# NilsJochem/audio-matcher

Measured on AMD Instinct MI355X. Metric: audio samples/s matched (whole node), 10 s needle vs 1 h haystack, 1/2/4/8 GPU, higher is better.
Workload: dtype f32

## Files before the change

audio-matcher_amd/csrc/am_context.hip:

```cpp
#include "am_internal.h"

namespace am {

thread_local std::string t_err;

int fail(int code, const std::string& msg) {
    t_err = msg;
    return code;
}
int hip_fail(hipError_t e, const char* what) {
    char buf[256];
    snprintf(buf, sizeof(buf), "%s: %s", what, hipGetErrorString(e));
    t_err = buf;
    return e == hipErrorOutOfMemory ? AM_ERR_OOM : AM_ERR_HIP;
}

static std::mutex g_hooks_mu;
static Hooks g_hooks;
Hooks snapshot_hooks() {
    std::lock_guard<std::mutex> lk(g_hooks_mu);
    return g_hooks;
}

using OptRule = const char* (*)(long long& v);
static const char* opt_any(long long&) { return nullptr; }
static const char* opt_bool(long long& v) { v = v ? 1 : 0; return nullptr; }
static const char* opt_log_n(long long& v) { return v != 0 && (v < kLogNMin || v > kLogNMax) ? "log_n out of range" : nullptr; }
static const char* opt_half(long long& v) { v = v <= 0 ? 0 : (v >= 2 ? 2 : 1); return nullptr; }
static const char* opt_every(long long& v) { v = v < 1 ? 1 : v; return nullptr; }
static const char* opt_arm_at(long long& v) { v = v < -1 ? -2 : v; return nullptr; }
static const char* opt_needle_group(long long& v) { return v < 1 || v > kMaxNeedleGroup ? "needle_group out of range" : nullptr; }
static const char* opt_pairs(long long& v) { return v < 1 || v > 64 ? "pairs_per_group out of range" : nullptr; }
static const char* opt_score_norm(long long& v) { return v < 0 || v > 1 ? "score_norm out of range (0 = off, 1 = NCC)" : nullptr; }
static const char* opt_floor_db(long long& v) { return v < 0 || v > 200 ? "score_norm_floor_db out of range (0..200)" : nullptr; }
static const char* opt_trace_form(long long& v) { return v < 0 || v > 2 ? "trace_form out of range (0 = by bin length, 1 = wave form, 2 = sliced form)" : nullptr; }
static const char* opt_distance(long long& v) {
    return v < 0 || v > 3 ? "distance_rule out of range (bit 0: inclusive, bit 1: between plateau starts)" : nullptr;
}
struct Option {
    const char* name;
    std::atomic<long long> value;
    OptRule rule;
    long long Opts::*field;
};
static Option g_options[] = {
    {"log_n", {0}, opt_log_n, &Opts::log_n},
    {"pairs_per_group", {64}, opt_pairs, &Opts::pairs_per_group},
    {"profile_mask", {-1}, opt_any, &Opts::profile_mask},
    {"profile_every", {1}, opt_every, &Opts::profile_every},
    {"half_pipeline", {0}, opt_half, &Opts::half},
    {"batch_overlap", {1}, opt_bool, &Opts::batch_overlap},
    {"needle_group", {8}, opt_needle_group, &Opts::needle_group},
    {"pick_stream_priority", {0}, opt_bool, &Opts::pick_priority},
    {"pick_group", {1}, opt_bool, &Opts::pick_group},
    {"k3_group", {1}, opt_bool, &Opts::k3_group},
    {"host_pick_wait", {1}, opt_bool, &Opts::host_pick_wait},
    {"device_redo", {1}, opt_bool, &Opts::device_redo},
    {"tail_block", {1}, opt_bool, &Opts::tail_block},
    {"dense_scores", {0}, opt_bool, &Opts::dense},
    {"score_norm", {0}, opt_score_norm, &Opts::score_norm},
    {"score_norm_floor_db", {60}, opt_floor_db, &Opts::score_norm_floor_db},
    {"debug_no_realloc", {0}, opt_bool, &Opts::debug_no_realloc},
    {"debug_redo_arm_at", {-2}, opt_arm_at, &Opts::debug_redo_arm_at},
    {"trace_form", {0}, opt_trace_form, &Opts::trace_form},
    {"peak_filter_order", {0}, opt_bool, &Opts::peak_filter_order},
    {"distance_rule", {0}, opt_distance, &Opts::distance_rule},
    {"tail_window", {0}, opt_bool, &Opts::tail_window},
    {"surrounding_from", {0}, opt_bool, &Opts::surrounding_from},
};
static Option* find_option(const char* key) {
    for (Option& r : g_options)
        if (!strcmp(key, r.name)) return &r;
    return nullptr;
}

thread_local const Opts* t_opts_pin = nullptr;
Opts snapshot_opts(const am_needle* h) {
    if (t_opts_pin) return *t_opts_pin;
    Opts o;
    for (const Option& r : g_options) o.*r.field = r.value.load(std::memory_order_relaxed);
    if (h && h->opt_log_n >= 0) o.log_n = h->opt_log_n;
    if (h && h->opt_half >= 0) o.half = h->opt_half;
    if (h && h->opt_score_norm >= 0) o.score_norm = h->opt_score_norm;
    return o;
}

thread_local int t_no_realloc = 0;
int realloc_refused(const char* what, size_t bytes, size_t cap) {
    char buf[160];
    snprintf(buf, sizeof(buf), "debug_no_realloc: %s buffer would grow from %zu to %zu bytes while a call is queueing", what, cap, bytes);
    return fail(AM_ERR_HIP, buf);
}

static const char* kKernelNames[] = {"k1_cols_fwd", "k2_rows", "k3_cols_inv", "tile_stats", "peaks", "other", "trace", "discover"};
static std::mutex g_ctx_mu;
static std::map<int, Ctx*> g_ctx;

int get_ctx(int device, Ctx** out) {
    std::lock_guard<std::mutex> lk(g_ctx_mu);
    int n = 0;
    hipError_t e = hipGetDeviceCount(&n);
    if (e != hipSuccess || n <= 0) return fail(AM_ERR_NO_DEVICE, "no HIP device available");
    if (device < 0 || device >= n) return fail(AM_ERR_NO_DEVICE, "device ordinal out of range");
    auto it = g_ctx.find(device);
    if (it != g_ctx.end()) { *out = it->second; AM_HIP(hipSetDevice(device)); return AM_OK; }
    AM_HIP(hipSetDevice(device));
    (void)hipSetDeviceFlags(hipDeviceScheduleSpin);
    (void)hipGetLastError();
    AM_HIP(fft_kernels_init());
    Ctx* c = new Ctx();
    c->device = device;
    c->hdr.flags = hipHostMallocMapped | hipHostMallocCoherent;
    c->failcnt.flags = hipHostMallocMapped | hipHostMallocCoherent;
    c->spill.flags = hipHostMallocMapped | hipHostMallocCoherent;
    hipError_t se = hipStreamCreateWithFlags(&c->stream, hipStreamNonBlocking);
    if (se != hipSuccess) { delete c; return hip_fail(se, "hipStreamCreate"); }
    {
        int least = 0, greatest = 0;
        if (snapshot_opts(nullptr).pick_priority && hipDeviceGetStreamPriorityRange(&least, &greatest) == hipSuccess && least != greatest)
            (void)hipStreamCreateWithPriority(&c->stream2, hipStreamNonBlocking, least);
        else
            (void)hipStreamCreateWithFlags(&c->stream2, hipStreamNonBlocking);
        (void)hipGetLastError();
    }
    (void)hipStreamCreateWithFlags(&c->stream_tail, hipStreamNonBlocking);
    (void)hipEventCreateWithFlags(&c->ev_fork, kSyncEvent);
    (void)hipEventCreateWithFlags(&c->ev_join, kSyncEvent);
    (void)hipGetLastError();
    for (int i = 0; i < 2; ++i) {
        (void)hipEventCreateWithFlags(&c->ev_k3[i], kSyncEvent);
        (void)hipEventCreateWithFlags(&c->ev_pick[i], kSyncEvent);
    }
    g_ctx[device] = c;
    *out = c;
    return AM_OK;
}

static hipEvent_t prof_event(Ctx* c) {
    if (!c->pool.empty()) { hipEvent_t e = c->pool.back(); c->pool.pop_back(); return e; }
    hipEvent_t e = nullptr;
    (void)hipEventCreateWithFlags(&e, AM_EVENT_NO_SYSTEM_FENCE ? hipEventDisableSystemFence : hipEventDefault);
    return e;
}
ProfScope::ProfScope(Ctx* c_, int name_, hipStream_t st_) : c(c_), name(name_), st(st_ ? st_ : c_->stream) {
    on = c->prof;
    if (on) {
        const Opts o = snapshot_opts(nullptr);
        on = ((o.profile_mask >> name) & 1) && (c->prof_seq[name]++ % (uint64_t)std::max<long long>(1, o.profile_every)) == 0;
    }
    if (on) { e0 = prof_event(c); e1 = prof_event(c); (void)hipEventRecord(e0, st); }
}
static void prof_harvest(Ctx* c) {
    if (c->pending.empty()) return;
    (void)hipStreamSynchronize(c->stream);
    if (c->stream2) (void)hipStreamSynchronize(c->stream2);
    if (c->stream_tail) (void)hipStreamSynchronize(c->stream_tail);
    for (auto& r : c->pending) {
        float ms = 0.f;
        if (hipEventElapsedTime(&ms, r.e0, r.e1) == hipSuccess) { c->prof_ms[r.name] += ms; c->prof_n[r.name] += 1; }
        c->pool.push_back(r.e0); c->pool.push_back(r.e1);
    }
    c->pending.clear();
}

hipError_t copy_on_stream(Ctx* c, void* dst, const void* src, size_t bytes, hipMemcpyKind kind) {
    hipError_t e = hipMemcpyAsync(dst, src, bytes, kind, c->stream);
    if (e != hipSuccess) return e;
    return hipStreamSynchronize(c->stream);
}

static void fill_twiddles(std::vector<float2>& v, size_t off, size_t count, double denom, double mult) {
    for (size_t k = 0; k < count; ++k) {
        const double ang = -2.0 * M_PI * (double)k * mult / denom;
        v[off + k] = make_float2((float)std::cos(ang), (float)std::sin(ang));
    }
}

static void build_mfma_tables(std::vector<unsigned>& tab) {
    tab.assign((size_t)k2_mfma_table_dwords(), 0u);
    auto pack = [](double re, double im) {
        const _Float16 a = (_Float16)re, b = (_Float16)im;
        unsigned short ua, ub;
        memcpy(&ua, &a, 2); memcpy(&ub, &b, 2);
        return (unsigned)ua | ((unsigned)ub << 16);
    };
    auto operand = [&](size_t base, int m_off, int p_off, double denom) {
        for (int ri = 0; ri < 2; ++ri)
            for (int lane = 0; lane < 64; ++lane)
                for (int pp = 0; pp < 4; ++pp) {
                    const int m = m_off + (lane & 15), pt = p_off + 4 * (lane >> 4) + pp;
                    const double ang = 2.0 * M_PI * (double)((m * pt) % (int)denom) / denom;
                    tab[base + (size_t)ri * 256 + (size_t)lane * 4 + pp] = ri == 0 ? pack(std::cos(ang), std::sin(ang)) : pack(-std::sin(ang), std::cos(ang));
                }
    };
    operand(0, 0, 0, 16.0);
    for (int mb = 0; mb < 2; ++mb)
        for (int ks = 0; ks < 2; ++ks) operand(512 + (size_t)(mb * 2 + ks) * 512, 16 * mb, 16 * ks, 32.0);
    const size_t t1 = 512 + 2048, t2 = t1 + 256 * 32;
    for (int t = 0; t < 256; ++t) {
        const int w = t >> 6, g = (t >> 4) & 3, n = t & 15;
        for (int gl = 0; gl < 4; ++gl)
            for (int e = 0; e < 2; ++e)
                for (int r = 0; r < 4; ++r) {
                    const long long m = ((long long)(32 * (4 * w + gl) + 2 * n + e) * (4 * g + r)) % 8192;
                    const double ang = -2.0 * M_PI * (double)m / 8192.0;
                    tab[t1 + (size_t)t * 32 + gl * 8 + e * 4 + r] = pack(std::cos(ang), std::sin(ang));
                }
        for (int ch = 0; ch < 2; ++ch)
            for (int r = 0; r < 4; ++r) {
                const int m = ((16 * ch + n) * (4 * g + r)) % 512;
                const double ang = -2.0 * M_PI * (double)m / 512.0;
                tab[t2 + (size_t)t * 8 + ch * 4 + r] = pack(std::cos(ang), std::sin(ang));
            }
    }
}

// ... 370 lines not shown
```

audio-matcher_amd/csrc/am_correlate.hip:

```cpp
#include "am_internal.h"

namespace am {

static int pick_log_n(size_t s, long long out_count, const Opts& o, int* logN_out) {
    int min_log = kLogNMin;
    while (min_log <= kLogNMax && ((size_t)1 << min_log) < s + 1) ++min_log;
    if (min_log > kLogNMax) return fail(AM_ERR_INVALID_ARG, "needle too long for a forced transform size (2^23 at most; leave log_n at 0 for needle partitioning)");
    if (o.log_n > 0) {
        int l = (int)o.log_n;
        if (l < min_log) l = min_log;
        if (l > kLogNMax) l = kLogNMax;
        *logN_out = l;
        return AM_OK;
    }
    const long long span = out_count + (long long)s - 1;
    if (span > (1ll << 19)) {
        if ((long long)s <= kWideFromSamples) { *logN_out = 21; return AM_OK; }
        if ((long long)s <= kWidestFromSamples) {
            long long hop21 = (1ll << 21) - (long long)s + 1;
            if (hop21 >= 8 * kTile) hop21 = (hop21 / kTile) * kTile;
            *logN_out = (hop21 > 0 && out_count <= 2 * hop21) ? 21 : 22;
            return AM_OK;
        }
        if ((long long)s <= kSegmentFrom) {
            long long hop22 = (1ll << 22) - (long long)s + 1;
            if (hop22 >= 8 * kTile) hop22 = (hop22 / kTile) * kTile;
            *logN_out = (hop22 > 0 && out_count <= 2 * hop22) ? 22 : 23;
            return AM_OK;
        }
    }
    int pref = min_log;
    while (pref < kLogNMax) {
        const double n = (double)((size_t)1 << pref);
        if ((n - (double)s + 1.0) / n >= kMinEfficiency) break;
        ++pref;
    }
    int single = kLogNMin;
    while (single < kLogNMax && (long long)((size_t)1 << single) < span) ++single;
    *logN_out = std::min(pref, std::max(single, min_log));
    return AM_OK;
}

int plan_geometry(size_t s, long long out_count, const Opts& o, Geometry* g) {
    int rc = pick_log_n(s, out_count, o, &g->logN);
    if (rc) return rc;
    g->N = 1ll << g->logN;
    g->hop = g->N - (long long)s + 1;
    if (g->hop >= 8 * kTile) g->hop = (g->hop / kTile) * kTile;
    g->nblocks = (out_count + g->hop - 1) / g->hop;
    g->npairs = (g->nblocks + 1) / 2;
    return AM_OK;
}
bool tail_plan(size_t s, long long out_count, const Opts& o, const Geometry& g, TailPlan* t) {
    t->on = false;
    if (!o.tail_block || o.log_n != 0 || g.logN < 22 || !(g.nblocks & 1) || g.nblocks < 3 || (g.hop % kTile) != 0) return false;
    const long long T = (g.nblocks - 1) * g.hop, rest = out_count - T;
    for (int lt = 21; lt < g.logN; ++lt) {
        const long long N = 1ll << lt;
        long long hop = N - (long long)s + 1;
        if (hop < 8 * kTile) continue;
        hop = (hop / kTile) * kTile;
        if (2 * hop < rest) continue;
        t->on = true; t->T = T;
        t->g.logN = lt; t->g.N = N; t->g.hop = hop; t->g.nblocks = (rest + hop - 1) / hop; t->g.npairs = 1;
        return true;
    }
    return false;
}

static size_t sparse_word_bytes(long long nblocks, const PlanDev& pl) {
    return sizeof(unsigned long long) * (size_t)nblocks * ballot_layout(pl.logN1, pl.logN2).words;
}
size_t sparse_bytes(long long nblocks, const PlanDev& pl) {
    return sparse_word_bytes(nblocks, pl) + sizeof(float) * (size_t)nblocks * ballot_layout(pl.logN1, pl.logN2).tiles;
}
void fill_scan_cfg(ScanCfg* cfg, void* stats32, void* side, long long nblocks, const PlanDev& pl, float margin, float hist_min,
                          long long seg_c, long long seg_d) {
    cfg->stats32 = static_cast<float2*>(stats32);
    cfg->wbits = static_cast<unsigned long long*>(side);
    cfg->tile_theta = reinterpret_cast<float*>(static_cast<char*>(side) + sparse_word_bytes(nblocks, pl));
    cfg->margin = margin;
    cfg->hist_min = hist_min;
    cfg->seg_c = seg_c; cfg->seg_d = seg_d;
    cfg->inv_c = seg_c > 0 ? 1.0 / (double)seg_c : 0.0;
}
SparseScores sparse_view(const ScanCfg& cfg, long long hop, const PlanDev& pl) {
    if (cfg.margin < 0.0f) return SparseScores{nullptr, cfg.stats32, nullptr, (int)hop, pl.logN2, pl.logN1, 1.0 / (double)hop};
    return SparseScores{cfg.wbits, cfg.stats32, cfg.tile_theta, (int)hop, pl.logN2, pl.logN1, 1.0 / (double)hop};
}

bool needle_is_segmented(const am_needle* h, const Opts& o) {
    return (long long)h->n > kSegmentFrom && o.log_n == 0;
}
static void needle_segments(am_needle* h) {
    if (!h->segments.empty()) return;
    const long long n = (long long)h->n;
    const long long nseg = (n + kSegmentLen - 1) / kSegmentLen;
    for (long long i = 0; i < nseg; ++i) {
        const long long a = n * i / nseg, b = n * (i + 1) / nseg;
        am_needle* sub = new am_needle();
        sub->ctx = h->ctx; sub->d_needle = h->d_needle + a; sub->n = (size_t)(b - a);
        sub->inv_autocorr = h->inv_autocorr; sub->owns_data = false;
        h->segments.push_back(sub);
        h->seg_off.push_back(a);
    }
}

bool plan_fuses_scan(const PlanDev& pl, const Geometry& g) { return plan_has_scan(pl) && (g.hop % kTile) == 0; }

int pass_plan(am_needle* h, const Opts& o, long long out_count, bool allow_tail, PassPlan* pp) {
    Ctx* c = h->ctx;
    *pp = PassPlan{};
    int rc;
    if (needle_is_segmented(h, o)) {
        pp->kind = PassKind::Partitioned;
        needle_segments(h);
        Opts os = o;
        os.half = 0;
        pp->parts.resize(h->segments.size());
        for (size_t i = 0; i < pp->parts.size(); ++i) {
            if ((rc = pass_plan(h->segments[i], os, out_count, false, &pp->parts[i]))) return rc;
            pp->need.work = std::max(pp->need.work, pp->parts[i].need.work);
        }
        return AM_OK;
    }
    if (h->n <= (size_t)kDirectMaxNeedle && o.log_n == 0) return AM_OK;
    pp->kind = PassKind::Transform;
    Geometry& g = pp->g;
    if ((rc = plan_geometry(h->n, out_count, o, &g))) return rc;
    if ((rc = get_plan(c, g.logN, &pp->pl))) return rc;
    if ((rc = needle_k2_spectrum(h, o, pp->pl, &pp->hc, &pp->hs))) return rc;
    pp->fused = plan_fuses_scan(pp->pl->dev, g);
    if (allow_tail && pp->fused && c->stream_tail && c->ev_fork && c->ev_join && tail_plan(h->n, out_count, o, g, &pp->tail)) {
        if ((rc = get_plan(c, pp->tail.g.logN, &pp->tail_pl))) return rc;
        if ((rc = needle_k2_spectrum(h, o, pp->tail_pl, &pp->tail_hc, &pp->tail_hs))) return rc;
        pp->need.work_tail = (size_t)pp->tail.g.N * sizeof(float2);
    }
    pp->nblocks = pp->tail.on ? g.nblocks - 1 : g.nblocks;
    pp->npairs = pp->tail.on ? g.npairs - 1 : g.npairs;
    pp->main_count = pp->tail.on ? pp->tail.T : out_count;
    pp->ppg = std::min(std::max<long long>(1, o.pairs_per_group), pp->npairs);
    pp->need.work = (size_t)pp->ppg * (size_t)g.N * sizeof(float2);
    pp->need.npairs = g.npairs;
    if (pp->fused) {
        pp->need.stats32 = (size_t)((out_count + 31) / 32) * sizeof(float2);
        pp->need.side = sparse_bytes(g.nblocks, pp->pl->dev);
    }
    return AM_OK;
}

static int run_tail_block(Ctx* c, const PassPlan& pp, const void* d_src, long long src_len,
                          float* d_dst, long long out_count, float factor, const ScanCfg& main_scan, int src_kind) {
    hipStream_t st = c->stream_tail;
    const TailPlan& tail = pp.tail;
    const PlanDev& pl = pp.tail_pl->dev;
    const HalfScale& hs = pp.tail_hs;
    int rc;
    if ((rc = c->work_tail.ensure(pp.need.work_tail))) return rc;
    Job job = tail_job(tail, d_src, src_len, out_count, src_kind);
    job.dst = d_dst + tail.T;
    ScanCfg scan{};
    scan.stats32 = main_scan.stats32 ? main_scan.stats32 + tail.T / 32 : nullptr;
    scan.margin = -1.0f; scan.hist_min = FLT_MAX;
    { ProfScope ps(c, KN_OTHER, st); AM_HIP(launch_k1(st, job, 1, (float2*)c->work_tail.p, pl, hs.level)); }
    { ProfScope ps(c, KN_OTHER, st); AM_HIP(launch_k2(st, 1, (float2*)c->work_tail.p, pp.tail_hc, pl, nullptr, hs.level, hs.hscale, hs.pre, true)); }
    { ProfScope ps(c, KN_OTHER, st); AM_HIP(launch_k3(st, job, 1, (const float2*)c->work_tail.p, pl, hs.k3(factor), scan, hs.level, false)); }
    if (main_scan.stats32 && main_scan.margin >= 0.0f && main_scan.wbits && main_scan.tile_theta) {
        const BallotLayout bl = ballot_layout(pp.pl->dev.logN1, pp.pl->dev.logN2);
        const size_t blk = (size_t)(pp.g.nblocks - 1);
        AM_HIP(hipMemsetAsync(main_scan.wbits + blk * bl.words, 0xFF, bl.words * sizeof(unsigned long long), st));
        AM_HIP(hipMemsetD32Async(reinterpret_cast<hipDeviceptr_t>(main_scan.tile_theta + blk * bl.tiles), (int)0xFF7FFFFFu, bl.tiles, st));
    }
    return AM_OK;
}

static int run_correlation_one(am_needle* h, const PassPlan& pp, const void* d_src, long long src_len, long long lead,
                               float* d_dst, long long out_count, float factor,
                               const ScanRequest* scan_req, ScanResult* res, int src_kind, bool accumulate);

int run_correlation(am_needle* h, const Opts& o, const void* d_src, long long src_len, long long lead,
                           float* d_dst, long long out_count, float factor,
                           const ScanRequest* scan_req, ScanResult* res, int src_kind, const PassPlan* plan) {
    int rc;
    PassPlan own;
    if (!plan) {
        if ((rc = pass_plan(h, o, out_count, scan_req && !scan_req->no_scan && lead == 0, &own))) return rc;
        plan = &own;
    }
    if (res) { res->fused = false; res->redo_ok = false; res->sparse = plain_scores(); }
    if (plan->kind != PassKind::Partitioned) return run_correlation_one(h, *plan, d_src, src_len, lead, d_dst, out_count, factor, scan_req, res, src_kind, false);
    if (scan_req && scan_req->skip_launch) return fail(AM_ERR_INVALID_ARG, "internal: streaming ingest does not run early pairs for partitioned needles");
    for (size_t i = 0; i < plan->parts.size(); ++i) {
        ScanRequest plain{};
        if (scan_req) {
            plain.margin = -1.0f; plain.range_a = scan_req->range_a; plain.range_b = scan_req->range_b;
            plain.before_k3 = i == 0 ? scan_req->before_k3 : nullptr;
            plain.no_scan = true;
        }
        if ((rc = run_correlation_one(h->segments[i], plan->parts[i], d_src, src_len, lead - h->seg_off[i], d_dst, out_count, factor,
                                      scan_req ? &plain : nullptr, nullptr, src_kind, i > 0)))
            return rc;
    }
    return AM_OK;
}

static int run_correlation_one(am_needle* h, const PassPlan& pp, const void* d_src, long long src_len, long long lead,
                               float* d_dst, long long out_count, float factor,
                               const ScanRequest* scan_req, ScanResult* res, int src_kind, bool accumulate) {
    Ctx* c = h->ctx;
    Job job{};
    job.src = d_src; job.src_len = src_len; job.lead = lead; job.src_kind = src_kind;
    job.dst = d_dst; job.out_count = out_count;
    if (pp.kind == PassKind::Direct) {
        ProfScope ps(c, KN_OTHER);
        AM_HIP(launch_direct(c->stream, job, h->d_needle, (int)h->n, factor));
        return AM_OK;
    }
    int rc;
    const PlanDev& pl = pp.pl->dev;
    const HalfScale& hs = pp.hs;
    const TailPlan& tail = pp.tail;
    const long long N = pp.g.N, hop = pp.g.hop, npairs = pp.npairs, ppg = pp.ppg;
    const ScanBuffers out = (scan_req && scan_req->out.work) ? scan_req->out : scan_buffers(c->side[0]);
    DevBuf& wk = *out.work;
    if ((rc = wk.ensure((size_t)ppg * (size_t)N * sizeof(float2)))) return rc;
    ScanCfg scan{};
    bool fused = false;
    if (scan_req && !scan_req->no_scan) {
        if (res) res->sparse = SparseScores{nullptr, nullptr, nullptr, (int)hop, pl.logN2, pl.logN1, 1.0 / (double)hop};
        if (pp.fused) {
            const long long side_blocks = std::max(pp.g.nblocks, scan_req->side_nblocks);
            if ((rc = out.stats32->ensure((size_t)((out_count + 31) / 32) * sizeof(float2)))) return rc;
            if ((rc = out.wflags->ensure(sparse_bytes(side_blocks, pl)))) return rc;
            fill_scan_cfg(&scan, out.stats32->p, out.wflags->p, side_blocks, pl, scan_req->margin, scan_req->hist_min, scan_req->seg_c, scan_req->seg_d);
            fused = true;
            if (res) { res->fused = true; res->sparse = sparse_view(scan, hop, pl); }
        }
    }
    const float k3scale = hs.k3(factor);
    job.out_count = pp.main_count; job.hop = (int)hop; job.nblocks = (int)pp.nblocks;
    if (scan_req && scan_req->skip_launch) return AM_OK;
    long long pair_lo = 0, pair_hi = npairs;
    bool with_tail = tail.on;
    if (scan_req && scan_req->range_b > scan_req->range_a) {
        pair_lo = (scan_req->range_a / hop) / 2;
        pair_hi = std::min(npairs, ((scan_req->range_b - 1) / hop) / 2 + 1);
        with_tail = tail.on && scan_req->range_b > tail.T;
    }
    if (scan_req && scan_req->tail_by_caller) with_tail = false;
    if (with_tail) {
        AM_HIP(hipEventRecord(c->ev_fork, c->stream));
        AM_HIP(hipStreamWaitEvent(c->stream_tail, c->ev_fork, 0));
        if ((rc = run_tail_block(c, pp, d_src, src_len, d_dst, out_count, factor, scan, src_kind))) return rc;
        AM_HIP(hipEventRecord(c->ev_join, c->stream_tail));
    }
    bool waited = false;
    for (long long first = pair_lo; first < pair_hi; first += ppg) {
        const int np = (int)std::min(ppg, pair_hi - first);
        job.first_pair = (int)first;
        { ProfScope ps(c, KN_K1); AM_HIP(launch_k1(c->stream, job, np, (float2*)wk.p, pl, hs.level)); }
        { ProfScope ps(c, KN_K2); AM_HIP(launch_k2(c->stream, np, (float2*)wk.p, pp.hc, pl, nullptr, hs.level, hs.hscale, hs.pre)); }
        if (!waited && scan_req && scan_req->before_k3) AM_HIP(hipStreamWaitEvent(c->stream, scan_req->before_k3, 0));
        waited = true;
        { ProfScope ps(c, KN_K3); AM_HIP(launch_k3(c->stream, job, np, (const float2*)wk.p, pl, k3scale, scan, hs.level, accumulate)); }
    }
    if (with_tail) AM_HIP(hipStreamWaitEvent(c->stream, c->ev_join, 0));
    if (res && fused && !accumulate && pair_lo == 0 && pair_hi == npairs && npairs <= ppg) {
        res->redo_ok = true;
        job.first_pair = 0;
        res->redo_job = job; res->redo_pl = pl; res->redo_scale = k3scale; res->redo_half = hs.level;
        res->redo_npairs = (int)npairs; res->redo_work = (const float2*)wk.p; res->redo_cfg = scan;
    }
    return AM_OK;
}

float scale_factor(const am_needle* h, int scale, size_t w) {
    if (scale == AM_SCALE_LIB) return h->inv_autocorr;
    if (scale == AM_SCALE_MY) return h->inv_autocorr / (float)w;
    return 1.0f;
}

static uint64_t start_nanos(uint64_t start, uint32_t sr) {
    const double t = (double)start / (double)sr;
    if (!(t > 0.0)) return 0;
    int e = 0;
    const double m = std::frexp(t, &e);
    const unsigned long long mant = (unsigned long long)std::ldexp(m, 53);
    const int sh = e - 53;
    unsigned __int128 v = (unsigned __int128)mant * 1000000000ull;
    if (sh >= 0) return (uint64_t)(v << sh);
    const int r = -sh;
    if (r >= 127) return 0;
    unsigned __int128 q = v >> r;
    const unsigned __int128 rem = v & (((unsigned __int128)1 << r) - 1);
    const unsigned __int128 half = (unsigned __int128)1 << (r - 1);
    if (rem > half || (rem == half && (q & 1))) ++q;
    return (uint64_t)q;
}

static bool is_overshadowed(const am_peak& element, const am_peak* other, uint32_t sr, double max_distance_s) {
    if (!other) return false;
    uint64_t e = start_nanos(element.start, sr), b = start_nanos(other->start, sr);
    if (e < b) std::swap(e, b);
    const uint64_t maxd = (uint64_t)std::llround(max_distance_s * 1e9);
    return (e - b) < maxd && other->prominence > element.prominence;
}

int upload_segments(Ctx* c, const std::vector<Segment>& segs) {
    const size_t bytes = sizeof(Segment) * segs.size();
    if (c->segs.p && segs.size() == c->segs_resident.size() &&
        memcmp(segs.data(), c->segs_resident.data(), bytes) == 0)
        return AM_OK;
    int rc;
    c->segs_resident.clear();
    if ((rc = c->segs.ensure(bytes))) return rc;
    if ((rc = c->pinned.ensure(bytes))) return rc;
    memcpy(c->pinned.p, segs.data(), bytes);
    AM_HIP(hipMemcpyAsync(c->segs.p, c->pinned.p, bytes, hipMemcpyHostToDevice, c->stream));
    AM_HIP(hipStreamSynchronize(c->stream));
    c->segs_resident = segs;
    return AM_OK;
}

int prepare_results(Ctx* c, size_t nhdr, size_t arena_entries, PeakArena* arena) {
    const size_t hdr_bytes = (sizeof(SegHeader) * nhdr + 63) / 64 * 64;
    int rc;
    if ((rc = c->hdr.ensure(hdr_bytes + sizeof(am_peak) * arena_entries))) return rc;
    if ((rc = c->arena_cur.ensure(sizeof(unsigned)))) return rc;
    AM_HIP(hipMemsetAsync(c->arena_cur.p, 0, sizeof(unsigned), c->stream));
    arena->base = reinterpret_cast<am_peak*>(static_cast<char*>(c->hdr.p) + hdr_bytes);
    arena->cursor = static_cast<unsigned*>(c->arena_cur.p);
    arena->cap = (unsigned)arena_entries;
    return AM_OK;
}

int wide_reserve(Ctx* c, size_t n) {
    int rc;
    if ((rc = c->wide_ctl.ensure(n * kWideCtlBytes))) return rc;
    if ((rc = c->wide_list.ensure(n * AM_MAX_PEAKS_PER_CHUNK * sizeof(am_peak)))) return rc;
// ... 178 lines not shown
```

audio-matcher_amd/csrc/am_engine.hip:

```cpp
#include "am_internal.h"

namespace am {

static int launch_pick_group(Ctx* c, const K3Group& kg, long long n_scores, int seg_off, int nsegs, float min_prom, long long min_dist,
                             const SparseScores& sp_common, int* bad, const int* hdr_off, const PeakArena& arena, const PeakPolicy& pol,
                             hipStream_t st) {
    if (nsegs == 0 || n_scores <= 0 || kg.n <= 0) return AM_OK;
    int rc;
    const size_t nz = (size_t)kg.n, total = nz * (size_t)nsegs;
    const long long ntiles = (n_scores + kTile - 1) / kTile;
    PickGroup pg{};
    pg.n = kg.n;
    for (int z = 0; z < kg.n; ++z) {
        if ((rc = c->grp_stats[z].ensure((size_t)ntiles * sizeof(float2)))) return rc;
        pg.g[z] = kg.dst[z]; pg.stats[z] = static_cast<float2*>(c->grp_stats[z].p);
        pg.stats32[z] = kg.stats32[z]; pg.wbits[z] = kg.wbits[z]; pg.theta[z] = kg.tile_theta[z];
        pg.hdr_off[z] = hdr_off[z];
    }
    { ProfScope ps(c, KN_STATS, st);
      AM_HIP(launch_stats_reduce(st, pg.stats32[0], n_scores, pg.stats[0], bad, &pg)); }
    if ((rc = wide_reserve(c, total))) return rc;
    if ((rc = c->side[0].peaks.ensure(total * AM_MAX_PEAKS_PER_CHUNK * sizeof(am_peak)))) return rc;
    {
        ProfScope ps(c, KN_PEAKS, st);
        AM_HIP(launch_peaks(st, pg.g[0], n_scores, pg.stats[0], (const Segment*)c->segs.p + seg_off, nsegs, min_prom, min_dist,
                            (am_peak*)c->side[0].peaks.p, (SegHeader*)c->hdr.p, sp_common, arena, wide_carve(c, total), false, pol, &pg));
    }
    return AM_OK;
}


struct ChunkPlan {
    std::vector<Segment> segs, short_segs;
    std::vector<size_t> widths, short_w;
    std::vector<int> seg_off, short_off;
    std::vector<int> n_chunks;
    size_t max_scores = 0, max_segs = 1;
    int ns(size_t k) const { return seg_off[k + 1] - seg_off[k]; }
    bool too_many(size_t nn) const { return max_segs > (size_t)1 << 18 || segs.size() * nn > (size_t)1 << 24; }
};
static void plan_chunks(size_t s, const void* const* d_hays, const size_t* lens, size_t n_hay, const am_match_params* p, const Opts& o,
                        bool split_short, size_t max_windows, ChunkPlan* cp) {
    const size_t window = (size_t)(p->chunk + p->overlap);
    cp->seg_off.assign(n_hay + 1, 0);
    cp->short_off.assign(n_hay + 1, 0);
    cp->n_chunks.assign(n_hay, 0);
    for (size_t k = 0; k < n_hay; ++k) {
        cp->seg_off[k] = (int)cp->segs.size();
        cp->short_off[k] = (int)cp->short_segs.size();
        if (!d_hays[k] || lens[k] < s) continue;
        std::vector<Segment> one;
        std::vector<size_t> w1;
        make_segments(lens[k], s, p, o.tail_window != 0, one, &w1, max_windows);
        cp->n_chunks[k] = (int)one.size();
        for (size_t i = 0; i < one.size(); ++i) {
            const bool shorter = split_short && w1[i] != window;
            (shorter ? cp->short_segs : cp->segs).push_back(one[i]);
            (shorter ? cp->short_w : cp->widths).push_back(w1[i]);
        }
        if (!one.empty()) cp->max_scores = std::max(cp->max_scores, lens[k] - s + 1);
        cp->max_segs = std::max(cp->max_segs, cp->segs.size() - (size_t)cp->seg_off[k]);
    }
    cp->seg_off[n_hay] = (int)cp->segs.size();
    cp->short_off[n_hay] = (int)cp->short_segs.size();
}

struct ScoreSets {
    Ctx* c;
    bool overlap;
    size_t seq = 0;
    ScoreSets(Ctx* c_, const Opts& o, size_t n_items)
        : c(c_), overlap(o.batch_overlap && n_items > 1 && c_->stream2 && c_->ev_k3[0] && c_->ev_k3[1] && c_->ev_pick[0] && c_->ev_pick[1]) {}
    int count() const { return overlap ? 2 : 1; }
    int set() const { return overlap ? (int)(seq & 1) : 0; }
    ScoreSide& side() const { return c->side[set()]; }
    float* scores() const { return (float*)side().scores.p; }
    hipStream_t pick_stream() const { return overlap ? c->stream2 : c->stream; }
    int size(size_t max_scores, size_t max_segs) {
        int rc;
        for (int set = 0; set < count(); ++set) {
            ScoreSide& sd = c->side[set];
            if ((rc = sd.scores.ensure(max_scores * sizeof(float)))) return rc;
            if ((rc = sd.peaks.ensure(sizeof(am_peak) * max_segs * AM_MAX_PEAKS_PER_CHUNK))) return rc;
            if ((rc = sd.stats.ensure((max_scores + kTile - 1) / kTile * sizeof(float2)))) return rc;
        }
        return wide_reserve(c, max_segs);
    }
    int wait_pick(bool on_host) {
        if (!overlap || seq < 2) return AM_OK;
        if (on_host) AM_HIP(hipEventSynchronize(c->ev_pick[set()]));
        else AM_HIP(hipStreamWaitEvent(c->stream, c->ev_pick[set()], 0));
        return AM_OK;
    }
    int k3_done() {
        if (!overlap) return AM_OK;
        AM_HIP(hipEventRecord(c->ev_k3[set()], c->stream));
        AM_HIP(hipStreamWaitEvent(c->stream2, c->ev_k3[set()], 0));
        return AM_OK;
    }
    int pick_done() {
        if (overlap) AM_HIP(hipEventRecord(c->ev_pick[set()], c->stream2));
        ++seq;
        return AM_OK;
    }
    int drain() {
        AM_HIP(hipStreamSynchronize(c->stream));
        if (overlap) AM_HIP(hipStreamSynchronize(c->stream2));
        return AM_OK;
    }
};

static int match_alone(am_needle* h, const void* d_hay, size_t len, const am_match_params* p, am_peak* out, size_t cap, size_t slot,
                       size_t* n_out, int src_kind, const PartSpec* part, int* worst) {
    const int rc = match_many(h, &d_hay, &len, 1, p, out ? out + slot * cap : nullptr, cap, &n_out[slot], src_kind, 0, 1, false, nullptr, part);
    if (rc == AM_ERR_CAPACITY) *worst = rc;
    return rc == AM_ERR_CAPACITY ? AM_OK : rc;
}

static int pick_alone(am_needle* h, const Opts& o, const am_match_params* p, const void* src, long long src_len, float factor,
                      const ScanRequest& req, long long n_scores, int seg_idx, const Segment& sg, int spare_hdr, uint64_t shift, int src_kind,
                      const NormSpec& nrm, std::vector<am_peak>& all) {
    Ctx* c = h->ctx;
    const PeakPolicy pol = o.peak_policy();
    int rc;
    PeakArena own{};
    if ((rc = c->spill.ensure(sizeof(am_peak) * AM_MAX_PEAKS_PER_CHUNK))) return rc;
    AM_HIP(hipMemsetAsync(c->arena_cur.p, 0, sizeof(unsigned), c->stream));
    own.base = static_cast<am_peak*>(c->spill.p); own.cursor = static_cast<unsigned*>(c->arena_cur.p);
    own.cap = AM_MAX_PEAKS_PER_CHUNK;
    ScoreSide& side = c->side[0];
    if ((rc = side.scores.ensure((size_t)n_scores * sizeof(float)))) return rc;
    float* d_scores = (float*)side.scores.p;
    ScanResult res{};
    if ((rc = run_correlation(h, o, src, src_len, 0, d_scores, n_scores, factor, &req, &res, src_kind))) return rc;
    if (nrm.on) {
        if ((rc = normalise_scores(c, c->stream, nrm, src, src_len, src_kind, 0, (long long)h->n, d_scores, sg.a, std::min(sg.b, n_scores))))
            return rc;
        res.fused = false;
    }
    if ((rc = launch_pick(c, side, d_scores, n_scores, seg_idx, 1, p->min_prominence, (long long)p->min_distance, nullptr, &res, spare_hdr, own, pol))) return rc;
    AM_HIP(hipStreamSynchronize(c->stream));
    const SegHeader& hd = static_cast<const SegHeader*>(c->hdr.p)[spare_hdr];
    const size_t old = all.size();
    if (hd.overflow & 1) {
        if ((rc = pick_chunk_big(c, d_scores, n_scores, seg_idx, sg, p->min_prominence, (long long)p->min_distance, &res, hd.seg_min, all, pol)))
            return rc;
    } else append_header_peaks(hd, own, all);
    for (size_t j = old; j < all.size(); ++j) { all[j].start += shift; all[j].end += shift; }
    return AM_OK;
}

struct TailSlots { size_t scores, stats; };
static bool tail_batchable(const TailPlan& t) { return t.on && t.g.logN == 21; }
static int launch_tail_batch(am_needle* h, const std::vector<PassPlan>& plans, const std::vector<size_t>& members, int half_idx,
                             const TailSlots& sl, const void* const* d_hays, const size_t* lens, float factor, int src_kind) {
    Ctx* c = h->ctx;
    const PassPlan& lead = plans[members[0]];
    const TailPlan& first = lead.tail;
    const Plan* pl = lead.tail_pl;
    const float2* hc = lead.tail_hc;
    const HalfScale& hs = lead.tail_hs;
    TailBatch tb{};
    tb.n = (int)members.size();
    for (int j = 0; j < tb.n; ++j) {
        const size_t k = members[j];
        const size_t slot = (size_t)half_idx * kMaxTailBatch + (size_t)j;
        const Job job = tail_job(plans[k].tail, d_hays[k], (long long)lens[k], (long long)(lens[k] - h->n + 1), src_kind);
        tb.src[j] = job.src;
        tb.src_len[j] = job.src_len;
        tb.out_count[j] = job.out_count;
        tb.dst[j] = static_cast<float*>(c->tail_scores.p) + slot * sl.scores;
        tb.stats32[j] = static_cast<float2*>(c->tail_stats.p) + slot * sl.stats;
    }
    float2* work = static_cast<float2*>(c->work_tail.p);
    { ProfScope ps(c, KN_OTHER); AM_HIP(launch_tail_batch_k1(c->stream, tb, (int)first.g.hop, src_kind, work, pl->dev, hs.level)); }
    { ProfScope ps(c, KN_OTHER); AM_HIP(launch_k2(c->stream, tb.n, work, hc, pl->dev, nullptr, hs.level, hs.hscale, hs.pre, true)); }
    { ProfScope ps(c, KN_OTHER); AM_HIP(launch_tail_batch_k3(c->stream, tb, (int)first.g.hop, work, pl->dev, hs.k3(factor), hs.level)); }
    return AM_OK;
}

static int classify_nonfinite(am_needle* h, const PassPlan& pp, const float* d_hay, size_t len,
                              const std::vector<Segment>& segs, int s0, int s1,
                              std::vector<char>* drop, std::vector<char>* again) {
    Ctx* c = h->ctx;
    const long long s = (long long)h->n;
    const int nch = s1 - s0;
    drop->assign(nch, 0); again->assign(nch, 0);
    std::vector<Segment> ranges;
    for (int i = s0; i < s1; ++i)
        ranges.push_back(Segment{segs[i].a, std::min<long long>((long long)len, segs[i].b + s - 1)});
    const long long npairs = pp.kind == PassKind::Transform ? pp.npairs : 0;
    for (long long q = 0; q < npairs; ++q) ranges.push_back(pp.pair_reads(q, (long long)len));
    if (pp.tail.on) ranges.push_back(pp.tail_reads((long long)len));
    std::vector<int> flags(ranges.size(), 0);
    int rc = nonfinite_flags(c, d_hay, ranges.data(), (int)ranges.size(), flags.data());
    if (rc) return rc;
    for (int i = 0; i < nch; ++i) {
        if (flags[i]) { (*drop)[i] = 1; continue; }
        if (pp.kind == PassKind::Partitioned) { (*again)[i] = 1; continue; }
        const Segment sg = segs[s0 + i];
        for (long long q = 0; q < npairs && !(*again)[i]; ++q)
            if (flags[nch + q] && 2 * q * pp.g.hop < sg.b && (2 * q + 2) * pp.g.hop > sg.a) (*again)[i] = 1;
        if (pp.tail.on && flags[nch + npairs] && pp.tail.T < sg.b) (*again)[i] = 1;
    }
    return AM_OK;
}

int match_many(am_needle* h, const void* const* d_hays, const size_t* lens, size_t n_hay,
               const am_match_params* p, am_peak* out, size_t cap_per_hay, size_t* n_out, int src_kind,
               size_t index_base, size_t index_stride, bool fire_hooks, const StreamPre* pre, const PartSpec* part) {
    Ctx* c = h->ctx;
    const Opts o = snapshot_opts(h);
    const PeakPolicy pol = o.peak_policy();
    Hooks hooks = fire_hooks ? snapshot_hooks() : Hooks{};
    if (part) hooks.fn = nullptr;
    if (part && n_hay != 1) return fail(AM_ERR_INVALID_ARG, "internal: a part is one haystack");
    auto G = [&](size_t k) { return index_base + k * index_stride; };
    const size_t s = h->n;
    if (p->chunk == 0) return fail(AM_ERR_INVALID_ARG, "chunk must be > 0");
    if (p->scale < AM_SCALE_NONE || p->scale > AM_SCALE_MY) return fail(AM_ERR_INVALID_ARG, "bad scale");
    const NormSpec nrm = norm_spec(h, o);
    if (nrm.on && (pre || part)) return fail(AM_ERR_INVALID_ARG, AM_NORM_UNSUPPORTED);
    int rc = norm_check(nrm, p->scale);
    if (rc) return rc;
    const bool my = p->scale == AM_SCALE_MY;
    const float factor = nrm.on ? norm_factor(nrm) : scale_factor(h, p->scale, (size_t)(p->chunk + p->overlap));
    const int sm = p->scale == AM_SCALE_LIB ? 1 : 0;
    ScanRequest base{};
    base.margin = nrm.on ? -1.0f : write_margin(o, p);
    const bool sparse_ok = base.margin >= 0.0f;
    base.hist_min = nrm.on ? FLT_MAX : h->hist_min(sm);
    base.seg_c = (long long)p->chunk;
    base.seg_d = (long long)(p->chunk + p->overlap) - (long long)s;
    for (size_t k = 0; k < n_hay; ++k) n_out[G(k)] = 0;
    ChunkPlan cp;
    plan_chunks(s, d_hays, lens, n_hay, p, o, my, part ? part->max_windows : (size_t)-1, &cp);
    const std::vector<Segment>& segs = cp.segs;
    const std::vector<int>& seg_off = cp.seg_off;
    const size_t nsegs = segs.size();
    if (nsegs == 0 && cp.short_segs.empty()) return AM_OK;
    if (cp.too_many(1)) return fail(AM_ERR_INVALID_ARG, "chunk size too small for this haystack (more than 2^18 chunks)");
    size_t n_active = 0;
    for (size_t k = 0; k < n_hay; ++k) n_active += cp.ns(k) > 0;
    ScoreSets sets(c, o, n_active);
    if ((rc = sets.size(cp.max_scores, cp.max_segs))) return rc;
    std::vector<PassPlan> plans(n_hay);
    Footprint need;
    for (size_t k = 0; k < n_hay; ++k) {
        if (cp.n_chunks[k] == 0 || cp.ns(k) == 0) continue;
        if ((rc = pass_plan(h, o, (long long)(lens[k] - s + 1), pre == nullptr, &plans[k]))) return rc;
        need.take(plans[k].need);
    }
    std::vector<int> tail_slot(n_hay, -1);
    TailSlots tslots{0, 0};
    bool batch_tails = false;
    if (need.work_tail) {
        size_t n_tails = 0;
        for (size_t k = 0; k < n_hay; ++k)
            if (tail_batchable(plans[k].tail)) {
                ++n_tails;
                tslots.scores = std::max(tslots.scores, (size_t)(2 * plans[k].tail.g.hop));
            }
        tslots.stats = tslots.scores / 32;
        batch_tails = sets.overlap && n_tails > 1;
        const size_t nslot = batch_tails ? kMaxTailBatch : 1;
        if ((rc = c->work_tail.ensure(need.work_tail * nslot))) return rc;
        if (batch_tails) {
            if ((rc = c->tail_scores.ensure(2 * kMaxTailBatch * tslots.scores * sizeof(float)))) return rc;
            if ((rc = c->tail_stats.ensure(2 * kMaxTailBatch * tslots.stats * sizeof(float2)))) return rc;
        }
    }
    int tail_batches = 0;
    for (int set = 0; set < sets.count(); ++set) {
        if (need.work && (rc = c->side[set].work.ensure(need.work))) return rc;
        if (pre) continue;
        if (need.stats32 && (rc = c->side[set].stats32.ensure(need.stats32))) return rc;
        if (need.side && (rc = c->side[set].wflags.ensure(need.side))) return rc;
    }
    PeakArena arena{};
    if ((rc = prepare_results(c, nsegs + 1, std::min<size_t>(cp.max_segs * AM_MAX_PEAKS_PER_CHUNK, (size_t)1 << 20) + nsegs * 8, &arena))) return rc;
    std::vector<Segment> resident = segs;
    for (const Segment& sg : cp.short_segs) resident.push_back(Segment{0, sg.b - sg.a});
    const int local_seg = (int)resident.size();
    resident.push_back(Segment{0, std::max<long long>(base.seg_d + 1, 1)});
    if ((rc = upload_segments(c, resident))) return rc;
    if ((rc = c->badflag.ensure(sizeof(int) * n_hay))) return rc;
    int* h_bad = static_cast<int*>(c->badflag.p);
    memset(h_bad, 0, sizeof(int) * n_hay);
    if ((rc = c->failcnt.ensure(nsegs + 1))) return rc;
    if (nrm.on) {
        size_t max_len = 0;
        for (size_t k = 0; k < n_hay; ++k) if (cp.ns(k) > 0) max_len = std::max(max_len, lens[k]);
        if ((rc = norm_reserve(c, (long long)max_len))) return rc;
    }
    unsigned char* h_fail = static_cast<unsigned char*>(c->failcnt.p);
    memset(h_fail, 0, nsegs + 1);
    const bool device_redo = sets.overlap && sparse_ok && !needle_is_segmented(h, o) && o.device_redo != 0;
    if (device_redo) {
        for (int set = 0; set < 2; ++set)
            if ((rc = c->redo_pairs[set].ensure(sizeof(int) * (size_t)std::max<long long>(need.npairs, 1)))) return rc;
    }
    SegHeader* h_hdr = static_cast<SegHeader*>(c->hdr.p);
    auto chunk_events = [&](size_t k, int stage) {
        if (hooks.chunk_fn)
            for (int i = 0; i < cp.n_chunks[k]; ++i)
                hooks.chunk_fn(hooks.chunk_user, G(k), (part ? part->chunk_base : 0) + (size_t)i,
                               part ? part->chunk_total : (size_t)cp.n_chunks[k], stage);
    };
    const bool arm_forced = o.debug_redo_arm_at >= -1;
    bool redo_armed = device_redo && (arm_forced ? o.debug_redo_arm_at == 0 : h->redo_armed_left[sm] > 0);
    QueueingScope queueing(o.debug_no_realloc != 0);
    for (size_t k = 0; k < n_hay; ++k) {
        const int ns = cp.ns(k);
        if (cp.n_chunks[k] == 0) continue;
        if (device_redo && arm_forced) redo_armed = o.debug_redo_arm_at >= 0 && (long long)k >= o.debug_redo_arm_at;
        else if (device_redo && !redo_armed && (k & 3) == 0) {
            const volatile unsigned char* f = h_fail;
            for (int i = 0; i < seg_off[k] && !redo_armed; ++i) redo_armed = f[i] != 0;
        }
        if (hooks.fn) hooks.fn(hooks.user, G(k), 0, (size_t)cp.n_chunks[k]);
        chunk_events(k, 0);
        if (ns == 0) continue;
        const long long out_count = (long long)(lens[k] - s + 1);
        const int set = sets.set();
        const PassPlan& pp = plans[k];
        ScoreSide& side = sets.side();
        float* d_scores = sets.scores();
        ScanRequest req = base;
        req.out = scan_buffers(side);
// ... 463 lines not shown
```

audio-matcher_amd/csrc/am_fft.hip:

```cpp
#include "am_kernels.h"

#include <float.h>
#include <stdlib.h>
#include <algorithm>
#include <atomic>
#include <hip/hip_fp16.h>

namespace am {

__device__ __forceinline__ float2 cadd(float2 a, float2 b) { return make_float2(a.x + b.x, a.y + b.y); }
__device__ __forceinline__ float2 csub(float2 a, float2 b) { return make_float2(a.x - b.x, a.y - b.y); }
__device__ __forceinline__ float2 cmul(float2 a, float2 b) {
    return make_float2(a.x * b.x - a.y * b.y, a.x * b.y + a.y * b.x);
}
__device__ __forceinline__ float2 cmulc(float2 a, float2 b) {
    return make_float2(a.x * b.x + a.y * b.y, a.y * b.x - a.x * b.y);
}
__device__ __forceinline__ float2 mul_neg_i(float2 a) { return make_float2(a.y, -a.x); }
__device__ __forceinline__ float2 mul_pos_i(float2 a) { return make_float2(-a.y, a.x); }

__device__ __forceinline__ float2 tw_big(const PlanDev& pl, unsigned m) {
    return cmul(pl.twhi[m >> pl.logLo], pl.twlo[m & ((1u << pl.logLo) - 1u)]);
}

// ... 31 lines not shown
}

typedef _Float16 h2 __attribute__((ext_vector_type(2)));
__device__ __forceinline__ h2 cadd(h2 a, h2 b) { return a + b; }
__device__ __forceinline__ h2 csub(h2 a, h2 b) { return a - b; }
__device__ __forceinline__ h2 cmul(h2 a, h2 b) {
    const h2 t = a * b.xx;
    return __builtin_elementwise_fma(a.yx, (h2){-b.y, b.y}, t);
}
__device__ __forceinline__ h2 mul_neg_i(h2 a) { return (h2){a.y, -a.x}; }
__device__ __forceinline__ h2 mul_pos_i(h2 a) { return (h2){-a.y, a.x}; }
__device__ __forceinline__ h2 to_h2(float2 v) { return (h2){(_Float16)v.x, (_Float16)v.y}; }
__device__ __forceinline__ float2 to_f2(h2 v) { return make_float2((float)v.x, (float)v.y); }
__device__ __forceinline__ unsigned h2_bits(h2 v) { return __builtin_bit_cast(unsigned, v); }
__device__ __forceinline__ h2 bits_h2(unsigned u) { return __builtin_bit_cast(h2, u); }
template <bool INV>
__device__ __forceinline__ h2 mul_w32(h2 d, int idx) {
    if (idx == 0) return d;
    if (idx == 8) return INV ? mul_pos_i(d) : mul_neg_i(d);
    const _Float16 c = (_Float16)kCos32[idx], s = (_Float16)kSin32[idx];
    const h2 t = d * (h2){c, c};
    if (INV) return __builtin_elementwise_fma(d.yx, (h2){-s, s}, t);
    return __builtin_elementwise_fma(d.yx, (h2){s, -s}, t);
}

__device__ __forceinline__ float2 add_signed(float2 u, float2 v, float sgn) {
    return make_float2(fmaf(sgn, v.x, u.x), fmaf(sgn, v.y, u.y));
}

template <int R, bool INV, typename T>
__device__ __forceinline__ void dif(T* x) {
    if constexpr (R >= 2) {
#pragma unroll
        for (int i = 0; i < R / 2; ++i) {
            const T a = x[i], b = x[i + R / 2];
            x[i] = cadd(a, b);
            x[i + R / 2] = mul_w32<INV>(csub(a, b), i * (32 / R));
        }
        dif<R / 2, INV>(x);
        dif<R / 2, INV>(x + R / 2);
    }
}

template <int R, bool CONJ, bool BREV>
__device__ __forceinline__ void twiddle_apply(float2* x, float2 w) {
    float2 pw[R / 2 + 1];
    if (CONJ) w.y = -w.y;
    pw[1] = w;
    x[BREV ? brev<R>(1) : 1] = cmul(x[BREV ? brev<R>(1) : 1], w);
#pragma unroll
    for (int e = 2; e < R; ++e) {
        const float2 v = cmul(pw[(e + 1) / 2], pw[e / 2]);
        if (e <= R / 2) pw[e] = v;
        x[BREV ? brev<R>(e) : e] = cmul(x[BREV ? brev<R>(e) : e], v);
    }
}
template <int R, bool CONJ, bool BREV>
__device__ __forceinline__ void twiddle_apply(h2* x, float2 w) {
    float2 pw[R / 2 + 1];
    if (CONJ) w.y = -w.y;
    pw[1] = w;
    x[BREV ? brev<R>(1) : 1] = cmul(x[BREV ? brev<R>(1) : 1], to_h2(w));
#pragma unroll
    for (int e = 2; e < R; ++e) {
        const float2 v = cmul(pw[(e + 1) / 2], pw[e / 2]);
        if (e <= R / 2) pw[e] = v;
        x[BREV ? brev<R>(e) : e] = cmul(x[BREV ? brev<R>(e) : e], to_h2(v));
    }
}
template <int R, bool CONJ, bool BREV>
__device__ __forceinline__ void twiddle_apply2(h2* x0, h2* x1, float2 w) {
    float2 pw[R / 2 + 1];
    if (CONJ) w.y = -w.y;
    pw[1] = w;
    {
        const h2 wh = to_h2(w);
        x0[BREV ? brev<R>(1) : 1] = cmul(x0[BREV ? brev<R>(1) : 1], wh);
        x1[BREV ? brev<R>(1) : 1] = cmul(x1[BREV ? brev<R>(1) : 1], wh);
    }
#pragma unroll
    for (int e = 2; e < R; ++e) {
        const float2 v = cmul(pw[(e + 1) / 2], pw[e / 2]);
        if (e <= R / 2) pw[e] = v;
        const h2 vh = to_h2(v);
        x0[BREV ? brev<R>(e) : e] = cmul(x0[BREV ? brev<R>(e) : e], vh);
        x1[BREV ? brev<R>(e) : e] = cmul(x1[BREV ? brev<R>(e) : e], vh);
    }
}
template <int R, bool CONJ, bool BREV>
__device__ __forceinline__ void twiddle_chain(h2* x, float2 base, float2 step) {
    if (CONJ) { base.y = -base.y; step.y = -step.y; }
    float2 c = base;
    x[0] = cmul(x[0], to_h2(c));
#pragma unroll
    for (int e = 1; e < R; ++e) {
        c = cmul(c, step);
        x[BREV ? brev<R>(e) : e] = cmul(x[BREV ? brev<R>(e) : e], to_h2(c));
    }
}
template <int R, bool CONJ, bool BREV>
__device__ __forceinline__ void twiddle_chain(float2* x, float2 base, float2 step) {
    if (CONJ) { base.y = -base.y; step.y = -step.y; }
    float2 c = base;
    x[0] = cmul(x[0], c);
#pragma unroll
    for (int e = 1; e < R; ++e) {
        c = cmul(c, step);
        x[BREV ? brev<R>(e) : e] = cmul(x[BREV ? brev<R>(e) : e], c);
    }
}
template <int R, bool CONJ, typename T>
__device__ __forceinline__ void twiddle_brev(T* x, float2 w) { twiddle_apply<R, CONJ, true>(x, w); }
template <int R, bool CONJ, typename T>
__device__ __forceinline__ void twiddle_nat(T* x, float2 w) { twiddle_apply<R, CONJ, false>(x, w); }

__device__ __forceinline__ float2 tw_as(float2 v, float2) { return v; }
__device__ __forceinline__ h2 tw_as(float2 v, h2) { return to_h2(v); }
template <int R, bool CONJ, bool BREV, typename T>
__device__ __forceinline__ void twiddle_apply(T* x, float2 w, float2 w4) {
    static_assert(R == 16, "powers 1..15 from w and w^4");
    if (CONJ) { w.y = -w.y; w4.y = -w4.y; }
    float2 lo[4];
    lo[1] = w; lo[2] = cmul(w, w); lo[3] = cmul(lo[2], w);
    float2 g = w4;
#pragma unroll
    for (int e = 1; e < R; ++e) {
        if ((e & 3) == 0 && e > 4) g = cmul(g, w4);
        const float2 v = e < 4 ? lo[e] : (e & 3) == 0 ? g : cmul(g, lo[e & 3]);
        x[BREV ? brev<R>(e) : e] = cmul(x[BREV ? brev<R>(e) : e], tw_as(v, T{}));
    }
}
template <int R, bool CONJ, typename T>
__device__ __forceinline__ void twiddle_brev(T* x, float2 w, float2 w4) { twiddle_apply<R, CONJ, true>(x, w, w4); }
template <int R, bool CONJ, typename T>
__device__ __forceinline__ void twiddle_nat(T* x, float2 w, float2 w4) { twiddle_apply<R, CONJ, false>(x, w, w4); }
template <int R, bool CONJ, bool BREV, typename T>
__device__ __forceinline__ void twiddle_chain(T* x, float2 base, float2 step, float2 step4) {
    static_assert(R == 16, "four runs of four");
    if (CONJ) { base.y = -base.y; step.y = -step.y; step4.y = -step4.y; }
    float2 g = base;
#pragma unroll
    for (int k = 0; k < R; k += 4) {
        if (k) g = cmul(g, step4);
        float2 c = g;
        x[BREV ? brev<R>(k) : k] = cmul(x[BREV ? brev<R>(k) : k], tw_as(c, T{}));
#pragma unroll
        for (int j = 1; j < 4; ++j) {
            c = cmul(c, step);
            x[BREV ? brev<R>(k + j) : k + j] = cmul(x[BREV ? brev<R>(k + j) : k + j], tw_as(c, T{}));
        }
    }
}

typedef float f32x4 __attribute__((ext_vector_type(4)));
typedef float f32x2 __attribute__((ext_vector_type(2)));
__device__ __forceinline__ __amdgpu_buffer_rsrc_t make_rsrc(const void* p, unsigned bytes) {
    return __builtin_amdgcn_make_buffer_rsrc(const_cast<void*>(p), 0, bytes, 0x00020000);
}
template <int AUX = 0>
__device__ __forceinline__ float4 buf_load4(__amdgpu_buffer_rsrc_t r, unsigned voff, unsigned soff) {
    const f32x4 v = __builtin_bit_cast(f32x4, __builtin_amdgcn_raw_buffer_load_b128(r, voff, soff, AUX));
    return make_float4(v.x, v.y, v.z, v.w);
}
template <int AUX = 0>
__device__ __forceinline__ void buf_store4(__amdgpu_buffer_rsrc_t r, unsigned voff, unsigned soff, float4 v) {
    f32x4 o; o.x = v.x; o.y = v.y; o.z = v.z; o.w = v.w;
    __builtin_amdgcn_raw_buffer_store_b128(__builtin_bit_cast(__attribute__((__vector_size__(4 * sizeof(unsigned)))) unsigned, o), r, voff, soff, AUX);
    asm volatile("s_nop 1" : : "v"(o));
}

__device__ __forceinline__ unsigned pack_h2(float2 v) {
    const __half2 h = __float22half2_rn(v);
    return __builtin_bit_cast(unsigned, h);
}
__device__ __forceinline__ float2 unpack_h2(unsigned u) {
    return __half22float2(__builtin_bit_cast(__half2, u));
}
template <int AUX = 0>
__device__ __forceinline__ uint2 buf_load_u2(__amdgpu_buffer_rsrc_t r, unsigned voff, unsigned soff) {
    const f32x2 v = __builtin_bit_cast(f32x2, __builtin_amdgcn_raw_buffer_load_b64(r, voff, soff, AUX));
    const float lo = v.x, hi = v.y;
    return make_uint2(__float_as_uint(lo), __float_as_uint(hi));
}
__device__ __forceinline__ void buf_store_u2(__amdgpu_buffer_rsrc_t r, unsigned voff, unsigned soff, uint2 v) {
    typedef unsigned u32x2 __attribute__((ext_vector_type(2)));
    u32x2 o; o.x = v.x; o.y = v.y;
    __builtin_amdgcn_raw_buffer_store_b64(__builtin_bit_cast(__attribute__((__vector_size__(2 * sizeof(unsigned)))) unsigned, o), r, voff, soff, 0);
}

constexpr int kR16LogN1 = 8, kR16LogN2 = 13;
constexpr int kN2 = 1 << kR16LogN2;

__device__ __forceinline__ float downmix_s16(short2 lr) {
    return __fmul_rn((float)((int)lr.x + (int)lr.y), 0.5f * (1.0f / 65535.0f));
}
template <int KIND>
__device__ __forceinline__ float load_sample(const void* __restrict__ src, long long i) {
    if (KIND == 0) return static_cast<const float*>(src)[i];
    return downmix_s16(static_cast<const short2*>(src)[i]);
}
template <int KIND>
__device__ __forceinline__ float2 decode_sample2(uint2 raw) {
    if (KIND == 0) return make_float2(__uint_as_float(raw.x), __uint_as_float(raw.y));
    short2 a, b;
    a.x = (short)(raw.x & 0xffffu); a.y = (short)(raw.x >> 16);
    b.x = (short)(raw.y & 0xffffu); b.y = (short)(raw.y >> 16);
    return make_float2(downmix_s16(a), downmix_s16(b));
}
constexpr bool kK1LoadNt = true;
template <int KIND>
__device__ __forceinline__ float2 load_sample2(const void* __restrict__ src, long long i) {
    if (KIND == 0) {
        if (kK1LoadNt) {
            const f32x2 v = __builtin_nontemporal_load(reinterpret_cast<const f32x2*>(static_cast<const float*>(src) + i));
            return make_float2(v.x, v.y);
        }
        return *reinterpret_cast<const float2*>(static_cast<const float*>(src) + i);
    }
    typedef int i32x2 __attribute__((ext_vector_type(2)));
    const i32x2* p = reinterpret_cast<const i32x2*>(static_cast<const short2*>(src) + i);
    const i32x2 raw = kK1LoadNt ? __builtin_nontemporal_load(p) : *p;
    const int lo = raw.x, hi = raw.y;
    return make_float2(downmix_s16(__builtin_bit_cast(short2, lo)), downmix_s16(__builtin_bit_cast(short2, hi)));
}
template <int KIND>
__device__ __forceinline__ float2 load2_padded(const void* __restrict__ src, long long i, long long len) {
    float2 v;
    v.x = (i >= 0 && i < len) ? load_sample<KIND>(src, i) : 0.0f;
    v.y = (i + 1 >= 0 && i + 1 < len) ? load_sample<KIND>(src, i + 1) : 0.0f;
    return v;
}

struct K1Twiddles { float2 w256, w256q, base0, base1, step0, step1, step0q, step1q; };
__device__ __forceinline__ K1Twiddles k1_twiddles(const PlanDev& pl, long long col, int hi) {
    const unsigned maskN = (unsigned)((1ll << pl.logN) - 1);
    K1Twiddles w;
    w.w256 = pl.tw1[hi];
    w.w256q = pl.tw1[4 * hi];
    w.base0 = tw_big(pl, ((unsigned)col * (unsigned)hi) & maskN);
    w.base1 = tw_big(pl, (((unsigned)col + 1u) * (unsigned)hi) & maskN);
    tw_big_pair(pl, ((unsigned)col * 16u) & maskN, w.step0, w.step0q);
    tw_big_pair(pl, (((unsigned)col + 1u) * 16u) & maskN, w.step1, w.step1q);
    return w;
}
template <int KIND>
__device__ __forceinline__ void k1_load(const Job& job, long long col, int in_stride, int hi, long long baseA, long long baseB,
                                        bool validB, bool fast, float2 (&x0)[16], float2 (&x1)[16]) {
    if (fast) {
#pragma unroll
        for (int a = 0; a < 16; ++a) {
            const long long off = (long long)(a * 16 + hi) * in_stride + col;
            const float2 va = load_sample2<KIND>(job.src, baseA + off), vb = load_sample2<KIND>(job.src, baseB + off);
            x0[a] = make_float2(va.x, vb.x);
            x1[a] = make_float2(va.y, vb.y);
        }
    } else {
#pragma unroll
        for (int a = 0; a < 16; ++a) {
            const long long n = (long long)(a * 16 + hi) * in_stride + col;
            const float2 va = load2_padded<KIND>(job.src, baseA + n, job.src_len);
            const float2 vb = validB ? load2_padded<KIND>(job.src, baseB + n, job.src_len) : make_float2(0.f, 0.f);
            x0[a] = make_float2(va.x, vb.x);
            x1[a] = make_float2(va.y, vb.y);
        }
    }
}
__device__ __forceinline__ void k1_transform(const K1Twiddles& w, float2* lds2, int hi, int cp, float2 (&x0)[16], float2 (&x1)[16]) {
    dif<16, false>(x0);
    dif<16, false>(x1);
    twiddle_brev<16, false>(x0, w.w256, w.w256q);
    twiddle_brev<16, false>(x1, w.w256, w.w256q);
#pragma unroll
    for (int ap = 0; ap < 16; ++ap) lds2[(ap * 16 + hi) * 17 + cp] = x0[brev<16>(ap)];
    __syncthreads();
#pragma unroll
    for (int b = 0; b < 16; ++b) x0[b] = lds2[(hi * 16 + b) * 17 + cp];
    __syncthreads();
#pragma unroll
    for (int ap = 0; ap < 16; ++ap) lds2[(ap * 16 + hi) * 17 + cp] = x1[brev<16>(ap)];
    __syncthreads();
#pragma unroll
    for (int b = 0; b < 16; ++b) x1[b] = lds2[(hi * 16 + b) * 17 + cp];
    dif<16, false>(x0);
    dif<16, false>(x1);
    twiddle_chain<16, false, true>(x0, w.base0, w.step0, w.step0q);
    twiddle_chain<16, false, true>(x1, w.base1, w.step1, w.step1q);
}
template <int KIND>
__device__ __forceinline__ void k1_tile(const Job& job, const PlanDev& pl, float2* lds2, long long col, int in_stride,
                                        int hi, int cp, long long baseA, long long baseB, bool validB, bool fast,
                                        float2 (&x0)[16], float2 (&x1)[16]) {
    const K1Twiddles w = k1_twiddles(pl, col, hi);
    k1_load<KIND>(job, col, in_stride, hi, baseA, baseB, validB, fast, x0, x1);
    k1_transform(w, lds2, hi, cp, x0, x1);
}

__device__ __forceinline__ void k1_transform_h16(const K1Twiddles& w, uint2* ldsu, int hi, int cp, h2 (&x0)[16], h2 (&x1)[16]) {
    dif<16, false>(x0);
    dif<16, false>(x1);
    twiddle_apply2<16, false, true>(x0, x1, w.w256);
#pragma unroll
    for (int ap = 0; ap < 16; ++ap) ldsu[(ap * 16 + hi) * 17 + cp] = make_uint2(h2_bits(x0[brev<16>(ap)]), h2_bits(x1[brev<16>(ap)]));
    __syncthreads();
#pragma unroll
    for (int b = 0; b < 16; ++b) {
        const uint2 v = ldsu[(hi * 16 + b) * 17 + cp];
        x0[b] = bits_h2(v.x);
        x1[b] = bits_h2(v.y);
    }
    dif<16, false>(x0);
    dif<16, false>(x1);
    twiddle_chain<16, false, true>(x0, w.base0, w.step0);
    twiddle_chain<16, false, true>(x1, w.base1, w.step1);
}

template <int KIND, int HALF>
__device__ __forceinline__ void k1_cols_fwd_r16_tile(const Job& job, float2* __restrict__ work, const PlanDev& pl) {
    extern __shared__ float4 lds4[];
    const int t = threadIdx.x;
    const int hi = t >> 4, cp = t & 15;
    const int n2_0 = blockIdx.x << kColsLog;
    const int pair = job.first_pair + blockIdx.y;
    const long long blkA = 2ll * pair, blkB = blkA + 1;
    const bool validB = blkB < job.nblocks;
    const long long N = 1ll << pl.logN;
    const long long baseA = blkA * job.hop - job.lead;
    const long long baseB = blkB * job.hop - job.lead;
    const bool fast = ((reinterpret_cast<uintptr_t>(job.src) & 7) == 0) && ((baseA & 1) == 0) && ((baseB & 1) == 0) &&
                      baseA >= 0 && baseA + N <= job.src_len && validB && baseB + N <= job.src_len;
    float2 x0[16], x1[16];
    if constexpr (HALF == 2) {
        const long long col = (long long)n2_0 + 2 * cp;
        const K1Twiddles w = k1_twiddles(pl, col, hi);
        k1_load<KIND>(job, col, kN2, hi, baseA, baseB, validB, fast, x0, x1);
        h2 hx0[16], hx1[16];
#pragma unroll
        for (int a = 0; a < 16; ++a) { hx0[a] = to_h2(x0[a]); hx1[a] = to_h2(x1[a]); }
        k1_transform_h16(w, reinterpret_cast<uint2*>(lds4), hi, cp, hx0, hx1);
        uint2* __restrict__ out2 = reinterpret_cast<uint2*>(reinterpret_cast<unsigned*>(work) + ((size_t)blockIdx.y << pl.logN) + n2_0) + cp;
#pragma unroll
        for (int bp = 0; bp < 16; ++bp) {
            const size_t k1 = (size_t)(hi + 16 * bp);
            out2[k1 * (kN2 / 2)] = make_uint2(h2_bits(hx0[brev<16>(bp)]), h2_bits(hx1[brev<16>(bp)]));
        }
        return;
    }
    k1_tile<KIND>(job, pl, reinterpret_cast<float2*>(lds4), (long long)n2_0 + 2 * cp, kN2, hi, cp, baseA, baseB, validB, fast, x0, x1);
    if (HALF) {
        uint2* __restrict__ out2 = reinterpret_cast<uint2*>(reinterpret_cast<unsigned*>(work) + ((size_t)blockIdx.y << pl.logN) + n2_0) + cp;
#pragma unroll
        for (int bp = 0; bp < 16; ++bp) {
            const size_t k1 = (size_t)(hi + 16 * bp);
            out2[k1 * (kN2 / 2)] = make_uint2(pack_h2(x0[brev<16>(bp)]), pack_h2(x1[brev<16>(bp)]));
        }
        return;
    }
    float4* __restrict__ out4 = reinterpret_cast<float4*>(work + ((size_t)blockIdx.y << pl.logN) + n2_0) + cp;
#pragma unroll
    for (int bp = 0; bp < 16; ++bp) {
        const size_t k1 = (size_t)(hi + 16 * bp);
        out4[k1 * (kN2 / 2)] = make_float4(x0[brev<16>(bp)].x, x0[brev<16>(bp)].y,
                                             x1[brev<16>(bp)].x, x1[brev<16>(bp)].y);
    }
}
template <int KIND, int HALF>
__global__ void __launch_bounds__(256, 3)
k1_cols_fwd_r16(Job job, float2* __restrict__ work, PlanDev pl) {
    k1_cols_fwd_r16_tile<KIND, HALF>(job, work, pl);
}
template <int KIND, int HALF>
__global__ void __launch_bounds__(256, 3)
tail_cols_fwd_r16(TailBatch tb, int hop, float2* __restrict__ work, PlanDev pl) {
    const unsigned z = blockIdx.y;
    Job job;
    job.src = tb.src[z]; job.src_len = tb.src_len[z]; job.lead = 0; job.dst = nullptr; job.out_count = tb.out_count[z];
    job.hop = hop; job.nblocks = (int)((tb.out_count[z] + hop - 1) / hop); job.first_pair = -(int)z; job.src_kind = KIND;
    k1_cols_fwd_r16_tile<KIND, HALF>(job, work, pl);
}

__device__ __forceinline__ void wave_sync_lds() {
    __builtin_amdgcn_fence(__ATOMIC_ACQ_REL, "wavefront");
    __builtin_amdgcn_wave_barrier();
}

struct K2Lane {
    int t, hi, cp;
    unsigned voff;
    float2 wj0, wj1, wc0, wc1;
    float2 qj0, qj1, qc0, qc1;
};
__device__ __forceinline__ K2Lane k2_lane(const PlanDev& pl, int t = threadIdx.x) {
    K2Lane k;
    k.t = t; k.hi = k.t >> 4; k.cp = k.t & 15;
    k.voff = (unsigned)k.t * 16u;
    const float4 j = pl.k2j[2 * k.t], jq = pl.k2j[2 * k.t + 1], c = pl.k2c[2 * k.cp], cq = pl.k2c[2 * k.cp + 1];
    k.wj0 = make_float2(j.x, j.y); k.wj1 = make_float2(j.z, j.w);
    k.qj0 = make_float2(jq.x, jq.y); k.qj1 = make_float2(jq.z, jq.w);
    k.wc0 = make_float2(c.x, c.y); k.wc1 = make_float2(c.z, c.w);
    k.qc0 = make_float2(cq.x, cq.y); k.qc1 = make_float2(cq.z, cq.w);
    return k;
}

__device__ __forceinline__ void k2_forward12(const K2Lane& k, __amdgpu_buffer_rsrc_t rrow, float4* lds4) {
    const int t = k.t, hi = k.hi, cp = k.cp;
    float2 x0[16], x1[16];
#pragma unroll
    for (int a = 0; a < 16; ++a) {
        const float4 v = buf_load4(rrow, k.voff, a * 4096);
        x0[a] = make_float2(v.x, v.y);
        x1[a] = make_float2(v.z, v.w);
    }
    dif<16, false>(x0);
    dif<16, false>(x1);
    twiddle_brev<16, false>(x0, k.wj0, k.qj0);
    twiddle_brev<16, false>(x1, k.wj1, k.qj1);
#pragma unroll
    for (int ap = 0; ap < 16; ++ap)
        lds4[ap * 256 + t] = make_float4(x0[brev<16>(ap)].x, x0[brev<16>(ap)].y,
                                         x1[brev<16>(ap)].x, x1[brev<16>(ap)].y);
    __syncthreads();
#pragma unroll
    for (int b = 0; b < 16; ++b) {
        const float4 v = lds4[hi * 256 + b * 16 + cp];
        x0[b] = make_float2(v.x, v.y);
        x1[b] = make_float2(v.z, v.w);
    }
    dif<16, false>(x0);
    dif<16, false>(x1);
    twiddle_brev<16, false>(x0, k.wc0, k.qc0);
    twiddle_brev<16, false>(x1, k.wc1, k.qc1);
    wave_sync_lds();
#pragma unroll
    for (int bp = 0; bp < 16; ++bp)
        lds4[(hi * 16 + bp) * 16 + (cp ^ bp)] = make_float4(x0[brev<16>(bp)].x, x0[brev<16>(bp)].y,
                                                            x1[brev<16>(bp)].x, x1[brev<16>(bp)].y);
    wave_sync_lds();
}

__device__ __forceinline__ void k2_forward3(const K2Lane& k, const float4* lds4, float2 (&z)[32]) {
#pragma unroll
    for (int i = 0; i < 16; ++i) {
        const float4 v = lds4[k.t * 16 + (i ^ k.cp)];
        z[2 * i] = make_float2(v.x, v.y);
        z[2 * i + 1] = make_float2(v.z, v.w);
    }
    dif<32, false>(z);
}

__device__ __forceinline__ void k2_fetch_quarter(__amdgpu_buffer_rsrc_t rh, unsigned voff, int part, float4 (&h)[4]) {
#pragma unroll
    for (int i = 0; i < 4; ++i) h[i] = buf_load4(rh, voff, (part * 4 + i) * 4096);
}
__device__ __forceinline__ void k2_multiply_quarter(const float2 (&z)[32], const float4 (&h)[4], int part, float2 (&q)[32]) {
#pragma unroll
    for (int i = 0; i < 4; ++i) {
        const int e = part * 4 + i;
        q[brev<32>(2 * e)] = cmul(z[2 * e], make_float2(h[i].x, h[i].y));
        q[brev<32>(2 * e + 1)] = cmul(z[2 * e + 1], make_float2(h[i].z, h[i].w));
    }
}
__device__ __forceinline__ void k2_multiply_fetch(const float2 (&z)[32], __amdgpu_buffer_rsrc_t rh, unsigned voff,
                                                  const float4 (&first)[4], float2 (&q)[32]) {
    float4 ha[4], hb[4];
    k2_fetch_quarter(rh, voff, 1, ha);
    __builtin_amdgcn_sched_barrier(0);
    k2_multiply_quarter(z, first, 0, q);
    k2_fetch_quarter(rh, voff, 2, hb);
    __builtin_amdgcn_sched_barrier(0);
    k2_multiply_quarter(z, ha, 1, q);
    k2_fetch_quarter(rh, voff, 3, ha);
    __builtin_amdgcn_sched_barrier(0);
    k2_multiply_quarter(z, hb, 2, q);
    k2_multiply_quarter(z, ha, 3, q);
}

__device__ __forceinline__ void k2_place(unsigned npairs, unsigned& row, unsigned& slot) {
    const unsigned lin = blockIdx.x, xcd = lin & 7u, seq = lin >> 3;
    row = (seq / npairs) * 8u + xcd;
    slot = seq % npairs;
}

__global__ void __launch_bounds__(256, 2)
k2_rows_r16_spectrum(float2* __restrict__ work, const float2* __restrict__ hc, float2* __restrict__ hc_out, PlanDev pl,
                     unsigned npairs, float hscale) {
    extern __shared__ float4 lds4[];
    unsigned row, slot;
    k2_place(npairs, row, slot);
    const size_t row_off = ((size_t)slot << pl.logN) + (size_t)row * kN2;
    const __amdgpu_buffer_rsrc_t rrow = make_rsrc(work + row_off, kN2 * 8);
    const size_t hoff4 = (size_t)row * (kN2 / 2);
    const K2Lane k = k2_lane(pl);
    k2_forward12(k, rrow, lds4);
    float2 z[32];
    k2_forward3(k, lds4, z);
    const float invN = 1.0f / (float)(1u << pl.logN);
    const __amdgpu_buffer_rsrc_t rho = make_rsrc(reinterpret_cast<float4*>(hc_out) + hoff4, kN2 * 8);
#pragma unroll
    for (int i = 0; i < 16; ++i)
        buf_store4(rho, k.voff, i * 4096, make_float4(z[2 * i].x * invN, -z[2 * i].y * invN,
                                                     z[2 * i + 1].x * invN, -z[2 * i + 1].y * invN));
}

constexpr int kK2hSlab = 272;
constexpr int kK2hLds = 16 * kK2hSlab * 8;

constexpr int kK2hWaves = 3;
__device__ __forceinline__ void k2_rows_h16_row(unsigned* __restrict__ work, const unsigned* __restrict__ hc16, unsigned* __restrict__ dst,
                                                const PlanDev& pl, unsigned npairs, float pre) {
    extern __shared__ float4 lds4[];
    uint2* ldsu = reinterpret_cast<uint2*>(lds4);
    unsigned row, slot;
    k2_place(npairs, row, slot);
    const size_t row_off = ((size_t)slot << pl.logN) + (size_t)row * kN2;
    const __amdgpu_buffer_rsrc_t rrow = make_rsrc(work + row_off, kN2 * 4);
    const __amdgpu_buffer_rsrc_t rdst = dst ? make_rsrc(dst + row_off, kN2 * 4) : rrow;
    const K2Lane k = k2_lane(pl);
    const int t = k.t, hi = k.hi, cp = k.cp;
    h2 x0[16], x1[16];
    {
        const h2 p2 = (h2){(_Float16)pre, (_Float16)pre};
#pragma unroll
        for (int a = 0; a < 16; ++a) {
            const uint2 v = buf_load_u2(rrow, k.voff / 2, a * 2048);
            x0[a] = bits_h2(v.x) * p2;
            x1[a] = bits_h2(v.y) * p2;
        }
    }
    dif<16, false>(x0);
    dif<16, false>(x1);
    twiddle_brev<16, false>(x0, k.wj0, k.qj0);
// ... 57 lines not shown
    wave_sync_lds();
#pragma unroll
    for (int b = 0; b < 16; ++b)
        ldsu[hi * kK2hSlab + b * 16 + cp] = make_uint2(h2_bits(x0[brev<16>(b)]), h2_bits(x1[brev<16>(b)]));
    __syncthreads();
#pragma unroll
    for (int ap = 0; ap < 16; ++ap) {
        const uint2 v = ldsu[ap * kK2hSlab + t];
        x0[ap] = bits_h2(v.x);
        x1[ap] = bits_h2(v.y);
    }
    twiddle_nat<16, true>(x0, k.wj0, k.qj0);
    twiddle_nat<16, true>(x1, k.wj1, k.qj1);
    dif<16, true>(x0);
    dif<16, true>(x1);
#pragma unroll
    for (int a = 0; a < 16; ++a)
        buf_store_u2(rdst, k.voff / 2, a * 2048, make_uint2(h2_bits(x0[brev<16>(a)]), h2_bits(x1[brev<16>(a)])));
}
__global__ void __launch_bounds__(256, kK2hWaves)
k2_rows_h16(unsigned* __restrict__ work, const unsigned* __restrict__ hc16, unsigned* __restrict__ dst, PlanDev pl, unsigned npairs,
            float pre) {
    k2_rows_h16_row(work, hc16, dst, pl, npairs, pre);
}
__global__ void __launch_bounds__(256, kK2hWaves)
tail_rows_h16(unsigned* __restrict__ work, const unsigned* __restrict__ hc16, unsigned* __restrict__ dst, PlanDev pl, unsigned npairs,
              float pre) {
    k2_rows_h16_row(work, hc16, dst, pl, npairs, pre);
}

constexpr int kK2pWaves = 4;
template <bool HALF>
__device__ __forceinline__ void k2p_forward(const K2Lane& k, __amdgpu_buffer_rsrc_t rrow, float2* lds2, float2 (&z)[32]) {
    const int t = k.t, hi = k.hi, cp = k.cp;
    float2 x0[16], x1[16];
#pragma unroll
    for (int a = 0; a < 16; ++a) {
        if (HALF) {
            const uint2 v = buf_load_u2(rrow, k.voff / 2, a * 2048);
            x0[a] = unpack_h2(v.x);
            x1[a] = unpack_h2(v.y);
        } else {
            const float4 v = buf_load4(rrow, k.voff, a * 4096);
            x0[a] = make_float2(v.x, v.y);
            x1[a] = make_float2(v.z, v.w);
        }
    }
    dif<16, false>(x0);
    twiddle_brev<16, false>(x0, k.wj0, k.qj0);
#pragma unroll
    for (int ap = 0; ap < 16; ++ap) lds2[ap * kK2hSlab + t] = x0[brev<16>(ap)];
    dif<16, false>(x1);
    twiddle_brev<16, false>(x1, k.wj1, k.qj1);
    __syncthreads();
#pragma unroll
    for (int b = 0; b < 16; ++b) x0[b] = lds2[hi * kK2hSlab + b * 16 + cp];
    __syncthreads();
#pragma unroll
    for (int ap = 0; ap < 16; ++ap) lds2[ap * kK2hSlab + t] = x1[brev<16>(ap)];
    dif<16, false>(x0);
    twiddle_brev<16, false>(x0, k.wc0, k.qc0);
    __syncthreads();
#pragma unroll
    for (int b = 0; b < 16; ++b) x1[b] = lds2[hi * kK2hSlab + b * 16 + cp];
    wave_sync_lds();
#pragma unroll
    for (int bp = 0; bp < 16; ++bp) lds2[hi * kK2hSlab + bp * 16 + (cp ^ bp)] = x0[brev<16>(bp)];
    dif<16, false>(x1);
    twiddle_brev<16, false>(x1, k.wc1, k.qc1);
    wave_sync_lds();
#pragma unroll
    for (int i = 0; i < 16; ++i) z[2 * i] = lds2[hi * kK2hSlab + cp * 16 + (i ^ cp)];
    wave_sync_lds();
#pragma unroll
    for (int bp = 0; bp < 16; ++bp) lds2[hi * kK2hSlab + bp * 16 + (cp ^ bp)] = x1[brev<16>(bp)];
    wave_sync_lds();
#pragma unroll
    for (int i = 0; i < 16; ++i) z[2 * i + 1] = lds2[hi * kK2hSlab + cp * 16 + (i ^ cp)];
}

template <bool HALF, int SAUX = 0, bool LATE_J = false>
__device__ __forceinline__ void k2p_inverse(const PlanDev& pl, float2 (&q)[32], float2* lds2, __amdgpu_buffer_rsrc_t rdst) {
    int t = threadIdx.x;
    asm volatile("" : "+v"(t));
    const int hi = t >> 4, cp = t & 15;
    K2Lane ki;
    ki.t = t; ki.hi = hi; ki.cp = cp; ki.voff = (unsigned)t * 16u;
    {
        const float4 c = pl.k2c[2 * cp], cq = pl.k2c[2 * cp + 1];
        ki.wc0 = make_float2(c.x, c.y); ki.wc1 = make_float2(c.z, c.w);
        ki.qc0 = make_float2(cq.x, cq.y); ki.qc1 = make_float2(cq.z, cq.w);
    }
    if (!LATE_J) {
        const float4 j = pl.k2j[2 * t], jq = pl.k2j[2 * t + 1];
        ki.wj0 = make_float2(j.x, j.y); ki.wj1 = make_float2(j.z, j.w);
        ki.qj0 = make_float2(jq.x, jq.y); ki.qj1 = make_float2(jq.z, jq.w);
    }
    const K2Lane& k = ki;
    float2 x0[16], x1[16];
    dif<32, true>(q);
    wave_sync_lds();
#pragma unroll
    for (int i = 0; i < 16; ++i) lds2[hi * kK2hSlab + cp * 16 + (i ^ cp)] = q[brev<32>(2 * i)];
    wave_sync_lds();
#pragma unroll
    for (int bp = 0; bp < 16; ++bp) x0[bp] = lds2[hi * kK2hSlab + bp * 16 + (cp ^ bp)];
    wave_sync_lds();
#pragma unroll
    for (int i = 0; i < 16; ++i) lds2[hi * kK2hSlab + cp * 16 + (i ^ cp)] = q[brev<32>(2 * i + 1)];
    twiddle_nat<16, true>(x0, ki.wc0, ki.qc0);
    dif<16, true>(x0);
    wave_sync_lds();
#pragma unroll
    for (int bp = 0; bp < 16; ++bp) x1[bp] = lds2[hi * kK2hSlab + bp * 16 + (cp ^ bp)];
    wave_sync_lds();
#pragma unroll
    for (int b = 0; b < 16; ++b) lds2[hi * kK2hSlab + b * 16 + cp] = x0[brev<16>(b)];
    if (LATE_J) {
        __builtin_amdgcn_sched_barrier(0);
        const float4 j = pl.k2j[2 * t], jq = pl.k2j[2 * t + 1];
        ki.wj0 = make_float2(j.x, j.y); ki.wj1 = make_float2(j.z, j.w);
        ki.qj0 = make_float2(jq.x, jq.y); ki.qj1 = make_float2(jq.z, jq.w);
        __builtin_amdgcn_sched_barrier(0);
    }
    twiddle_nat<16, true>(x1, ki.wc1, ki.qc1);
    dif<16, true>(x1);
    __syncthreads();
#pragma unroll
    for (int ap = 0; ap < 16; ++ap) x0[ap] = lds2[ap * kK2hSlab + t];
    __syncthreads();
#pragma unroll
    for (int b = 0; b < 16; ++b) lds2[hi * kK2hSlab + b * 16 + cp] = x1[brev<16>(b)];
    twiddle_nat<16, true>(x0, ki.wj0, ki.qj0);
    dif<16, true>(x0);
    __syncthreads();
#pragma unroll
    for (int ap = 0; ap < 16; ++ap) x1[ap] = lds2[ap * kK2hSlab + t];
    twiddle_nat<16, true>(x1, ki.wj1, ki.qj1);
    dif<16, true>(x1);
    if (HALF) {
#pragma unroll
        for (int a = 0; a < 16; ++a)
            buf_store_u2(rdst, k.voff / 2, a * 2048, make_uint2(pack_h2(x0[brev<16>(a)]), pack_h2(x1[brev<16>(a)])));
        return;
    }
#pragma unroll
    for (int a = 0; a < 16; ++a)
        buf_store4<SAUX>(rdst, k.voff, a * 4096, make_float4(x0[brev<16>(a)].x, x0[brev<16>(a)].y,
                                                           x1[brev<16>(a)].x, x1[brev<16>(a)].y));
}

template <bool HALF>
__device__ __forceinline__ void k2_rows_r16_planes_row(float2* __restrict__ work, const float2* __restrict__ hc, float2* __restrict__ dst,
                                                       const PlanDev& pl, unsigned npairs, float hscale) {
    extern __shared__ float4 lds4[];
    float2* lds2 = reinterpret_cast<float2*>(lds4);
    unsigned row, slot;
    k2_place(npairs, row, slot);
    const size_t row_off = ((size_t)slot << pl.logN) + (size_t)row * kN2;
    const __amdgpu_buffer_rsrc_t rrow = HALF ? make_rsrc(reinterpret_cast<unsigned*>(work) + row_off, kN2 * 4)
                                             : make_rsrc(work + row_off, kN2 * 8);
    const __amdgpu_buffer_rsrc_t rdst = !dst ? rrow
        : HALF ? make_rsrc(reinterpret_cast<unsigned*>(dst) + row_off, kN2 * 4) : make_rsrc(dst + row_off, kN2 * 8);
    const __amdgpu_buffer_rsrc_t rh = make_rsrc(reinterpret_cast<const float4*>(hc) + (size_t)row * (kN2 / 2), kN2 * 8);
    const K2Lane k = k2_lane(pl);
    float2 z[32];
    k2p_forward<HALF>(k, rrow, lds2, z);
    float4 ha[4], hb[4], hc4[4];
    __builtin_amdgcn_sched_barrier(0);
    k2_fetch_quarter(rh, k.voff, 0, ha);
    k2_fetch_quarter(rh, k.voff, 1, hb);
    __builtin_amdgcn_sched_barrier(0);
    dif<32, false>(z);
    __builtin_amdgcn_sched_barrier(0);
    k2_fetch_quarter(rh, k.voff, 2, hc4);
    __builtin_amdgcn_sched_barrier(0);
    auto scaled = [&](float4 (&h)[4]) {
        if (HALF) {
#pragma unroll
            for (int i = 0; i < 4; ++i) { h[i].x *= hscale; h[i].y *= hscale; h[i].z *= hscale; h[i].w *= hscale; }
        }
    };
    float2 q[32];
    scaled(ha);
    k2_multiply_quarter(z, ha, 0, q);
    k2_fetch_quarter(rh, k.voff, 3, ha);
    __builtin_amdgcn_sched_barrier(0);
    scaled(hb);
    k2_multiply_quarter(z, hb, 1, q);
    scaled(hc4);
    k2_multiply_quarter(z, hc4, 2, q);
    scaled(ha);
    k2_multiply_quarter(z, ha, 3, q);
    k2p_inverse<HALF>(pl, q, lds2, rdst);
}
template <bool HALF>
__global__ void __launch_bounds__(256, kK2pWaves)
k2_rows_r16_planes(float2* __restrict__ work, const float2* __restrict__ hc, float2* __restrict__ dst, PlanDev pl, unsigned npairs,
                   float hscale) {
    k2_rows_r16_planes_row<HALF>(work, hc, dst, pl, npairs, hscale);
}
template <bool HALF>
__global__ void __launch_bounds__(256, kK2pWaves)
tail_rows_r16_planes(float2* __restrict__ work, const float2* __restrict__ hc, float2* __restrict__ dst, PlanDev pl, unsigned npairs,
                     float hscale) {
    k2_rows_r16_planes_row<HALF>(work, hc, dst, pl, npairs, hscale);
}

constexpr int kK2gpWaves = 3;
constexpr int kK2gStoreAux = 2;
__global__ void __launch_bounds__(256, kK2gpWaves)
k2_rows_r16_group_planes(const float2* __restrict__ work, K2Group grp, PlanDev pl, unsigned npairs) {
    extern __shared__ float4 lds4[];
    float2* lds2 = reinterpret_cast<float2*>(lds4);
    unsigned row, slot;
    k2_place(npairs, row, slot);
    const size_t row_off = ((size_t)slot << pl.logN) + (size_t)row * kN2;
    const __amdgpu_buffer_rsrc_t rrow = make_rsrc(work + row_off, kN2 * 8);
    const size_t hoff4 = (size_t)row * (kN2 / 2);
    const K2Lane k = k2_lane(pl);
    float2 z[32];
    k2p_forward<false>(k, rrow, lds2, z);
    dif<32, false>(z);
#pragma unroll 1
    for (int j = 0; j < grp.n; ++j) {
        const __amdgpu_buffer_rsrc_t rh = make_rsrc(reinterpret_cast<const float4*>(grp.hc[j]) + hoff4, kN2 * 8);
        float4 hq[4];
        k2_fetch_quarter(rh, k.voff, 0, hq);
        float2 q[32];
        k2_multiply_fetch(z, rh, k.voff, hq, q);
        k2p_inverse<false, kK2gStoreAux, true>(pl, q, lds2, make_rsrc(grp.dst[j] + row_off, kN2 * 8));
        __syncthreads();
    }
}

__global__ void __launch_bounds__(256) spectrum_to_half_kernel(const float2* __restrict__ hc, long long n, float scale, unsigned* __restrict__ out) {
    for (long long i = (long long)blockIdx.x * 256 + threadIdx.x; i < n; i += (long long)gridDim.x * 256)
        out[i] = h2_bits(to_h2(make_float2(hc[i].x * scale, hc[i].y * scale)));
}
hipError_t launch_spectrum_to_half(hipStream_t st, const float2* hc, long long n, float scale, unsigned* out) {
    hipLaunchKernelGGL(spectrum_to_half_kernel, dim3(2048), dim3(256), 0, st, hc, n, scale, out);
    return hipGetLastError();
}

typedef _Float16 half8 __attribute__((ext_vector_type(8)));
typedef float f32x4v __attribute__((ext_vector_type(4)));
typedef unsigned u32x4v __attribute__((ext_vector_type(4)));
constexpr int kM16Ps1 = 516, kM16Ps4 = 520;
constexpr int kK2mLds = 16 * kM16Ps4 * 4;
constexpr int kMfA16 = 0, kMfA32 = 2 * 64 * 4, kMfT1 = kMfA32 + 8 * 64 * 4, kMfT2 = kMfT1 + 256 * 32, kMfTotal = kMfT2 + 256 * 8;

__device__ __forceinline__ half8 as_half8(const h2 (&v)[4]) {
    u32x4v u;
    u.x = h2_bits(v[0]); u.y = h2_bits(v[1]); u.z = h2_bits(v[2]); u.w = h2_bits(v[3]);
    return __builtin_bit_cast(half8, u);
}
__device__ __forceinline__ half8 load_half8(const unsigned* p) {
    const uint4 v = *reinterpret_cast<const uint4*>(p);
    u32x4v u; u.x = v.x; u.y = v.y; u.z = v.z; u.w = v.w;
    return __builtin_bit_cast(half8, u);
}
__device__ __forceinline__ void dft16_mfma(const half8& are, const half8& aim, const h2 (&b)[4], float2 (&y)[4]) {
    const half8 bv = as_half8(b);
    const f32x4v zero = {0.f, 0.f, 0.f, 0.f};
    const f32x4v dre = __builtin_amdgcn_mfma_f32_16x16x32_f16(are, bv, zero, 0, 0, 0);
    const f32x4v dim = __builtin_amdgcn_mfma_f32_16x16x32_f16(aim, bv, zero, 0, 0, 0);
    y[0] = make_float2(dre.x, dim.x); y[1] = make_float2(dre.y, dim.y);
    y[2] = make_float2(dre.z, dim.z); y[3] = make_float2(dre.w, dim.w);
}
__device__ __forceinline__ h2 cmul_conj_a(h2 a, h2 b) {
    const h2 t = a * b.xx;
    return __builtin_elementwise_fma(a.yx, b.yy, (h2){t.x, -t.y});
}
__device__ __forceinline__ int swap_bits02(int c) { return (c & ~5) | ((c & 1) << 2) | ((c >> 2) & 1); }

constexpr int kK2mWaves = 2;
__global__ void __launch_bounds__(256, kK2mWaves)
k2_rows_m16(unsigned* __restrict__ work, const unsigned* __restrict__ hcm, unsigned* __restrict__ dst, PlanDev pl, unsigned npairs,
            float pre) {
    extern __shared__ float4 lds4[];
    unsigned* lds = reinterpret_cast<unsigned*>(lds4);
    const int t = threadIdx.x, w = t >> 6, l = t & 63, n = l & 15, g = l >> 4;
    const half8 a16re = load_half8(pl.mf + kMfA16 + l * 4), a16im = load_half8(pl.mf + kMfA16 + 256 + l * 4);
    h2 tw1[4][2][4], tw2[2][4];
    {
        const uint4* p1 = reinterpret_cast<const uint4*>(pl.mf + kMfT1 + t * 32);
#pragma unroll
        for (int gl = 0; gl < 4; ++gl)
#pragma unroll
            for (int e = 0; e < 2; ++e) {
                const uint4 v = p1[gl * 2 + e];
                tw1[gl][e][0] = bits_h2(v.x); tw1[gl][e][1] = bits_h2(v.y); tw1[gl][e][2] = bits_h2(v.z); tw1[gl][e][3] = bits_h2(v.w);
            }
        const uint4* p2 = reinterpret_cast<const uint4*>(pl.mf + kMfT2 + t * 8);
#pragma unroll
        for (int ch = 0; ch < 2; ++ch) {
            const uint4 v = p2[ch];
            tw2[ch][0] = bits_h2(v.x); tw2[ch][1] = bits_h2(v.y); tw2[ch][2] = bits_h2(v.z); tw2[ch][3] = bits_h2(v.w);
        }
    }
    const h2 prescale = (h2){(_Float16)pre, (_Float16)pre};
    const int e1w = (4 * w) * kM16Ps1 + (4 * g) * 32 + 2 * n;
    const int e1r = (4 * g) * kM16Ps1 + (4 * w) * 32 + n;
    const int blk = (4 * w) * 512;
    const int e2w = blk + swap_bits02(n) * 16 + ((g ^ (n & 3)) * 4);
    const int e2r = blk + (g & 1) * 16 + (g >> 1) * 128 + (n & 3);
    const int e3w = blk + n * 32 + ((g ^ (n & 7)) * 4);
    const int e3r = blk + g * 128 + (n & 3);
    const int e4w = (4 * w) * kM16Ps4 + g * 128 + n;
    const int e4r = (4 * g) * kM16Ps4 + w * 128 + 2 * n;
    const unsigned voff = (unsigned)(((4 * g) * 512 + 128 * w + 2 * n) * 4);
    const unsigned xcd = blockIdx.x & 7u;
    const unsigned nseq = (npairs << pl.logN1) >> 3, sstep = gridDim.x >> 3;
    for (unsigned seq = blockIdx.x >> 3; seq < nseq; seq += sstep) {
        const unsigned row = (seq / npairs) * 8u + xcd, slot = seq % npairs;
        const size_t row_off = ((size_t)slot << pl.logN) + (size_t)row * kN2;
        const __amdgpu_buffer_rsrc_t rrow = make_rsrc(work + row_off, kN2 * 4);
        const __amdgpu_buffer_rsrc_t rdst = dst ? make_rsrc(dst + row_off, kN2 * 4) : rrow;
        uint2 raw[4][4];
#pragma unroll
        for (int gl = 0; gl < 4; ++gl)
#pragma unroll
            for (int r = 0; r < 4; ++r) raw[gl][r] = buf_load_u2(rrow, voff, (unsigned)((r * 512 + 32 * gl) * 4));
#pragma unroll
        for (int gl = 0; gl < 4; ++gl) {
            h2 b0[4], b1[4];
#pragma unroll
            for (int r = 0; r < 4; ++r) { b0[r] = bits_h2(raw[gl][r].x) * prescale; b1[r] = bits_h2(raw[gl][r].y) * prescale; }
            float2 y0[4], y1[4];
            dft16_mfma(a16re, a16im, b0, y0);
            dft16_mfma(a16re, a16im, b1, y1);
#pragma unroll
            for (int r = 0; r < 4; ++r) {
                const h2 v0 = cmul(to_h2(y0[r]), tw1[gl][0][r]), v1 = cmul(to_h2(y1[r]), tw1[gl][1][r]);
                *reinterpret_cast<uint2*>(lds + e1w + gl * kM16Ps1 + r * 32) = make_uint2(h2_bits(v0), h2_bits(v1));
            }
        }
        __syncthreads();
        h2 bb[4][2][4];
#pragma unroll
        for (int q = 0; q < 4; ++q)
#pragma unroll
            for (int ch = 0; ch < 2; ++ch)
#pragma unroll
                for (int r = 0; r < 4; ++r) bb[q][ch][r] = bits_h2(lds[e1r + r * kM16Ps1 + q * 32 + 16 * ch]);
        __syncthreads();
#pragma unroll
        for (int q = 0; q < 4; ++q)
#pragma unroll
            for (int ch = 0; ch < 2; ++ch) {
                float2 y[4];
                dft16_mfma(a16re, a16im, bb[q][ch], y);
                uint4 o;
                o.x = h2_bits(cmul(to_h2(y[0]), tw2[ch][0])); o.y = h2_bits(cmul(to_h2(y[1]), tw2[ch][1]));
                o.z = h2_bits(cmul(to_h2(y[2]), tw2[ch][2])); o.w = h2_bits(cmul(to_h2(y[3]), tw2[ch][3]));
                *reinterpret_cast<uint4*>(lds + e2w + q * 512 + 256 * ch) = o;
            }
        wave_sync_lds();
        {
// ... 76 lines not shown
                dft16_mfma(a16re, a16im, bt, y);
#pragma unroll
                for (int r = 0; r < 4; ++r) lds[e4w + q * kM16Ps4 + r * 32 + 16 * ch] = h2_bits(to_h2(y[r]));
            }
        __syncthreads();
#pragma unroll
        for (int gl = 0; gl < 4; ++gl)
#pragma unroll
            for (int r = 0; r < 4; ++r) raw[gl][r] = *reinterpret_cast<const uint2*>(lds + e4r + r * kM16Ps4 + gl * 32);
        __syncthreads();
#pragma unroll
        for (int gl = 0; gl < 4; ++gl) {
            h2 b0[4], b1[4];
#pragma unroll
            for (int r = 0; r < 4; ++r) { b0[r] = cmul(bits_h2(raw[gl][r].x), tw1[gl][0][r]); b1[r] = cmul(bits_h2(raw[gl][r].y), tw1[gl][1][r]); }
            float2 y0[4], y1[4];
            dft16_mfma(a16re, a16im, b0, y0);
            dft16_mfma(a16re, a16im, b1, y1);
#pragma unroll
            for (int r = 0; r < 4; ++r)
                buf_store_u2(rdst, voff, (unsigned)((r * 512 + 32 * gl) * 4),
                             make_uint2(h2_bits(to_h2(make_float2(y0[r].x, -y0[r].y))), h2_bits(to_h2(make_float2(y1[r].x, -y1[r].y)))));
        }
    }
}

__global__ void __launch_bounds__(256) spectrum_to_half_mfma_kernel(const float2* __restrict__ hc, long long n, float scale, unsigned* __restrict__ out) {
    for (long long o = (long long)blockIdx.x * 256 + threadIdx.x; o < n; o += (long long)gridDim.x * 256) {
        const long long row = o >> kR16LogN2;
        const int within = (int)(o & (kN2 - 1)), tt = within >> 5, cp = within & 31;
        const int rr = brev<32>(cp), i = rr >> 1, e = rr & 1;
        const float2 v = hc[row * kN2 + 2 * tt + 512 * i + e];
        out[o] = h2_bits(to_h2(make_float2(v.x * scale, -v.y * scale)));
    }
}
hipError_t launch_spectrum_to_half_mfma(hipStream_t st, const float2* hc, long long n, float scale, unsigned* out) {
    hipLaunchKernelGGL(spectrum_to_half_mfma_kernel, dim3(2048), dim3(256), 0, st, hc, n, scale, out);
    return hipGetLastError();
}

__device__ __forceinline__ float min3_raw(float a, float b, float c) {
    float r;
    asm("v_min3_f32 %0, %1, %2, %3" : "=v"(r) : "v"(a), "v"(b), "v"(c));
    return r;
}
__device__ __forceinline__ float max3_raw(float a, float b, float c) {
    float r;
    asm("v_max3_f32 %0, %1, %2, %3" : "=v"(r) : "v"(a), "v"(b), "v"(c));
    return r;
}

__device__ __forceinline__ float wave_min_f(float v) {
    asm("s_nop 1\n\tv_min_f32_dpp %0, %0, %0 row_shr:1 row_mask:0xf bank_mask:0xf\n\t"
        "s_nop 1\n\tv_min_f32_dpp %0, %0, %0 row_shr:2 row_mask:0xf bank_mask:0xf\n\t"
        "s_nop 1\n\tv_min_f32_dpp %0, %0, %0 row_shr:4 row_mask:0xf bank_mask:0xf\n\t"
        "s_nop 1\n\tv_min_f32_dpp %0, %0, %0 row_shr:8 row_mask:0xf bank_mask:0xf\n\t"
        "s_nop 1\n\tv_min_f32_dpp %0, %0, %0 row_bcast:15 row_mask:0xa bank_mask:0xf\n\t"
        "s_nop 1\n\tv_min_f32_dpp %0, %0, %0 row_bcast:31 row_mask:0xc bank_mask:0xf\n\t"
        "s_nop 1"
        : "+v"(v));
    return __int_as_float(__builtin_amdgcn_readlane(__float_as_int(v), 63));
}

template <int HB>
__device__ __forceinline__ unsigned scan_swizzle(unsigned row) { return (((row >> HB) & 3u) << 1) | ((row & 3u) >> 1); }
template <int HB>
__device__ __forceinline__ int scan_row_of(int t) { return ((t & 63) >> 2) * (1 << HB) + (t >> 6) * 4 + (t & 3); }
template <int HB>
__device__ __forceinline__ void scan_put(float2* lds2, int hi, int cp, const float (&c0)[16], const float (&c1)[16]) {
    const unsigned half = (unsigned)cp & 1u, chunk = (unsigned)cp >> 1, hb = ((unsigned)hi & 3u) >> 1;
#pragma unroll
    for (int a = 0; a < 16; ++a) {
        const unsigned pos = chunk ^ ((((unsigned)a & 3u) << 1) | hb);
        lds2[a * (16 << HB) + hi * 16 + (int)((pos << 1) | half)] = make_float2(c0[a], c1[a]);
    }
}
template <int HB>
__device__ __forceinline__ void scan_row_minmax(const float4* lds4, int row, bool whole, int nvalid, float& mn, float& mx) {
    const unsigned k = scan_swizzle<HB>((unsigned)row);
    float4 v[8];
#pragma unroll
    for (int i = 0; i < 8; ++i) v[i] = lds4[row * 8 + (int)((unsigned)i ^ k)];
    if (!whole) {
        mn = FLT_MAX; mx = -FLT_MAX;
#pragma unroll
        for (int i = 0; i < 8; ++i) {
            const int c0 = i << 2;
            const float e[4] = {v[i].x, v[i].y, v[i].z, v[i].w};
#pragma unroll
            for (int j = 0; j < 4; ++j)
                if (c0 + j < nvalid) { mn = fminf(mn, e[j]); mx = fmaxf(mx, e[j]); }
        }
        return;
    }
    mn = min3_raw(v[0].x, v[0].y, v[0].z); mx = max3_raw(v[0].x, v[0].y, v[0].z);
    mn = min3_raw(mn, v[0].w, v[1].x);     mx = max3_raw(mx, v[0].w, v[1].x);
#pragma unroll
    for (int i = 1; i < 8; ++i) {
        if (i > 1) { mn = min3_raw(mn, v[i - 1].w, v[i].x); mx = max3_raw(mx, v[i - 1].w, v[i].x); }
        mn = min3_raw(mn, v[i].y, v[i].z); mx = max3_raw(mx, v[i].y, v[i].z);
    }
    mn = fminf(mn, v[7].w); mx = fmaxf(mx, v[7].w);
}

__device__ __forceinline__ long long mod_recip(long long x, long long c, double inv_c) {
    long long q = (long long)((double)x * inv_c);
    long long r = x - q * c;
    if (r < 0) r += c;
    else if (r >= c) r -= c;
    return r;
}
__device__ __forceinline__ bool run_has_chunk_edge(long long lo, long long c, long long d, double inv_c) {
    if (c <= 0) return true;
    if (mod_recip(lo + 31, c, inv_c) <= 31) return true;
    const long long hi2 = lo + 31 - d;
    if (hi2 < 0) return false;
    return mod_recip(hi2, c, inv_c) <= 31;
}

struct K3Edges {
    long long outA, outB;
    int relcA, reldA, relcB, reldB;
    bool one_edge;
};
__device__ __forceinline__ K3Edges k3_edges(const Job& job, const ScanCfg& scan, long long blkA, long long blkB) {
    K3Edges e;
    e.outA = blkA * job.hop; e.outB = blkB * job.hop;
    e.one_edge = scan.stats32 != nullptr && scan.seg_c >= (long long)job.hop + 32;
    e.relcA = e.reldA = e.relcB = e.reldB = 0x7fffffff;
    if (scan.edges_n > 0) {
        const int s = (int)(blkA >> 1) - job.first_pair;
        e.relcA = scan.edge_rel[s][0]; e.reldA = scan.edge_rel[s][1];
        e.relcB = scan.edge_rel[s][2]; e.reldB = scan.edge_rel[s][3];
        return e;
    }
    if (e.one_edge) {
        const long long c = scan.seg_c, d = scan.seg_d;
        const long long m = mod_recip(e.outA, c, scan.inv_c);
        const long long ecA = m == 0 ? e.outA : e.outA + (c - m);
        long long edA = d;
        if (e.outA > d) {
            const long long m2 = mod_recip(e.outA - d, c, scan.inv_c);
            edA = m2 == 0 ? e.outA : e.outA + (c - m2);
        }
        const long long ecB = ecA >= e.outB ? ecA : ecA + c;
        const long long edB = edA >= e.outB ? edA : edA + c;
        auto rel = [](long long edge, long long start) { const long long r = edge - start; return r < 0x7fffffffll ? (int)r : 0x7fffffff; };
        e.relcA = rel(ecA, e.outA); e.reldA = rel(edA, e.outA);
        e.relcB = rel(ecB, e.outB); e.reldB = rel(edB, e.outB);
    }
    return e;
}

template <int HB, bool ACC = false, bool SCALED = false>
__device__ __forceinline__ void k3_finish(const Job& job, const ScanCfg& scan, const K3Edges& ed, float2* lds2,
                                          int n2_0, int out_stride, int t, long long blkA, long long blkB,
                                          float out_scale, const float2 (&x0)[16], const float2 (&x1)[16]) {
    const int hi = t >> 4, cp = t & 15;
    const long long col = n2_0 + 2 * cp;
    const long long outA = ed.outA, outB = ed.outB;
    const bool one_edge = ed.one_edge;
    const bool dst8 = ((reinterpret_cast<uintptr_t>(job.dst) & 7) == 0) && ((job.hop & 1) == 0);
    long long limA = job.out_count - outA; if (limA > job.hop) limA = job.hop;
    long long limB = blkB < job.nblocks ? job.out_count - outB : 0; if (limB > job.hop) limB = job.hop;
    float sa0[16], sa1[16], sb0[16], sb1[16];
#pragma unroll
    for (int a = 0; a < 16; ++a) {
        const float2 v0 = x0[brev<16>(a)], v1 = x1[brev<16>(a)];
        if (SCALED) {
            sa0[a] = v0.x; sa1[a] = v1.x;
            sb0[a] = v0.y; sb1[a] = v1.y;
        } else {
            sa0[a] = v0.x * out_scale; sa1[a] = v1.x * out_scale;
            sb0[a] = v0.y * out_scale; sb1[a] = v1.y * out_scale;
        }
    }
    unsigned wantA[2] = {0x11111111u, 0x11111111u}, wantB[2] = {0x11111111u, 0x11111111u};
    if (!ACC && scan.stats32 != nullptr) {
        const int row = scan_row_of<HB>(t);
        const int rowrun = row * out_stride + n2_0;
        const int leftA = (int)limA - rowrun, leftB = (int)limB - rowrun;
        const bool wholeA = leftA >= 32 || leftA <= 0, wholeB = leftB >= 32 || leftB <= 0;
        const float4* lds4 = reinterpret_cast<const float4*>(lds2);
        float rmnA, rmxA, rmnB, rmxB;
        __syncthreads();
        scan_put<HB>(lds2, hi, cp, sa0, sa1);
        wave_sync_lds();
        scan_row_minmax<HB>(lds4, row, wholeA, leftA < 32 ? leftA : 32, rmnA, rmxA);
        wave_sync_lds();
        scan_put<HB>(lds2, hi, cp, sb0, sb1);
        wave_sync_lds();
        scan_row_minmax<HB>(lds4, row, wholeB, leftB < 32 ? leftB : 32, rmnB, rmxB);
        float tminA = wave_min_f(leftA > 0 ? rmnA : FLT_MAX), tminB = wave_min_f(leftB > 0 ? rmnB : FLT_MAX);
        float* slots = reinterpret_cast<float*>(lds2 + scan_row_of<HB>(t & ~63) * 16);
        wave_sync_lds();
        if ((t & 63) == 0) { slots[0] = tminA; slots[1] = tminB; }
        __syncthreads();
#pragma unroll
        for (int w = 0; w < (1 << (HB - 2)); ++w) {
            const float* v = reinterpret_cast<const float*>(lds2 + scan_row_of<HB>(w * 64) * 16);
            tminA = fminf(tminA, v[0]);
            tminB = fminf(tminB, v[1]);
        }
        const bool dense = scan.margin < 0.0f;
        const float thA = dense ? -FLT_MAX : fminf(fminf(tminA, tminB), scan.hist_min) + scan.margin, thB = thA;
        bool edgeA, edgeB;
        if (one_edge) {
            edgeA = leftA > 0 && ((unsigned)(ed.relcA - rowrun) <= 31u || (unsigned)(ed.reldA - rowrun) <= 31u);
            edgeB = leftB > 0 && ((unsigned)(ed.relcB - rowrun) <= 31u || (unsigned)(ed.reldB - rowrun) <= 31u);
        } else {
            edgeA = leftA > 0 && run_has_chunk_edge(outA + rowrun, scan.seg_c, scan.seg_d, scan.inv_c);
            edgeB = leftB > 0 && run_has_chunk_edge(outB + rowrun, scan.seg_c, scan.seg_d, scan.inv_c);
        }
        const bool pa = (leftA > 0 && rmxA >= thA) || edgeA, pb = (leftB > 0 && rmxB >= thB) || edgeB;
        const unsigned long long ba = __ballot(pa), bb = __ballot(pb);
        const unsigned sh = (unsigned)hi & 3u;
        wantA[0] = ((unsigned)ba >> sh) & 0x11111111u; wantA[1] = ((unsigned)(ba >> 32) >> sh) & 0x11111111u;
        wantB[0] = ((unsigned)bb >> sh) & 0x11111111u; wantB[1] = ((unsigned)(bb >> 32) >> sh) & 0x11111111u;
        const long long tileA = blkA * (out_stride >> kColsLog) + ((unsigned)n2_0 >> kColsLog), tileB = tileA + (out_stride >> kColsLog);
        if (t == 0 && scan.tile_theta != nullptr) {
            scan.tile_theta[tileA] = thA;
            if (blkB < job.nblocks) scan.tile_theta[tileB] = thB;
        }
        if ((t & 63) == 0 && scan.wbits != nullptr) {
            scan.wbits[(tileA << (HB - 2)) + (t >> 6)] = ba;
            if (blkB < job.nblocks) scan.wbits[(tileB << (HB - 2)) + (t >> 6)] = bb;
        }
        if (leftA > 0) scan.stats32[(outA + rowrun) >> 5] = make_float2(rmnA, rmxA);
        if (leftB > 0) scan.stats32[(outB + rowrun) >> 5] = make_float2(rmnB, rmxB);
    }
    if (wantA[0] | wantA[1]) {
#pragma unroll
        for (int a = 0; a < 16; ++a) {
            if (!((wantA[a >> 3] >> ((a & 7) * 4)) & 1u)) continue;
            const long long n = (long long)(a * (1 << HB) + hi) * out_stride + col;
            if (dst8 && n + 1 < limA) {
                float2* ptr = reinterpret_cast<float2*>(job.dst + outA + n);
                float2 v = make_float2(sa0[a], sa1[a]);
                if (ACC) { const float2 o = *ptr; v.x += o.x; v.y += o.y; }
                *ptr = v;
            } else {
                if (n < limA) job.dst[outA + n] = sa0[a] + (ACC ? job.dst[outA + n] : 0.0f);
                if (n + 1 < limA) job.dst[outA + n + 1] = sa1[a] + (ACC ? job.dst[outA + n + 1] : 0.0f);
            }
            if (ACC && (a & 3) == 3) __builtin_amdgcn_sched_barrier(0);
        }
    }
    if (wantB[0] | wantB[1]) {
#pragma unroll
        for (int a = 0; a < 16; ++a) {
            if (!((wantB[a >> 3] >> ((a & 7) * 4)) & 1u)) continue;
            const long long n = (long long)(a * (1 << HB) + hi) * out_stride + col;
            if (dst8 && n + 1 < limB) {
                float2* ptr = reinterpret_cast<float2*>(job.dst + outB + n);
                float2 v = make_float2(sb0[a], sb1[a]);
                if (ACC) { const float2 o = *ptr; v.x += o.x; v.y += o.y; }
                *ptr = v;
            } else {
                if (n < limB) job.dst[outB + n] = sb0[a] + (ACC ? job.dst[outB + n] : 0.0f);
                if (n + 1 < limB) job.dst[outB + n + 1] = sb1[a] + (ACC ? job.dst[outB + n + 1] : 0.0f);
            }
            if (ACC && (a & 3) == 3) __builtin_amdgcn_sched_barrier(0);
        }
    }
}


template <bool ACC = false>
__device__ __forceinline__ void k3_tile(const Job& job, const PlanDev& pl, const ScanCfg& scan, float2* lds2,
                                        int n2_0, int out_stride, int t, long long blkA, long long blkB,
                                        float out_scale, float2 (&x0)[16], float2 (&x1)[16], const ScanCfg* geo = nullptr) {
    const int hi = t >> 4, cp = t & 15;
    const long long N = 1ll << pl.logN;
    const long long col = n2_0 + 2 * cp;
    const K3Edges ed = k3_edges(job, geo ? *geo : scan, blkA, blkB);
    const unsigned maskN = (unsigned)(N - 1);
    const float2 w256 = pl.tw1[hi], w256q = pl.tw1[4 * hi];
    {
        const unsigned n2 = (unsigned)col;
        float2 base0 = tw_big(pl, (n2 * (unsigned)hi) & maskN);
        float2 base1 = tw_big(pl, ((n2 + 1) * (unsigned)hi) & maskN);
        base0.x *= out_scale; base0.y *= out_scale;
        base1.x *= out_scale; base1.y *= out_scale;
        float2 step0, step1, step0q, step1q;
        tw_big_pair(pl, (n2 * 16u) & maskN, step0, step0q);
        tw_big_pair(pl, ((n2 + 1) * 16u) & maskN, step1, step1q);
        twiddle_chain<16, true, false>(x0, base0, step0, step0q);
        dif<16, true>(x0);
#pragma unroll
        for (int b = 0; b < 16; ++b) lds2[(hi * 16 + b) * 16 + cp] = x0[brev<16>(b)];
        twiddle_chain<16, true, false>(x1, base1, step1, step1q);
    }
    dif<16, true>(x1);
    __syncthreads();
#pragma unroll
    for (int ap = 0; ap < 16; ++ap) x0[ap] = lds2[(ap * 16 + hi) * 16 + cp];
    __syncthreads();
#pragma unroll
    for (int b = 0; b < 16; ++b) lds2[(hi * 16 + b) * 16 + cp] = x1[brev<16>(b)];
    twiddle_nat<16, true>(x0, w256, w256q);
    dif<16, true>(x0);
    __syncthreads();
#pragma unroll
    for (int ap = 0; ap < 16; ++ap) x1[ap] = lds2[(ap * 16 + hi) * 16 + cp];
    twiddle_nat<16, true>(x1, w256, w256q);
    dif<16, true>(x1);
    k3_finish<4, ACC, true>(job, scan, ed, lds2, n2_0, out_stride, t, blkA, blkB, out_scale, x0, x1);
}

__device__ __forceinline__ void k3_tile_h16(const Job& job, const PlanDev& pl, const ScanCfg& scan, float2* lds2,
                                            int n2_0, int out_stride, int t, long long blkA, long long blkB,
                                            float out_scale, h2 (&hx0)[16], h2 (&hx1)[16]) {
    const int hi = t >> 4, cp = t & 15;
    const long long N = 1ll << pl.logN;
    const long long col = n2_0 + 2 * cp;
    const K3Edges ed = k3_edges(job, scan, blkA, blkB);
    const unsigned maskN = (unsigned)(N - 1);
    const float2 w256 = pl.tw1[hi];
    {
        const unsigned n2 = (unsigned)col;
        const float2 base0 = tw_big(pl, (n2 * (unsigned)hi) & maskN);
        const float2 base1 = tw_big(pl, ((n2 + 1) * (unsigned)hi) & maskN);
        const float2 step0 = tw_big(pl, (n2 * 16u) & maskN);
        const float2 step1 = tw_big(pl, ((n2 + 1) * 16u) & maskN);
        twiddle_chain<16, true, false>(hx0, base0, step0);
        twiddle_chain<16, true, false>(hx1, base1, step1);
    }
    dif<16, true>(hx0);
    dif<16, true>(hx1);
    uint2* ldsu = reinterpret_cast<uint2*>(lds2);
#pragma unroll
    for (int b = 0; b < 16; ++b) ldsu[(hi * 16 + b) * 16 + cp] = make_uint2(h2_bits(hx0[brev<16>(b)]), h2_bits(hx1[brev<16>(b)]));
    __syncthreads();
    float2 x0[16], x1[16];
#pragma unroll
    for (int ap = 0; ap < 16; ++ap) {
        const uint2 v = ldsu[(ap * 16 + hi) * 16 + cp];
        x0[ap] = to_f2(bits_h2(v.x));
        x1[ap] = to_f2(bits_h2(v.y));
    }
    twiddle_nat<16, true>(x0, w256);
    twiddle_nat<16, true>(x1, w256);
    dif<16, true>(x0);
    dif<16, true>(x1);
    k3_finish<4>(job, scan, ed, lds2, n2_0, out_stride, t, blkA, blkB, out_scale, x0, x1);
}

constexpr int kK3Waves = 3;
constexpr int kK3LoadAux = 2, kK3hLoadAux = 2;
template <int HALF, bool ACC>
__device__ __forceinline__ void k3_cols_inv_r16_tile(unsigned lin, float4* lds4, const Job& job, const float2* __restrict__ work,
                                                     const PlanDev& pl, float out_scale, const ScanCfg& scan, const ScanCfg* geo = nullptr) {
    const int t = threadIdx.x;
    const int hi = t >> 4, cp = t & 15;
    const unsigned xcd = lin & 7u, seq = lin >> 3;
    const unsigned slot = seq >> 5, half = (seq >> 4) & 1u, tl = seq & 15u;
    const int n2_0 = (int)(((half * 8u + xcd) * 16u + tl) << kColsLog);
    const int pair = job.first_pair + (int)slot;
    if (scan.only_pairs != nullptr && scan.only_pairs[pair] == 0) return;
    const long long blkA = 2ll * pair, blkB = blkA + 1;
    if constexpr (HALF == 2) {
        const uint2* __restrict__ in2 = reinterpret_cast<const uint2*>(reinterpret_cast<const unsigned*>(work) + ((size_t)slot << pl.logN) + n2_0) + cp;
        h2 hx0[16], hx1[16];
#pragma unroll
        for (int bp = 0; bp < 16; ++bp) {
            const uint2 v = in2[(size_t)(hi + 16 * bp) * (kN2 / 2)];
            hx0[bp] = bits_h2(v.x);
            hx1[bp] = bits_h2(v.y);
        }
        k3_tile_h16(job, pl, scan, reinterpret_cast<float2*>(lds4), n2_0, kN2, t, blkA, blkB, out_scale, hx0, hx1);
        return;
    }
    float2 x0[16], x1[16];
    if (HALF) {
        const uint2* __restrict__ in2 = reinterpret_cast<const uint2*>(reinterpret_cast<const unsigned*>(work) + ((size_t)slot << pl.logN) + n2_0) + cp;
#pragma unroll
        for (int bp = 0; bp < 16; ++bp) {
            const uint2 v = in2[(size_t)(hi + 16 * bp) * (kN2 / 2)];
            x0[bp] = unpack_h2(v.x);
            x1[bp] = unpack_h2(v.y);
        }
    } else {
        const __amdgpu_buffer_rsrc_t rin = make_rsrc(work + ((size_t)slot << pl.logN) + n2_0, (unsigned)((((size_t)1 << pl.logN) - n2_0) * 8));
        const unsigned voff = (unsigned)hi * (kN2 * 8u) + (unsigned)cp * 16u;
#pragma unroll
        for (int bp = 0; bp < 16; ++bp) {
            const float4 v = buf_load4<kK3LoadAux>(rin, voff, (unsigned)bp * (16u * kN2 * 8u));
            x0[bp] = make_float2(v.x, v.y);
            x1[bp] = make_float2(v.z, v.w);
        }
    }
    k3_tile<ACC>(job, pl, scan, reinterpret_cast<float2*>(lds4), n2_0, kN2, t, blkA, blkB, out_scale, x0, x1, geo);
}
template <int HALF, bool ACC = false, int REDO = 0>
__global__ void __launch_bounds__(256, REDO ? 4 : kK3Waves)
k3_cols_inv_r16(Job job, const float2* __restrict__ work, PlanDev pl, float out_scale, ScanCfg scan) {
    extern __shared__ float4 lds4[];
    if constexpr (REDO != 0) {
        for (unsigned lin = blockIdx.x; lin < (unsigned)scan.redo_tiles; lin += gridDim.x) {
            k3_cols_inv_r16_tile<HALF, ACC>(lin, lds4, job, work, pl, out_scale, scan);
            __syncthreads();
        }
    } else {
        k3_cols_inv_r16_tile<HALF, ACC>(blockIdx.x, lds4, job, work, pl, out_scale, scan);
    }
}

__global__ void __launch_bounds__(256, kK3Waves)
k3_cols_inv_r16_group(Job job, PlanDev pl, ScanCfg scan, K3Group grp) {
    extern __shared__ float4 lds4[];
    const unsigned z = blockIdx.y;
    job.dst = grp.dst[z]; job.out_count = grp.out_count[z];
    ScanCfg mine;
    mine.stats32 = grp.stats32[z]; mine.wbits = grp.wbits[z]; mine.tile_theta = grp.tile_theta[z]; mine.hist_min = grp.hist_min[z];
    mine.margin = scan.margin; mine.seg_c = grp.seg_c; mine.seg_d = grp.seg_d[z]; mine.inv_c = grp.inv_c;
    mine.only_pairs = nullptr; mine.redo_tiles = 0; mine.edges_n = 0;
    k3_cols_inv_r16_tile<0, false>(blockIdx.x, lds4, job, grp.work[z], pl, grp.out_scale[z], mine, &scan);
}

template <int HALF>
__global__ void __launch_bounds__(256, kK3Waves)
tail_cols_inv_r16(TailBatch tb, int hop, const float2* __restrict__ work, PlanDev pl, float out_scale) {
    extern __shared__ float4 lds4[];
    const unsigned z = blockIdx.y;
    Job job;
    job.src = nullptr; job.src_len = 0; job.lead = 0; job.dst = tb.dst[z]; job.out_count = tb.out_count[z];
    job.hop = hop; job.nblocks = (int)((tb.out_count[z] + hop - 1) / hop); job.first_pair = 0; job.src_kind = 0;
    ScanCfg mine;
    mine.stats32 = tb.stats32[z]; mine.wbits = nullptr; mine.tile_theta = nullptr; mine.margin = -1.0f; mine.hist_min = FLT_MAX;
    mine.seg_c = 0; mine.seg_d = 0; mine.inv_c = 0.0; mine.only_pairs = nullptr; mine.redo_tiles = 0; mine.edges_n = 0;
    const float2* mywork = HALF ? reinterpret_cast<const float2*>(reinterpret_cast<const unsigned*>(work) + ((size_t)z << pl.logN))
                                : work + ((size_t)z << pl.logN);
    k3_cols_inv_r16_tile<HALF, false>(blockIdx.x, lds4, job, mywork, pl, out_scale, mine);
}

__global__ void __launch_bounds__(256)
tail_commit_kernel(const float* __restrict__ tsc, float* __restrict__ sc, long long n, const float2* __restrict__ tst, float2* __restrict__ st32,
                   unsigned long long* __restrict__ wbits, long long words, float* __restrict__ theta, int tiles) {
    const long long tid = (long long)blockIdx.x * blockDim.x + threadIdx.x, nth = (long long)gridDim.x * blockDim.x;
    const long long n4 = n >> 2;
    const float4* __restrict__ t4 = reinterpret_cast<const float4*>(tsc);
    float4* __restrict__ s4 = reinterpret_cast<float4*>(sc);
    for (long long i = tid; i < n4; i += nth) s4[i] = t4[i];
    for (long long i = (n4 << 2) + tid; i < n; i += nth) sc[i] = tsc[i];
    const long long n32 = (n + 31) >> 5;
    for (long long i = tid; i < n32; i += nth) st32[i] = tst[i];
    if (wbits != nullptr)
        for (long long i = tid; i < words; i += nth) wbits[i] = ~0ull;
    if (theta != nullptr)
        for (long long i = tid; i < tiles; i += nth) theta[i] = -FLT_MAX;
}

__global__ void __launch_bounds__(256)
tail_preset_group_kernel(K3Group grp, long long blk, int log_n1, int log_n2) {
    const unsigned z = blockIdx.y;
    const long long tiles = 1ll << (log_n2 - kColsLog), words = tiles << (log_n1 - 6);
    const long long tid = (long long)blockIdx.x * blockDim.x + threadIdx.x, nth = (long long)gridDim.x * blockDim.x;
    unsigned long long* __restrict__ wb = grp.wbits[z] + blk * words;
    float* __restrict__ th = grp.tile_theta[z] + blk * tiles;
    for (long long i = tid; i < words; i += nth) wb[i] = ~0ull;
    for (long long i = tid; i < tiles; i += nth) th[i] = -FLT_MAX;
}

constexpr int kC512Slab = 560;
__device__ __forceinline__ int c512_idx(int ap, int b, int cp) { return ap * kC512Slab + b * 17 + cp; }
constexpr int kC512Lds = (15 * kC512Slab + 31 * 17 + 16) * 8;
static_assert(kC512Lds >= 512 * 16 * 8, "K3's score scan needs 512 rows x 32 scores");
constexpr int kC512Slab3 = 32 * 16 + 16;
__device__ __forceinline__ int c512_idx3(int ap, int b, int cp) { return ap * kC512Slab3 + b * 16 + cp; }
static_assert((15 * kC512Slab3 + 31 * 16 + 16) * 8 <= kC512Lds, "K3's exchange fits the kernel's LDS");

template <int KIND, int HALF, int LN2 = kR16LogN2>
__global__ void __launch_bounds__(512, 4)
k1_cols_fwd_c512(Job job, float2* __restrict__ work, PlanDev pl) {
    constexpr int kN2 = 1 << LN2;
    extern __shared__ float4 lds4[];
    float2* lds2 = reinterpret_cast<float2*>(lds4);
    const int t = threadIdx.x;
    const int hi = t >> 4, cp = t & 15;
    const int ap = hi & 15, half = hi >> 4;
    const int k10 = ap + 16 * half;
    const int n2_0 = blockIdx.x << kColsLog;
    const int pair = job.first_pair + blockIdx.y;
    const long long blkA = 2ll * pair, blkB = blkA + 1;
    const bool validB = blkB < job.nblocks;
    const long long N = 1ll << pl.logN;
    const long long baseA = blkA * job.hop - job.lead;
    const long long baseB = blkB * job.hop - job.lead;
    const bool fast = ((reinterpret_cast<uintptr_t>(job.src) & 7) == 0) && ((baseA & 1) == 0) && ((baseB & 1) == 0) &&
                      baseA >= 0 && baseA + N <= job.src_len && validB && baseB + N <= job.src_len;
    const long long col = (long long)n2_0 + 2 * cp;
    const unsigned maskN = (unsigned)(N - 1);
    const float2 w512 = pl.tw1[hi];
    const float2 w512q = pl.tw1[4 * hi];
    const float2 base0 = tw_big(pl, ((unsigned)col * (unsigned)k10) & maskN);
    const float2 base1 = tw_big(pl, (((unsigned)col + 1u) * (unsigned)k10) & maskN);
    float2 step0, step1, step0q, step1q;
    if constexpr (HALF == 2) {
        step0 = tw_big(pl, ((unsigned)col * 32u) & maskN);
        step1 = tw_big(pl, (((unsigned)col + 1u) * 32u) & maskN);
    }
    float2 x0[16], x1[16];
    if (fast && KIND == 1) {
        const __amdgpu_buffer_rsrc_t rsrc = make_rsrc(static_cast<const char*>(job.src) + 4 * baseA, (unsigned)(4 * (N + job.hop)));
        const unsigned voff = 4u * ((unsigned)hi * kN2 + (unsigned)col), offB = 4u * (unsigned)job.hop;
#pragma unroll
        for (int a = 0; a < 16; ++a) {
            const float2 va = decode_sample2<KIND>(buf_load_u2<kK1LoadNt ? 2 : 0>(rsrc, voff, (unsigned)a * (4u * 32u * kN2)));
            const float2 vb = decode_sample2<KIND>(buf_load_u2<kK1LoadNt ? 2 : 0>(rsrc, voff, (unsigned)a * (4u * 32u * kN2) + offB));
            x0[a] = make_float2(va.x, vb.x);
            x1[a] = make_float2(va.y, vb.y);
        }
    } else if (fast) {
#pragma unroll
        for (int a = 0; a < 16; ++a) {
            const long long off = (long long)(a * 32 + hi) * kN2 + col;
            const float2 va = load_sample2<KIND>(job.src, baseA + off), vb = load_sample2<KIND>(job.src, baseB + off);
            x0[a] = make_float2(va.x, vb.x);
            x1[a] = make_float2(va.y, vb.y);
        }
    } else {
#pragma unroll
        for (int a = 0; a < 16; ++a) {
            const long long n = (long long)(a * 32 + hi) * kN2 + col;
            const float2 va = load2_padded<KIND>(job.src, baseA + n, job.src_len);
            const float2 vb = validB ? load2_padded<KIND>(job.src, baseB + n, job.src_len) : make_float2(0.f, 0.f);
            x0[a] = make_float2(va.x, vb.x);
            x1[a] = make_float2(va.y, vb.y);
        }
    }
    if constexpr (HALF == 2) {
        h2 hx0[16], hx1[16];
#pragma unroll
        for (int a = 0; a < 16; ++a) { hx0[a] = to_h2(x0[a]); hx1[a] = to_h2(x1[a]); }
        dif<16, false>(hx0);
        dif<16, false>(hx1);
        twiddle_apply2<16, false, true>(hx0, hx1, w512);
        uint2* ldsu = reinterpret_cast<uint2*>(lds4);
#pragma unroll
        for (int a2 = 0; a2 < 16; ++a2) ldsu[c512_idx(a2, hi, cp)] = make_uint2(h2_bits(hx0[brev<16>(a2)]), h2_bits(hx1[brev<16>(a2)]));
        __syncthreads();
#pragma unroll
        for (int b = 0; b < 16; ++b) {
            const uint2 lo = ldsu[c512_idx(ap, b, cp)], up = ldsu[c512_idx(ap, b + 16, cp)];
            hx0[b] = half ? mul_w32<false>(csub(bits_h2(lo.x), bits_h2(up.x)), b) : cadd(bits_h2(lo.x), bits_h2(up.x));
            hx1[b] = half ? mul_w32<false>(csub(bits_h2(lo.y), bits_h2(up.y)), b) : cadd(bits_h2(lo.y), bits_h2(up.y));
        }
        dif<16, false>(hx0);
        dif<16, false>(hx1);
        twiddle_chain<16, false, true>(hx0, base0, step0);
        twiddle_chain<16, false, true>(hx1, base1, step1);
        uint2* __restrict__ out2 = reinterpret_cast<uint2*>(reinterpret_cast<unsigned*>(work) + ((size_t)blockIdx.y << pl.logN) + n2_0) + cp;
#pragma unroll
        for (int bt = 0; bt < 16; ++bt) {
            const size_t k1 = (size_t)(k10 + 32 * bt);
            out2[k1 * (kN2 / 2)] = make_uint2(h2_bits(hx0[brev<16>(bt)]), h2_bits(hx1[brev<16>(bt)]));
        }
        return;
    }
    dif<16, false>(x0);
    dif<16, false>(x1);
    twiddle_brev<16, false>(x0, w512, w512q);
    twiddle_brev<16, false>(x1, w512, w512q);
    float2 y0[16], y1[16];
#pragma unroll
    for (int a2 = 0; a2 < 16; ++a2) lds2[c512_idx(a2, hi, cp)] = x0[brev<16>(a2)];
    __syncthreads();
#pragma unroll
    for (int b = 0; b < 16; ++b) {
        const float2 lo = lds2[c512_idx(ap, b, cp)], up = lds2[c512_idx(ap, b + 16, cp)];
        y0[b] = half ? mul_w32<false>(csub(lo, up), b) : cadd(lo, up);
    }
    __syncthreads();
#pragma unroll
    for (int a2 = 0; a2 < 16; ++a2) lds2[c512_idx(a2, hi, cp)] = x1[brev<16>(a2)];
    __syncthreads();
#pragma unroll
    for (int b = 0; b < 16; ++b) {
        const float2 lo = lds2[c512_idx(ap, b, cp)], up = lds2[c512_idx(ap, b + 16, cp)];
        y1[b] = half ? mul_w32<false>(csub(lo, up), b) : cadd(lo, up);
    }
    __builtin_amdgcn_sched_barrier(0);
    tw_big_pair(pl, ((unsigned)col * 32u) & maskN, step0, step0q);
    tw_big_pair(pl, (((unsigned)col + 1u) * 32u) & maskN, step1, step1q);
    __builtin_amdgcn_sched_barrier(0);
    dif<16, false>(y0);
// ... 473 lines not shown
    const long long blkA = 2ll * pair, blkB = blkA + 1;
    const bool validB = blkB < job.nblocks;
    const long long baseA = blkA * job.hop - job.lead;
    const long long baseB = blkB * job.hop - job.lead;
    const int total = N1 << BL;
    for (int idx = tid; idx < total; idx += nthr) {
        const int r = idx >> BL, c = idx & ((1 << BL) - 1);
        const long long n = (long long)r * N2 + n2_0 + c;
        const float a = load_padded<KIND>(job.src, baseA + n, job.src_len);
        const float b = validB ? load_padded<KIND>(job.src, baseB + n, job.src_len) : 0.0f;
        s[idx] = make_float2(a, b);
    }
    __syncthreads();
    lds_fft_fwd<BL>(s, pl.logN1, pl.tw1, tid, nthr);
    float2* out = work + ((size_t)blockIdx.y << pl.logN) + n2_0;
    const unsigned maskN = (1u << pl.logN) - 1u;
    for (int idx = tid; idx < total; idx += nthr) {
        const int p = idx >> BL, c = idx & ((1 << BL) - 1);
        const unsigned k1 = __brev((unsigned)p) >> (32 - pl.logN1);
        const float2 w = tw_big(pl, ((unsigned)(n2_0 + c) * k1) & maskN);
        out[(size_t)p * N2 + c] = cmul(s[idx], w);
    }
}

template <bool SPECTRUM>
__global__ void __launch_bounds__(kFftThreads)
k2_rows_gen(float2* __restrict__ work, const float2* __restrict__ hc, float2* __restrict__ hc_out, PlanDev pl) {
    extern __shared__ float2 s[];
    const int N2 = 1 << pl.logN2;
    const int tid = threadIdx.x, nthr = blockDim.x;
    const int p = blockIdx.x;
    float2* row = work + ((size_t)blockIdx.y << pl.logN) + (size_t)p * N2;
    for (int n2 = tid; n2 < N2; n2 += nthr) s[n2] = row[n2];
    __syncthreads();
    lds_fft_fwd<0>(s, pl.logN2, pl.tw2, tid, nthr);
    const size_t hoff = (size_t)p * N2;
    if (SPECTRUM) {
        const float invN = 1.0f / (float)(1u << pl.logN);
        for (int q = tid; q < N2; q += nthr) {
            const float2 v = s[q];
            hc_out[hoff + q] = make_float2(v.x * invN, -v.y * invN);
        }
        return;
    }
    for (int q = tid; q < N2; q += nthr) s[q] = cmul(s[q], hc[hoff + q]);
    __syncthreads();
    lds_fft_inv<0>(s, pl.logN2, pl.tw2, tid, nthr);
    float2* orow = hc_out ? hc_out + ((size_t)blockIdx.y << pl.logN) + (size_t)p * N2 : row;
    for (int n2 = tid; n2 < N2; n2 += nthr) orow[n2] = s[n2];
}

template <int BL>
__global__ void __launch_bounds__(kFftThreads)
k3_cols_inv_gen(Job job, const float2* __restrict__ work, PlanDev pl, float out_scale, int acc) {
    extern __shared__ float2 s[];
    const int N1 = 1 << pl.logN1, N2 = 1 << pl.logN2;
    const int tid = threadIdx.x, nthr = blockDim.x;
    const int n2_0 = blockIdx.x << BL;
    const int pair = job.first_pair + blockIdx.y;
    const long long blkA = 2ll * pair, blkB = blkA + 1;
    const bool validB = blkB < job.nblocks;
    const int total = N1 << BL;
    const float2* in = work + ((size_t)blockIdx.y << pl.logN) + n2_0;
    const unsigned maskN = (1u << pl.logN) - 1u;
    for (int idx = tid; idx < total; idx += nthr) {
        const int p = idx >> BL, c = idx & ((1 << BL) - 1);
        const unsigned k1 = __brev((unsigned)p) >> (32 - pl.logN1);
        const float2 w = tw_big(pl, ((unsigned)(n2_0 + c) * k1) & maskN);
        s[idx] = cmulc(in[(size_t)p * N2 + c], w);
    }
    __syncthreads();
    lds_fft_inv<BL>(s, pl.logN1, pl.tw1, tid, nthr);
    const long long outA = blkA * job.hop, outB = blkB * job.hop;
    for (int idx = tid; idx < total; idx += nthr) {
        const int r = idx >> BL, c = idx & ((1 << BL) - 1);
        const long long n = (long long)r * N2 + n2_0 + c;
        if (n >= job.hop) continue;
        const float2 v = s[idx];
        if (outA + n < job.out_count) job.dst[outA + n] = v.x * out_scale + (acc ? job.dst[outA + n] : 0.0f);
        if (validB && outB + n < job.out_count) job.dst[outB + n] = v.y * out_scale + (acc ? job.dst[outB + n] : 0.0f);
    }
}

template <int KIND>
__global__ void __launch_bounds__(256)
correlate_direct(Job job, const float* __restrict__ needle, int s, float out_scale) {
    __shared__ float nd[kDirectMaxNeedle];
    if ((int)threadIdx.x < s) nd[threadIdx.x] = needle[threadIdx.x];
    __syncthreads();
    for (long long j = (long long)blockIdx.x * 256 + threadIdx.x; j < job.out_count; j += (long long)gridDim.x * 256) {
        float acc = 0.0f;
        for (int n = 0; n < s; ++n) acc = fmaf(load_padded<KIND>(job.src, j + n - job.lead, job.src_len), nd[n], acc);
        job.dst[j] = acc * out_scale;
    }
}

hipError_t launch_direct(hipStream_t st, const Job& job, const float* needle, int s, float out_scale) {
    if (s < 1 || s > kDirectMaxNeedle || job.out_count <= 0) return hipErrorInvalidValue;
    long long blocks = (job.out_count + 255) / 256;
    if (blocks > 4096) blocks = 4096;
    if (job.src_kind == 1) hipLaunchKernelGGL(correlate_direct<1>, dim3((unsigned)blocks), dim3(256), 0, st, job, needle, s, out_scale);
    else hipLaunchKernelGGL(correlate_direct<0>, dim3((unsigned)blocks), dim3(256), 0, st, job, needle, s, out_scale);
    return hipGetLastError();
}

template <typename Fn>
struct Variant { Fn fn; int threads; int lds; };

template <typename Fn, typename... Args>
static hipError_t launch_row_lds(const Variant<Fn>& v, dim3 grid, size_t lds, hipStream_t st, const Args&... args) {
    if (v.fn == nullptr) return hipErrorInvalidValue;
    hipLaunchKernelGGL(v.fn, grid, dim3(v.threads), lds, st, args...);
    return hipGetLastError();
}
template <typename Fn, typename... Args>
static hipError_t launch_row(const Variant<Fn>& v, dim3 grid, hipStream_t st, const Args&... args) {
    return launch_row_lds(v, grid, (size_t)v.lds, st, args...);
}

bool plan_is_r16(const PlanDev& pl) { return pl.logN1 == kR16LogN1 && pl.logN2 == kR16LogN2; }
bool plan_is_c512(const PlanDev& pl) { return pl.logN1 == 9 && pl.logN2 == kR16LogN2; }
bool plan_is_c1024(const PlanDev& pl) { return pl.logN1 == 10 && pl.logN2 == kR16LogN2; }
bool plan_is_c512w(const PlanDev& pl) { return pl.logN1 == 9 && pl.logN2 == 14; }
bool plan_has_scan(const PlanDev& pl) { return plan_is_r16(pl) || plan_is_c512(pl) || plan_is_c1024(pl); }
bool plan_k2_is_r16(const PlanDev& pl) { return pl.logN2 == kR16LogN2 && pl.logN1 >= 3; }

enum ColPlan { kColR16, kColC512, kColC1024, kColC512w, kColGen, kColPlans };
static ColPlan col_plan(const PlanDev& pl) {
    return plan_is_r16(pl) ? kColR16 : plan_is_c512(pl) ? kColC512 : plan_is_c1024(pl) ? kColC1024 : plan_is_c512w(pl) ? kColC512w : kColGen;
}
static int half_level(int half) { return half == 2 ? 2 : half ? 1 : 0; }

static constexpr int kMaxLds = 160 * 1024;
static constexpr int kR16Lds = 64 * 1024;
static constexpr int kR16LdsK1 = 256 * 17 * 8;
static constexpr int kR16LdsK3 = 256 * 16 * 8;

using K1Fn = void (*)(Job, float2*, PlanDev);
static constexpr Variant<K1Fn> kK1[kColPlans][2][3] = {
     {{{k1_cols_fwd_r16<0, 0>, 256, kR16LdsK1}, {k1_cols_fwd_r16<0, 1>, 256, kR16LdsK1}, {k1_cols_fwd_r16<0, 2>, 256, kR16LdsK1}},
                 {{k1_cols_fwd_r16<1, 0>, 256, kR16LdsK1}, {k1_cols_fwd_r16<1, 1>, 256, kR16LdsK1}, {k1_cols_fwd_r16<1, 2>, 256, kR16LdsK1}}},
     {{{k1_cols_fwd_c512<0, 0>, 512, kC512Lds}, {k1_cols_fwd_c512<0, 1>, 512, kC512Lds}, {k1_cols_fwd_c512<0, 2>, 512, kC512Lds}},
                 {{k1_cols_fwd_c512<1, 0>, 512, kC512Lds}, {k1_cols_fwd_c512<1, 1>, 512, kC512Lds}, {k1_cols_fwd_c512<1, 2>, 512, kC512Lds}}},
     {{{k1_cols_fwd_c1024<0>, 1024, kC1024Lds}}, {{k1_cols_fwd_c1024<1>, 1024, kC1024Lds}}},
     {{{k1_cols_fwd_c512<0, 0, 14>, 512, kC512Lds}}},
     {{{k1_cols_fwd_gen<kColsLog, 0>, kFftThreads, kMaxLds}}, {{k1_cols_fwd_gen<kColsLog, 1>, kFftThreads, kMaxLds}}},
};
using TailK1Fn = void (*)(TailBatch, int, float2*, PlanDev);
static constexpr Variant<TailK1Fn> kTailK1[2][3] = {
    {{tail_cols_fwd_r16<0, 0>, 256, kR16LdsK1}, {tail_cols_fwd_r16<0, 1>, 256, kR16LdsK1}, {tail_cols_fwd_r16<0, 2>, 256, kR16LdsK1}},
    {{tail_cols_fwd_r16<1, 0>, 256, kR16LdsK1}, {tail_cols_fwd_r16<1, 1>, 256, kR16LdsK1}, {tail_cols_fwd_r16<1, 2>, 256, kR16LdsK1}},
};

using K2Fn = void (*)(float2*, const float2*, float2*, PlanDev, unsigned, float);
static constexpr Variant<K2Fn> kK2[2][2] = {
    {{k2_rows_r16_planes<false>, 256, kK2hLds}, {tail_rows_r16_planes<false>, 256, kK2hLds}},
    {{k2_rows_r16_planes<true>, 256, kK2hLds}, {tail_rows_r16_planes<true>, 256, kK2hLds}},
};
static constexpr Variant<K2Fn> kK2Spectrum = {k2_rows_r16_spectrum, 256, kR16Lds};
using K2hFn = void (*)(unsigned*, const unsigned*, unsigned*, PlanDev, unsigned, float);
static constexpr Variant<K2hFn> kK2h[2] = {{k2_rows_h16, 256, kK2hLds}, {tail_rows_h16, 256, kK2hLds}};
static constexpr Variant<K2hFn> kK2Mfma = {k2_rows_m16, 256, kK2mLds};
using K2GroupFn = void (*)(const float2*, K2Group, PlanDev, unsigned);
static constexpr Variant<K2GroupFn> kK2Group = {k2_rows_r16_group_planes, 256, kK2hLds};
using K2GenFn = void (*)(float2*, const float2*, float2*, PlanDev);
static constexpr Variant<K2GenFn> kK2Gen[2] = {{k2_rows_gen<false>, kFftThreads, kMaxLds}, {k2_rows_gen<true>, kFftThreads, kMaxLds}};

enum K3Form { kK3Plain, kK3Acc, kK3Redo, kK3Forms };
using K3Fn = void (*)(Job, const float2*, PlanDev, float, ScanCfg);
static constexpr Variant<K3Fn> kK3[kColGen][3][kK3Forms] = {
     {{{k3_cols_inv_r16<0>, 256, kR16LdsK3}, {}, {k3_cols_inv_r16<0, false, 1>, 256, kR16LdsK3}},
                 {{k3_cols_inv_r16<1>, 256, kR16LdsK3}, {}, {k3_cols_inv_r16<1, false, 1>, 256, kR16LdsK3}},
                 {{k3_cols_inv_r16<2>, 256, kR16LdsK3}, {}, {k3_cols_inv_r16<2, false, 1>, 256, kR16LdsK3}}},
     {{{k3_cols_inv_c512<0>, 512, kC512Lds}, {k3_cols_inv_c512<0, true>, 512, kC512Lds}, {k3_cols_inv_c512<0, false, 1>, 512, kC512Lds}},
                 {{k3_cols_inv_c512<1>, 512, kC512Lds}, {}, {k3_cols_inv_c512<1, false, 1>, 512, kC512Lds}},
                 {{k3_cols_inv_c512<2>, 512, kC512Lds}, {}, {k3_cols_inv_c512<2, false, 1>, 512, kC512Lds}}},
     {{{k3_cols_inv_c1024<false>, 1024, kC1024Lds}, {k3_cols_inv_c1024<true>, 1024, kC1024Lds}, {k3_cols_inv_c1024<false, 1>, 1024, kC1024Lds}}},
     {{{k3_cols_inv_c512w, 512, kC512Lds}}},
};
using K3GenFn = void (*)(Job, const float2*, PlanDev, float, int);
static constexpr Variant<K3GenFn> kK3Gen = {k3_cols_inv_gen<kColsLog>, kFftThreads, kMaxLds};
using K3GroupFn = void (*)(Job, PlanDev, ScanCfg, K3Group);
static constexpr Variant<K3GroupFn> kK3Group[kColGen] = {{k3_cols_inv_r16_group, 256, kR16LdsK3}, {k3_cols_inv_c512_group, 512, kC512Lds}};
using TailK3Fn = void (*)(TailBatch, int, const float2*, PlanDev, float);
static constexpr Variant<TailK3Fn> kTailK3[3] = {
    {tail_cols_inv_r16<0>, 256, kR16LdsK3}, {tail_cols_inv_r16<1>, 256, kR16LdsK3}, {tail_cols_inv_r16<2>, 256, kR16LdsK3}};

template <typename Fn>
static hipError_t allow_lds(const Variant<Fn>& v) {
    return v.fn == nullptr ? hipSuccess : hipFuncSetAttribute((const void*)v.fn, hipFuncAttributeMaxDynamicSharedMemorySize, v.lds);
}
template <typename T, size_t N>
static hipError_t allow_lds(const T (&table)[N]) {
    for (const T& t : table) {
        const hipError_t e = allow_lds(t);
        if (e != hipSuccess) return e;
    }
    return hipSuccess;
}
hipError_t fft_kernels_init() {
    hipError_t e = allow_lds(kK1);
    if (e == hipSuccess) e = allow_lds(kTailK1);
    if (e == hipSuccess) e = allow_lds(kK2);
    if (e == hipSuccess) e = allow_lds(kK2Spectrum);
    if (e == hipSuccess) e = allow_lds(kK2h);
    if (e == hipSuccess) e = allow_lds(kK2Mfma);
    if (e == hipSuccess) e = allow_lds(kK2Group);
    if (e == hipSuccess) e = allow_lds(kK2Gen);
    if (e == hipSuccess) e = allow_lds(kK3);
    if (e == hipSuccess) e = allow_lds(kK3Gen);
    if (e == hipSuccess) e = allow_lds(kK3Group);
    if (e == hipSuccess) e = allow_lds(kTailK3);
    return e;
}

hipError_t launch_k1(hipStream_t st, const Job& job, int npairs, float2* work, const PlanDev& pl, int half) {
    const dim3 grid((1u << pl.logN2) >> kColsLog, npairs);
    const ColPlan p = col_plan(pl);
    const int kind = job.src_kind == 1 ? 1 : 0;
    if (p == kColGen) return launch_row_lds(kK1[p][kind][0], grid, (sizeof(float2) << pl.logN1) << kColsLog, st, job, work, pl);
    return launch_row(kK1[p][kind][half_level(half)], grid, st, job, work, pl);
}

static int k2_mfma_initial() { const char* e = getenv("AM_K2_MFMA"); return e && atoi(e) ? 1 : 0; }
static std::atomic<int> g_k2_mfma{k2_mfma_initial()};
void set_k2_mfma(int on) { g_k2_mfma.store(on ? 1 : 0, std::memory_order_relaxed); }
bool k2_mfma_enabled() { return g_k2_mfma.load(std::memory_order_relaxed) != 0; }
int k2_mfma_table_dwords() { return kMfTotal; }

hipError_t launch_k2(hipStream_t st, int npairs, float2* work, const float2* hc, const PlanDev& pl, float2* dst,
                     int half, float hscale, float pre, bool tail) {
    if (!plan_k2_is_r16(pl))
        return launch_row_lds(kK2Gen[0], dim3(1u << pl.logN1, npairs), sizeof(float2) << pl.logN2, st, work, hc, dst, pl);
    const unsigned rows = (unsigned)npairs << pl.logN1;
    if (half == 2) {
        unsigned* const w = reinterpret_cast<unsigned*>(work);
        const unsigned* const h = reinterpret_cast<const unsigned*>(hc);
        unsigned* const d = reinterpret_cast<unsigned*>(dst);
        if (!tail && k2_mfma_enabled() && pl.mf != nullptr) {
            const unsigned grid = std::min<unsigned>(rows, 256u * 4u) & ~7u;
            return launch_row(kK2Mfma, dim3(grid ? grid : 8u), st, w, h, d, pl, (unsigned)npairs, pre);
        }
        return launch_row(kK2h[tail], dim3(rows), st, w, h, d, pl, (unsigned)npairs, pre);
    }
    return launch_row(kK2[half ? 1 : 0][tail], dim3(rows), st, work, hc, dst, pl, (unsigned)npairs, half ? hscale : 1.0f);
}

bool plan_k2_has_group(const PlanDev& pl) { return plan_k2_is_r16(pl); }

hipError_t launch_k2_group(hipStream_t st, int npairs, const float2* work, const K2Group& grp, const PlanDev& pl) {
    if (!plan_k2_has_group(pl) || grp.n < 1 || grp.n > kMaxNeedleGroup) return hipErrorInvalidValue;
    return launch_row(kK2Group, dim3((unsigned)npairs << pl.logN1), st, work, grp, pl, (unsigned)npairs);
}

hipError_t launch_k2_spectrum(hipStream_t st, float2* work, float2* hc_out, const PlanDev& pl) {
    if (plan_k2_is_r16(pl)) return launch_row(kK2Spectrum, dim3(1u << pl.logN1), st, work, (const float2*)nullptr, hc_out, pl, 1u, 1.0f);
    return launch_row_lds(kK2Gen[1], dim3(1u << pl.logN1, 1), sizeof(float2) << pl.logN2, st, work, (const float2*)nullptr, hc_out, pl);
}

static void fill_edges(const Job& job, int npairs, ScanCfg& scan) {
    scan.edges_n = 0;
    const long long c = scan.seg_c, d = scan.seg_d, hop = job.hop;
    if (scan.stats32 == nullptr || npairs > ScanCfg::kMaxEdgeSlots || c < hop + 32) return;
    auto rel = [](long long edge, long long start) { const long long r = edge - start; return r < 0x7fffffffll ? (int)r : 0x7fffffff; };
    for (int s = 0; s < npairs; ++s) {
        const long long outA = 2ll * (job.first_pair + s) * hop, outB = outA + hop;
        const long long m = outA % c;
        const long long ecA = m == 0 ? outA : outA + (c - m);
        long long edA = d;
        if (outA > d) {
            const long long m2 = (outA - d) % c;
            edA = m2 == 0 ? outA : outA + (c - m2);
        }
        const long long ecB = ecA >= outB ? ecA : ecA + c, edB = edA >= outB ? edA : edA + c;
        scan.edge_rel[s][0] = rel(ecA, outA); scan.edge_rel[s][1] = rel(edA, outA);
        scan.edge_rel[s][2] = rel(ecB, outB); scan.edge_rel[s][3] = rel(edB, outB);
    }
    scan.edges_n = npairs;
}

bool plan_k3_has_group(const PlanDev& pl) { return plan_is_c512(pl) || plan_is_r16(pl); }

hipError_t launch_tail_batch_k1(hipStream_t st, const TailBatch& tb, int hop, int src_kind, float2* work, const PlanDev& pl, int half) {
    if (!plan_is_r16(pl) || tb.n < 1 || tb.n > kMaxTailBatch) return hipErrorInvalidValue;
    const dim3 grid((1u << pl.logN2) >> kColsLog, (unsigned)tb.n);
    return launch_row(kTailK1[src_kind == 1 ? 1 : 0][half_level(half)], grid, st, tb, hop, work, pl);
}
hipError_t launch_tail_batch_k3(hipStream_t st, const TailBatch& tb, int hop, const float2* work, const PlanDev& pl, float out_scale, int half) {
    if (!plan_is_r16(pl) || tb.n < 1 || tb.n > kMaxTailBatch) return hipErrorInvalidValue;
    return launch_row(kTailK3[half_level(half)], dim3(kN2 >> kColsLog, (unsigned)tb.n), st, tb, hop, work, pl, out_scale);
}
hipError_t launch_tail_preset_group(hipStream_t st, const K3Group& grp, long long blk, int log_n1, int log_n2) {
    if (grp.n < 1 || grp.n > kMaxNeedleGroup) return hipErrorInvalidValue;
    for (int z = 0; z < grp.n; ++z) if (!grp.wbits[z] || !grp.tile_theta[z]) return hipErrorInvalidValue;
    hipLaunchKernelGGL(tail_preset_group_kernel, dim3(8, (unsigned)grp.n), dim3(256), 0, st, grp, blk, log_n1, log_n2);
    return hipGetLastError();
}
hipError_t launch_tail_commit(hipStream_t st, const float* tail_scores, float* scores, long long n, const float2* tail_stats32, float2* stats32,
                              unsigned long long* wbits, long long words, float* theta, int tiles) {
    const unsigned grid = (unsigned)std::min<long long>(512, std::max<long long>(1, (n / 4 + 255) / 256));
    hipLaunchKernelGGL(tail_commit_kernel, dim3(grid), dim3(256), 0, st, tail_scores, scores, n, tail_stats32, stats32, wbits, words, theta, tiles);
    return hipGetLastError();
}

hipError_t launch_k3_group(hipStream_t st, const Job& job, int npairs, const K3Group& grp, const PlanDev& pl, const ScanCfg& scan_in) {
    if (!plan_k3_has_group(pl) || grp.n < 1 || grp.n > kMaxNeedleGroup || scan_in.stats32 == nullptr) return hipErrorInvalidValue;
    for (int z = 0; z < grp.n; ++z) if (grp.out_count[z] > job.out_count) return hipErrorInvalidValue;
    ScanCfg scan = scan_in;
    scan.only_pairs = nullptr;
    fill_edges(job, npairs, scan);
    const dim3 grid((unsigned)npairs * (kN2 >> kColsLog), (unsigned)grp.n);
    return launch_row(kK3Group[col_plan(pl)], grid, st, job, pl, scan, grp);
}

hipError_t launch_k3(hipStream_t st, const Job& job, int npairs, const float2* work,
                     const PlanDev& pl, float out_scale, const ScanCfg& scan_in, int half, bool accumulate) {
    ScanCfg scan = scan_in;
    fill_edges(job, npairs, scan);
    const ColPlan p = col_plan(pl);
    if (p == kColGen) {
        if (accumulate && half) return hipErrorInvalidValue;
        const dim3 grid((1u << pl.logN2) >> kColsLog, npairs);
        return launch_row_lds(kK3Gen, grid, (sizeof(float2) << pl.logN1) << kColsLog, st, job, work, pl, out_scale, accumulate ? 1 : 0);
    }
    K3Form form = accumulate ? kK3Acc : kK3Plain;
    unsigned grid = (unsigned)npairs * ((1u << pl.logN2) >> kColsLog);
    if (scan.only_pairs != nullptr && !accumulate) {
        if (!plan_has_scan(pl)) return hipErrorInvalidValue;
        form = kK3Redo;
        scan.redo_tiles = (int)grid;
        const unsigned per_cu = p == kColC1024 ? 1u : p == kColC512 ? 2u : 4u;
        grid = std::min<unsigned>(grid, 256u * per_cu);
    }
    return launch_row(kK3[p][half_level(half)][form], dim3(grid), st, job, work, pl, out_scale, scan);
}

}
```

audio-matcher_amd/csrc/am_internal.h:

```cpp
#pragma once
#include <algorithm>
#include <atomic>
#include <cfloat>
#include <cmath>
#include <cstdio>
#include <cstring>
#include <map>
#include <mutex>
#include <string>
#include <vector>

#include "am_kernels.h"
#include "am_spans.h"

namespace am {

extern thread_local std::string t_err;
int fail(int code, const std::string& msg);
int hip_fail(hipError_t e, const char* what);
#define AM_HIP(call)                                         \
    do {                                                     \
        hipError_t e_ = (call);                              \
        if (e_ != hipSuccess) return hip_fail(e_, #call);    \
    } while (0)

struct Hooks {
    am_progress_fn fn = nullptr;
    void* user = nullptr;
    am_chunk_progress_fn chunk_fn = nullptr;
    void* chunk_user = nullptr;
};
Hooks snapshot_hooks();

struct Opts {
    long long log_n, pairs_per_group, half, batch_overlap, needle_group, dense, device_redo, debug_no_realloc, debug_redo_arm_at;
    long long peak_filter_order, distance_rule, tail_window, surrounding_from, k3_group, pick_group, tail_block, host_pick_wait;
    long long profile_mask, profile_every, pick_priority;
    long long score_norm, score_norm_floor_db;
    long long trace_form;
    PeakPolicy peak_policy() const { return PeakPolicy{(int)peak_filter_order, (int)(distance_rule & 1), (int)((distance_rule >> 1) & 1)}; }
};
static const float kHalfGain = 1024.0f;
static const double kMinEfficiency = 0.75;
static const int kLogNMin = 10, kLogNMax = 23;
static const long long kWideFromSamples = 140000;
static const long long kWidestFromSamples = 1500000;
static const long long kSegmentFrom = 1ll << 22;
static const long long kSegmentLen = 1ll << 22;

extern thread_local int t_no_realloc;
struct QueueingScope {
    bool on;
    explicit QueueingScope(bool enable) : on(enable) { if (on) ++t_no_realloc; }
    ~QueueingScope() { end(); }
    void end() { if (on) { --t_no_realloc; on = false; } }
    QueueingScope(const QueueingScope&) = delete;
    QueueingScope& operator=(const QueueingScope&) = delete;
};
int realloc_refused(const char* what, size_t bytes, size_t cap);

struct DevBuf {
    void* p = nullptr;
    size_t cap = 0;
    int ensure(size_t bytes) {
        if (bytes <= cap) return AM_OK;
        if (t_no_realloc > 0) return realloc_refused("a device", bytes, cap);
        release();
        size_t want = bytes + bytes / 8;
        hipError_t e = hipMalloc(&p, want);
        if (e != hipSuccess) {
            e = hipMalloc(&p, bytes);
            want = bytes;
            if (e != hipSuccess) { p = nullptr; return hip_fail(e, "hipMalloc(scratch)"); }
        }
        cap = want;
        return AM_OK;
    }
    void release() {
        if (p) (void)hipFree(p);
        p = nullptr; cap = 0;
    }
};
struct HostBuf {
    void* p = nullptr;
    size_t cap = 0;
    unsigned flags = hipHostMallocDefault;
    int ensure(size_t bytes) {
        if (bytes <= cap) return AM_OK;
        if (t_no_realloc > 0) return realloc_refused("a pinned host", bytes, cap);
        release();
        hipError_t e = hipHostMalloc(&p, bytes, flags);
        if (e != hipSuccess) { p = nullptr; return hip_fail(e, "hipHostMalloc"); }
        cap = bytes;
        return AM_OK;
    }
    void release() {
        if (p) (void)hipHostFree(p);
        p = nullptr; cap = 0;
    }
};

struct Plan {
    PlanDev dev{};
    float2* tables = nullptr;
    unsigned* mf = nullptr;
};

struct ScoreSide { DevBuf scores, stats, stats32, wflags, peaks, work; };

struct ProfRec { int name; hipEvent_t e0, e1; };
enum { KN_K1 = 0, KN_K2, KN_K3, KN_STATS, KN_PEAKS, KN_OTHER, KN_TRACE, KN_DISCOVER, KN_COUNT };

struct Ctx {
    int device = -1;
    hipStream_t stream = nullptr;
    hipStream_t stream2 = nullptr;
    hipStream_t stream_tail = nullptr;
    hipEvent_t ev_fork = nullptr, ev_join = nullptr;
    DevBuf work_tail, tail_scores, tail_stats;
    DevBuf work_tail2;
    std::recursive_mutex mu;
    std::map<int, Plan> plans;
    ScoreSide side[2];
    DevBuf work2, segs, io_in, io_out, sum, arena_cur, wide_ctl, wide_list, wide_tiles;
    DevBuf norm_blk;
    DevBuf hit_tab, hit_parts, hit_flags, hit_out, hit_stage;
    HostBuf hit_io;
    std::map<int, DevBuf> band_tabs;
    DevBuf warp_tab, warp_needles;
    DevBuf sig_span, sig_scores, sig_psum, sig_pmax, sig_mean, sig_hmax;
    std::map<std::pair<int, int>, DevBuf> rs_taps;
    DevBuf lag_parts, lag_r;
    DevBuf redo_pairs[2];
    DevBuf grp_scores[2][kMaxNeedleGroup], grp_stats32[2][kMaxNeedleGroup], grp_wflags[2][kMaxNeedleGroup];
    DevBuf grp_stats[kMaxNeedleGroup];
    HostBuf failcnt;
    hipEvent_t ev_k3[2] = {nullptr, nullptr}, ev_pick[2] = {nullptr, nullptr};
    HostBuf pinned;
    HostBuf hdr;
    HostBuf spill;
    HostBuf badflag;
    DevBuf ranges, range_flags;
    DevBuf big;
    DevBuf best_stats, best_lmax, best_ctl, best_trans, best_list, best_scores, best_mono;
    DevBuf trace_out, trace_parts;
    DevBuf disc_a, disc_probe, disc_energy, disc_parts, disc_out;
    std::vector<Segment> segs_resident;
    bool prof = false;
    std::vector<ProfRec> pending;
    std::vector<hipEvent_t> pool;
    double prof_ms[KN_COUNT] = {0};
    uint64_t prof_n[KN_COUNT] = {0};
    uint64_t prof_seq[KN_COUNT] = {0};
};

#ifndef AM_EVENT_NO_SYSTEM_FENCE
#define AM_EVENT_NO_SYSTEM_FENCE 1
#endif
constexpr unsigned kSyncEvent = hipEventDisableTiming | (AM_EVENT_NO_SYSTEM_FENCE ? hipEventDisableSystemFence : 0u);

int get_ctx(int device, Ctx** out);
struct ProfScope {
    Ctx* c; int name; hipStream_t st; hipEvent_t e0 = nullptr, e1 = nullptr;
    bool on;
    ProfScope(Ctx* c_, int name_, hipStream_t st_ = nullptr);
    ~ProfScope() {
        if (on) { (void)hipEventRecord(e1, st); c->pending.push_back({name, e0, e1}); }
    }
};
hipError_t copy_on_stream(Ctx* c, void* dst, const void* src, size_t bytes, hipMemcpyKind kind);
int get_plan(Ctx* c, int logN, const Plan** out, int force_logN1 = 0);

}

struct am_needle {
    am::Ctx* ctx = nullptr;
    float* d_needle = nullptr;
    size_t n = 0;
    float inv_autocorr = 0.f;
    double energy = 0.0;
    std::map<int, float2*> spectra;
    std::map<int, unsigned*> spectra16;
    std::map<int, unsigned*> spectra16m;
    static constexpr int kRecent = 8;
    float recent_min[2][kRecent];
    int recent_n[2] = {0, 0}, recent_pos[2] = {0, 0};
    void remember_min(int sm, float v) {
        recent_min[sm][recent_pos[sm]] = v;
        recent_pos[sm] = (recent_pos[sm] + 1) % kRecent;
        if (recent_n[sm] < kRecent) ++recent_n[sm];
    }
    int conservative_left[2] = {0, 0};
    int redo_armed_left[2] = {0, 0};
    float hist_min(int sm) const {
        float m = FLT_MAX;
        for (int i = 0; i < recent_n[sm]; ++i) m = std::min(m, recent_min[sm][i]);
        return m;
    }
    long long opt_log_n = -1, opt_half = -1, opt_score_norm = -1;
    std::vector<am_needle*> segments;
    std::vector<long long> seg_off;
    bool owns_data = true;
};

namespace am {

struct ScanBuffers { DevBuf* work; DevBuf* stats32; DevBuf* wflags; };
inline ScanBuffers scan_buffers(ScoreSide& sd) { return ScanBuffers{&sd.work, &sd.stats32, &sd.wflags}; }
struct ScanRequest {
    float margin;
    float hist_min;
    long long seg_c, seg_d;
    ScanBuffers out;
    hipEvent_t before_k3;
    long long range_a, range_b;
    long long side_nblocks;
    bool skip_launch;
    bool tail_by_caller;
    bool no_scan;
};
struct ScanResult {
    bool fused;
    SparseScores sparse;
    bool redo_ok;
    Job redo_job; PlanDev redo_pl; float redo_scale; int redo_half; int redo_npairs; const float2* redo_work; ScanCfg redo_cfg;
};
inline SparseScores plain_scores() { return SparseScores{nullptr, nullptr, nullptr, 1, 5, 5, 1.0}; }
struct Geometry {
    int logN;
    long long N, hop, nblocks, npairs;
};
struct TailPlan {
    bool on;
    long long T;
    Geometry g;
};
struct HalfScale {
    int level;
    float pre, hscale;
    float k3(float factor) const { return level ? factor / (hscale * pre) : factor; }
};
struct Footprint {
    size_t work = 0, stats32 = 0, side = 0, work_tail = 0;
    long long npairs = 0;
    void take(const Footprint& f) {
        work = std::max(work, f.work); stats32 = std::max(stats32, f.stats32); side = std::max(side, f.side);
        work_tail = std::max(work_tail, f.work_tail);
        npairs = std::max(npairs, f.npairs);
    }
};
enum class PassKind { Direct, Partitioned, Transform };
struct PassPlan {
    PassKind kind = PassKind::Direct;
    Geometry g{};
    const Plan* pl = nullptr;
    const float2* hc = nullptr;
    HalfScale hs{};
    bool fused = false;
    TailPlan tail{};
    const Plan* tail_pl = nullptr;
    const float2* tail_hc = nullptr;
    HalfScale tail_hs{};
    long long nblocks = 0, npairs = 0;
    long long ppg = 0;
    long long main_count = 0;
    std::vector<PassPlan> parts;
    Footprint need;
    Segment pair_reads(long long q, long long len) const {
        const long long last_block = (2 * q + 1 < nblocks) ? 2 * q + 1 : 2 * q;
        return Segment{2 * q * g.hop, std::min(len, last_block * g.hop + g.N)};
    }
    Segment tail_reads(long long len) const { return Segment{tail.T, std::min(len, tail.T + (tail.g.nblocks - 1) * tail.g.hop + tail.g.N)}; }
};
struct PartSpec {
    size_t max_windows;
    uint64_t first_sample;
    size_t chunk_base, chunk_total;
    std::vector<am_peak>* raw;
};
struct StreamPre {
    float* scores;
    DevBuf* stats32; DevBuf* side;
    long long pairs_done;
    long long layout_nblocks;
};

inline const void* advance_src(const void* src, size_t elements) {
    return static_cast<const char*>(src) + 4 * elements;
}

Opts snapshot_opts(const am_needle* h);
extern thread_local const Opts* t_opts_pin;
struct OptsPin {
    const Opts* prev;
    explicit OptsPin(const Opts* o) : prev(t_opts_pin) { t_opts_pin = o; }
    ~OptsPin() { t_opts_pin = prev; }
    OptsPin(const OptsPin&) = delete;
    OptsPin& operator=(const OptsPin&) = delete;
};
int check_needle(const am_needle* h);
int create_needle_common(Ctx* c, float* d_needle, size_t n, am_needle** out);
HalfScale half_scale(const am_needle* h, const Opts& o, const PlanDev& pl);
int needle_k2_spectrum(am_needle* h, const Opts& o, const Plan* pl, const float2** hc, HalfScale* hs);

struct NormSpec { bool on; double energy, thr; };
NormSpec norm_spec(const am_needle* h, const Opts& o);
int norm_check(const NormSpec& ns, int scale);
float norm_factor(const NormSpec& ns);
int norm_reserve(Ctx* c, long long max_src_len);
int normalise_scores(Ctx* c, hipStream_t st, const NormSpec& ns, const void* src, long long src_len, int src_kind, long long lead,
                     long long s, float* scores, long long a, long long b);
#define AM_NORM_UNSUPPORTED "score_norm: not supported by this entry point"

int hit_check_format(int sample_format);
double hit_floor(const am_needle* h);
double hit_floor_ratio(const am_needle* h);
struct HitWhere { long long pair; size_t hay, needle, hit; };
std::string hit_pair_name(const HitWhere& w);
std::string hit_needle_name(long long j);
int hit_check_device(const void* p, int device, const HitWhere& where);
int hit_desc(const am_needle* h, const void* hay, size_t len, int sample_format, const am_peak& pk, double thr,
             const HitWhere& where, HitDesc* d);

int hit_single_prelude(const am_needle* h, int sample_format, size_t n, const void* hay, const am_peak* peaks, const void* out,
                       const void* params, bool* done);
int hit_batch_counts(size_t n_needles, size_t n_hay, int sample_format, const void* needles, const void* d_haystacks, const void* lens,
                     const am_peak* peaks, size_t cap_per_pair, const size_t* n_peaks, const void* out, const void* params, size_t* total);
int hit_batch_needles(const am_needle* const* needles, size_t n_needles);
int stage_spans(Ctx* c, const void* haystack, const HitRange* r, size_t n, const void** at);
int hit_io_reserve(Ctx* c, size_t tab_bytes, size_t out_bytes);
int hit_table_put(Ctx* c, const void* rows, size_t off, size_t bytes);
int hit_results_get(Ctx* c, size_t tab_bytes, size_t out_bytes, const void** res);


template <class F>
int stage_host_spans(const F& f, Ctx* c, const am_needle* h, const void* haystack, size_t len, const am_peak* peaks,
                     std::vector<typename F::Desc>& hits) {
    const size_t n = hits.size();
    std::vector<HitRange> r(n);
    std::vector<const void*> at(n);
    for (size_t i = 0; i < n; ++i) r[i] = f.span(h, (size_t)peaks[i].start, len);
    int rc;
    if ((rc = stage_spans(c, haystack, r.data(), n, at.data()))) return rc;
    for (size_t i = 0; i < n; ++i) {
        const size_t e = (size_t)(static_cast<const char*>(hits[i].win) - static_cast<const char*>(haystack)) / 4;
        hits[i].win = advance_src(at[i], e - r[i].lo);
    }
    return AM_OK;
}

template <class F>
int hit_call(const F& f, bool on_host, const am_needle* h, const void* hay, size_t len, int sample_format, const am_peak* peaks,
             size_t n, typename F::Rec* out) {
    bool done = false;
    int rc = hit_single_prelude(h, sample_format, n, hay, peaks, out, f.params(), &done);
    if (rc || done) return rc;
    if ((rc = f.check_call()) || (rc = f.check(h, -1))) return rc;
    Ctx* c = h->ctx;
    std::lock_guard<std::recursive_mutex> lk(c->mu);
    if (!on_host && (rc = hit_check_device(hay, c->device, HitWhere{-1, 0, 0, 0}))) return rc;
    const double floor = f.floor(h);
    std::vector<typename F::Desc> hits(n);
    std::vector<typename F::Rec*> dst(n);
    for (size_t i = 0; i < n; ++i) {
        if ((rc = f.desc(h, hay, len, sample_format, peaks[i], floor, HitWhere{-1, 0, 0, i}, &hits[i]))) return rc;
        dst[i] = out + i * f.recs();
    }
    if (on_host && (rc = stage_host_spans(f, c, h, hay, len, peaks, hits))) return rc;
    return f.score(c, hits, dst.data());
}

template <class F>
int hit_call_batch(const F& f, const am_needle* const* needles, size_t n_needles, const void* const* d_haystacks, const size_t* lens,
                   size_t n_hay, int sample_format, const am_peak* peaks, size_t cap_per_pair, const size_t* n_peaks,
                   typename F::Rec* out) {
    size_t total = 0;
    int rc = hit_batch_counts(n_needles, n_hay, sample_format, needles, d_haystacks, lens, peaks, cap_per_pair, n_peaks, out, f.params(), &total);
    if (rc || total == 0) return rc;
    if ((rc = f.check_call()) || (rc = hit_batch_needles(needles, n_needles))) return rc;
    for (size_t j = 0; j < n_needles; ++j)
        if ((rc = f.check(needles[j], (long long)j))) return rc;
    Ctx* c = needles[0]->ctx;
    std::lock_guard<std::recursive_mutex> lk(c->mu);
    std::vector<double> floor(n_needles);
    for (size_t j = 0; j < n_needles; ++j) floor[j] = f.floor(needles[j]);
    std::vector<typename F::Desc> hits;
    std::vector<typename F::Rec*> dst;
    hits.reserve(total);
// ... 111 lines not shown
```

audio-matcher_amd/csrc/am_kernels.h:

```cpp
#pragma once

#include <hip/hip_runtime.h>
#include <stdint.h>

#include "../../include/audiomatch.h"

namespace am {

struct Job {
    const void* src;
    long long src_len;
    long long lead;
    float* dst;
    long long out_count;
    int hop;
    int nblocks;
    int first_pair;
    int src_kind;
};

struct PlanDev {
    int logN, logN1, logN2, logLo;
    const float2* tw1;
    const float2* tw2;
    const float2* twlo;
    const float2* twhi;
    const float4* twlo4;
    const float4* twhi4;
    const float4* k2j;
    const float4* k2c;
    const unsigned* mf;
};

constexpr int kColsLog = 5;
constexpr int kCols = 1 << kColsLog;
constexpr int kTile = 1024;
constexpr int kFftThreads = 256;

struct Segment {
    long long a, b;
};

hipError_t launch_k1(hipStream_t st, const Job& job, int npairs, float2* work, const PlanDev& pl, int half = 0);
hipError_t launch_k2(hipStream_t st, int npairs, float2* work, const float2* hc, const PlanDev& pl, float2* dst = nullptr,
                     int half = 0, float hscale = 1.0f, float pre = 1.0f, bool tail = false);
hipError_t launch_spectrum_to_half(hipStream_t st, const float2* hc, long long n, float scale, unsigned* out);
void set_k2_mfma(int on);
bool k2_mfma_enabled();
int k2_mfma_table_dwords();
hipError_t launch_spectrum_to_half_mfma(hipStream_t st, const float2* hc, long long n, float scale, unsigned* out);
hipError_t launch_k2_spectrum(hipStream_t st, float2* work, float2* hc_out, const PlanDev& pl);
constexpr int kMaxNeedleGroup = 8;
struct K2Group {
    const float2* hc[kMaxNeedleGroup];
    float2* dst[kMaxNeedleGroup];
    int n;
};
bool plan_k2_has_group(const PlanDev& pl);
hipError_t launch_k2_group(hipStream_t st, int npairs, const float2* work, const K2Group& grp, const PlanDev& pl);
struct ScanCfg {
    float2* stats32;
    unsigned long long* wbits;
    float* tile_theta;
    float margin;
    float hist_min;
    long long seg_c, seg_d;
    double inv_c;
    const int* only_pairs;
    int redo_tiles;
    static constexpr int kMaxEdgeSlots = 64;
    int edges_n;
    int edge_rel[kMaxEdgeSlots][4];
};
hipError_t launch_k3(hipStream_t st, const Job& job, int npairs, const float2* work,
                     const PlanDev& pl, float out_scale, const ScanCfg& scan, int half = 0, bool accumulate = false);
struct K3Group {
    int n;
    const float2* work[kMaxNeedleGroup];
    float* dst[kMaxNeedleGroup];
    float2* stats32[kMaxNeedleGroup];
    unsigned long long* wbits[kMaxNeedleGroup];
    float* tile_theta[kMaxNeedleGroup];
    float hist_min[kMaxNeedleGroup];
    float out_scale[kMaxNeedleGroup];
    long long out_count[kMaxNeedleGroup];
    long long seg_d[kMaxNeedleGroup];
    long long seg_c;
    double inv_c;
};
bool plan_k3_has_group(const PlanDev& pl);
constexpr int kMaxTailBatch = 8;
struct TailBatch {
    int n;
    const void* src[kMaxTailBatch];
    long long src_len[kMaxTailBatch];
    float* dst[kMaxTailBatch];
    long long out_count[kMaxTailBatch];
    float2* stats32[kMaxTailBatch];
};
hipError_t launch_tail_batch_k1(hipStream_t st, const TailBatch& tb, int hop, int src_kind, float2* work, const PlanDev& pl, int half);
hipError_t launch_tail_batch_k3(hipStream_t st, const TailBatch& tb, int hop, const float2* work, const PlanDev& pl, float out_scale, int half);
hipError_t launch_tail_preset_group(hipStream_t st, const K3Group& grp, long long blk, int log_n1, int log_n2);
hipError_t launch_tail_commit(hipStream_t st, const float* tail_scores, float* scores, long long n, const float2* tail_stats32, float2* stats32,
                              unsigned long long* wbits, long long words, float* theta, int tiles);
hipError_t launch_k3_group(hipStream_t st, const Job& job, int npairs, const K3Group& grp, const PlanDev& pl, const ScanCfg& scan);
constexpr int kDirectMaxNeedle = 64;
hipError_t launch_direct(hipStream_t st, const Job& job, const float* needle, int s, float out_scale);
bool plan_is_r16(const PlanDev& pl);
bool plan_is_c512(const PlanDev& pl);
bool plan_is_c512w(const PlanDev& pl);
bool plan_is_c1024(const PlanDev& pl);
bool plan_has_scan(const PlanDev& pl);
bool plan_k2_is_r16(const PlanDev& pl);
hipError_t fft_kernels_init();

hipError_t launch_nonfinite_ranges(hipStream_t st, const float* x, const Segment* ranges, int nranges, int* flags);
hipError_t launch_tile_stats(hipStream_t st, const float* g, long long n, float2* stats, int* bad = nullptr);
struct PickGroup {
    int n;
    const float* g[kMaxNeedleGroup];
    float2* stats[kMaxNeedleGroup];
    const float2* stats32[kMaxNeedleGroup];
    const unsigned long long* wbits[kMaxNeedleGroup];
    const float* theta[kMaxNeedleGroup];
    int hdr_off[kMaxNeedleGroup];
};
hipError_t launch_stats_reduce(hipStream_t st, const float2* stats32, long long n, float2* stats, int* bad = nullptr,
                               const PickGroup* grp = nullptr);
constexpr int kInlinePeaks = 4;
struct SegHeader {
    int n;
    int overflow;
    float seg_min;
    int arena_off;
    am_peak first[kInlinePeaks];
};
struct PeakArena {
    am_peak* base;
    unsigned* cursor;
    unsigned cap;
};
struct SparseScores {
    const unsigned long long* wbits;
    const float2* stats32;
    const float* tile_theta;
    int hop, log_n2, log_n1;
    double inv_hop;
    int* redo_pairs;
    unsigned char* fail_flags;
};
struct WideState {
    int* state;
    unsigned* count;
    float* seg_min;
    unsigned long long* best;
    am_peak* list;
    unsigned cap;
    int* ntiles;
    int* tiles;
};
constexpr int kWideTileList = 1024;
struct PeakPolicy {
    int order;
    int inclusive;
    int from_start;
};
hipError_t launch_peaks_wide_one(hipStream_t st, const float* g, long long g_len, const float2* stats, const Segment* d_seg,
                                 float min_prom, long long min_dist, const SparseScores& sp, const WideState& wide, const PeakPolicy& pol);
hipError_t launch_peaks_big_finish(hipStream_t st, const am_peak* list, unsigned n, long long a, long long min_dist,
                                   unsigned long long* keys, unsigned* idx, long long* table, am_peak* out, unsigned* out_n,
                                   const PeakPolicy& pol);
hipError_t launch_peaks(hipStream_t st, const float* g, long long g_len, const float2* stats,
                        const Segment* d_segs, int nsegs, float min_prom, long long min_dist,
                        am_peak* d_out, SegHeader* d_hdr, const SparseScores& sp, const PeakArena& arena,
                        const WideState& wide, bool only_failed, const PeakPolicy& pol, const PickGroup* grp = nullptr);
int sumsq_parts(long long n);
hipError_t launch_sumsq(hipStream_t st, const float* x, long long n, double* d_parts);
hipError_t launch_synth(hipStream_t st, float* out, uint32_t seed, uint32_t stream, uint64_t first,
                        long long n, float amp);
hipError_t launch_axpy(hipStream_t st, float* dst, const float* src, long long n, float gain);
hipError_t launch_synth_pcm16(hipStream_t st, int16_t* out, uint32_t seed, uint32_t stream, uint64_t first, long long frames, float amp);
hipError_t launch_add_pcm16(hipStream_t st, int16_t* dst, const int16_t* src, long long frames);
hipError_t launch_pcm_downmix(hipStream_t st, const int16_t* in, long long frames, float* out);

__device__ __forceinline__ float norm_downmix(short2 lr) {
    return __fmul_rn((float)((int)lr.x + (int)lr.y), 0.5f * (1.0f / 65535.0f));
}
typedef __attribute__((address_space(1))) const float gfloat;
typedef __attribute__((address_space(1))) const unsigned guint;
template <int KIND>
__device__ __forceinline__ float hit_sample(const void* win, long long u) {
    return KIND ? norm_downmix(__builtin_bit_cast(short2, ((guint*)win)[u])) : ((gfloat*)win)[u];
}

constexpr int kNormBlock = 1024;
constexpr int kNormTile = 2048;
inline long long norm_blocks(long long src_len) { return (src_len + kNormBlock - 1) / kNormBlock; }
hipError_t launch_block_energy(hipStream_t st, const void* src, long long src_len, int src_kind, double* blk);
struct NormJob {
    const void* src;
    long long src_len;
    int src_kind;
    long long lead, s;
    const double* blk;
    long long nblk;
    double thr;
    float* scores;
    long long a, b;
};
hipError_t launch_norm_scores(hipStream_t st, const NormJob& j);

constexpr int kHitSlice = 4096;
constexpr long long kHitMaxGridY = 65535;
struct HitDesc {
    const void* win;
    const float* needle;
    long long s;
    int kind;
    int edge;
    long long t;
    double en, thr;
    long long part0;
};
hipError_t launch_hit_scores(hipStream_t st, const HitDesc* d_hits, long long n, long long max_slices, int kind, double* parts,
                             unsigned* pflags, am_hit_score* d_out);

constexpr int kSegRadii[3] = {1, 4, 16};
inline int seg_kernel_radius(int r) { return r <= kSegRadii[0] ? kSegRadii[0] : r <= kSegRadii[1] ? kSegRadii[1] : kSegRadii[2]; }
inline int seg_record_len(int rt) { return 2 * (2 * rt + 1) + 1; }
struct SegDesc {
    const void* win;
    const float* needle;
    long long s;
    long long ulo, uhi;
    long long part0;
    double floor_ratio;
    int kind;
    int nsl;
};
hipError_t launch_hit_segments(hipStream_t st, const SegDesc* d_hits, long long n, int m, int r, int max_nsl, int kind,
                               double* parts, unsigned* pflags, am_hit_segment* d_out);

hipError_t launch_seg_slices(hipStream_t st, const SegDesc* d_hits, long long n, int m, int r, int max_nsl, int kind, double* parts,
                             unsigned* pflags);

constexpr int kWarpThreads = 256;
constexpr int kWarpCombineThreads = 256;
constexpr int kWarpMaxRates = 2 * AM_WARP_MAX_STEPS + 1;
constexpr size_t kWarpRoundBytes = (size_t)64 << 20;
struct WarpJob {
    const float* needle;
    float* out;
    long long s, s_q;
// ... 134 lines not shown
```

Measured before the change: 226.1 billion.

## Add real-input lone tail block path exploiting Hermitian symmetry in tail FFT

```diff
diff --git a/audio-matcher_amd/csrc/am_context.hip b/audio-matcher_amd/csrc/am_context.hip
--- a/audio-matcher_amd/csrc/am_context.hip
+++ b/audio-matcher_amd/csrc/am_context.hip
@@ -62,6 +62,8 @@
     {"score_norm_floor_db", {60}, opt_floor_db, &Opts::score_norm_floor_db},
     {"debug_no_realloc", {0}, opt_bool, &Opts::debug_no_realloc},
     {"debug_redo_arm_at", {-2}, opt_arm_at, &Opts::debug_redo_arm_at},
+    {"debug_tail_full_pair", {0}, opt_bool, &Opts::debug_tail_full_pair},
+    {"debug_correlate_tail", {0}, opt_bool, &Opts::debug_correlate_tail},
     {"trace_form", {0}, opt_trace_form, &Opts::trace_form},
     {"peak_filter_order", {0}, opt_bool, &Opts::peak_filter_order},
     {"distance_rule", {0}, opt_distance, &Opts::distance_rule},
diff --git a/audio-matcher_amd/csrc/am_correlate.hip b/audio-matcher_amd/csrc/am_correlate.hip
--- a/audio-matcher_amd/csrc/am_correlate.hip
+++ b/audio-matcher_amd/csrc/am_correlate.hip
@@ -52,7 +52,7 @@
     return AM_OK;
 }
 bool tail_plan(size_t s, long long out_count, const Opts& o, const Geometry& g, TailPlan* t) {
-    t->on = false;
+    t->on = false; t->lone = false;
     if (!o.tail_block || o.log_n != 0 || g.logN < 22 || !(g.nblocks & 1) || g.nblocks < 3 || (g.hop % kTile) != 0) return false;
     const long long T = (g.nblocks - 1) * g.hop, rest = out_count - T;
     for (int lt = 21; lt < g.logN; ++lt) {
@@ -63,6 +63,7 @@
         if (2 * hop < rest) continue;
         t->on = true; t->T = T;
         t->g.logN = lt; t->g.N = N; t->g.hop = hop; t->g.nblocks = (rest + hop - 1) / hop; t->g.npairs = 1;
+        t->lone = rest <= hop && lt == 21 && !o.debug_tail_full_pair;
         return true;
     }
     return false;
@@ -134,6 +135,7 @@
     if (allow_tail && pp->fused && c->stream_tail && c->ev_fork && c->ev_join && tail_plan(h->n, out_count, o, g, &pp->tail)) {
         if ((rc = get_plan(c, pp->tail.g.logN, &pp->tail_pl))) return rc;
         if ((rc = needle_k2_spectrum(h, o, pp->tail_pl, &pp->tail_hc, &pp->tail_hs))) return rc;
+        if (pp->tail_hs.level) pp->tail.lone = false;
         pp->need.work_tail = (size_t)pp->tail.g.N * sizeof(float2);
     }
     pp->nblocks = pp->tail.on ? g.nblocks - 1 : g.nblocks;
@@ -162,9 +164,20 @@
     ScanCfg scan{};
     scan.stats32 = main_scan.stats32 ? main_scan.stats32 + tail.T / 32 : nullptr;
     scan.margin = -1.0f; scan.hist_min = FLT_MAX;
-    { ProfScope ps(c, KN_OTHER, st); AM_HIP(launch_k1(st, job, 1, (float2*)c->work_tail.p, pl, hs.level)); }
-    { ProfScope ps(c, KN_OTHER, st); AM_HIP(launch_k2(st, 1, (float2*)c->work_tail.p, pp.tail_hc, pl, nullptr, hs.level, hs.hscale, hs.pre, true)); }
-    { ProfScope ps(c, KN_OTHER, st); AM_HIP(launch_k3(st, job, 1, (const float2*)c->work_tail.p, pl, hs.k3(factor), scan, hs.level, false)); }
+    if (tail.lone) {
+        TailBatch tb{};
+        tb.n = 1; tb.lone = 1u;
+        tb.src[0] = job.src; tb.src_len[0] = job.src_len; tb.out_count[0] = job.out_count;
+        tb.dst[0] = job.dst; tb.stats32[0] = scan.stats32;
+        float2* work = (float2*)c->work_tail.p;
+        { ProfScope ps(c, KN_OTHER, st); AM_HIP(launch_tail_batch_k1(st, tb, job.hop, src_kind, work, pl, hs.level)); }
+        { ProfScope ps(c, KN_OTHER, st); AM_HIP(launch_tail_batch_k2(st, tb, work, pp.tail_hc, pl, hs.level, hs.hscale, hs.pre)); }
+        { ProfScope ps(c, KN_OTHER, st); AM_HIP(launch_tail_batch_k3(st, tb, job.hop, work, pl, hs.k3(factor), hs.level)); }
+    } else {
+        { ProfScope ps(c, KN_OTHER, st); AM_HIP(launch_k1(st, job, 1, (float2*)c->work_tail.p, pl, hs.level)); }
+        { ProfScope ps(c, KN_OTHER, st); AM_HIP(launch_k2(st, 1, (float2*)c->work_tail.p, pp.tail_hc, pl, nullptr, hs.level, hs.hscale, hs.pre, true)); }
+        { ProfScope ps(c, KN_OTHER, st); AM_HIP(launch_k3(st, job, 1, (const float2*)c->work_tail.p, pl, hs.k3(factor), scan, hs.level, false)); }
+    }
     if (main_scan.stats32 && main_scan.margin >= 0.0f && main_scan.wbits && main_scan.tile_theta) {
         const BallotLayout bl = ballot_layout(pp.pl->dev.logN1, pp.pl->dev.logN2);
         const size_t blk = (size_t)(pp.g.nblocks - 1);
@@ -184,7 +197,8 @@
     int rc;
     PassPlan own;
     if (!plan) {
-        if ((rc = pass_plan(h, o, out_count, scan_req && !scan_req->no_scan && lead == 0, &own))) return rc;
+        const bool allow_tail = lead == 0 && (scan_req ? !scan_req->no_scan : o.debug_correlate_tail != 0);
+        if ((rc = pass_plan(h, o, out_count, allow_tail, &own))) return rc;
         plan = &own;
     }
     if (res) { res->fused = false; res->redo_ok = false; res->sparse = plain_scores(); }
diff --git a/audio-matcher_amd/csrc/am_engine.hip b/audio-matcher_amd/csrc/am_engine.hip
--- a/audio-matcher_amd/csrc/am_engine.hip
+++ b/audio-matcher_amd/csrc/am_engine.hip
@@ -171,10 +171,11 @@
         tb.out_count[j] = job.out_count;
         tb.dst[j] = static_cast<float*>(c->tail_scores.p) + slot * sl.scores;
         tb.stats32[j] = static_cast<float2*>(c->tail_stats.p) + slot * sl.stats;
+        if (plans[k].tail.lone) tb.lone |= 1u << j;
     }
     float2* work = static_cast<float2*>(c->work_tail.p);
     { ProfScope ps(c, KN_OTHER); AM_HIP(launch_tail_batch_k1(c->stream, tb, (int)first.g.hop, src_kind, work, pl->dev, hs.level)); }
-    { ProfScope ps(c, KN_OTHER); AM_HIP(launch_k2(c->stream, tb.n, work, hc, pl->dev, nullptr, hs.level, hs.hscale, hs.pre, true)); }
+    { ProfScope ps(c, KN_OTHER); AM_HIP(launch_tail_batch_k2(c->stream, tb, work, hc, pl->dev, hs.level, hs.hscale, hs.pre)); }
     { ProfScope ps(c, KN_OTHER); AM_HIP(launch_tail_batch_k3(c->stream, tb, (int)first.g.hop, work, pl->dev, hs.k3(factor), hs.level)); }
     return AM_OK;
 }
diff --git a/audio-matcher_amd/csrc/am_fft.hip b/audio-matcher_amd/csrc/am_fft.hip
--- a/audio-matcher_amd/csrc/am_fft.hip
+++ b/audio-matcher_amd/csrc/am_fft.hip
@@ -207,6 +207,23 @@
     }
 }
 
+__device__ __forceinline__ void twiddle_chain_mirror(float2* x, float2 base, float2 step, float2 step4, float2 up) {
+    base.y = -base.y; step.y = -step.y; step4.y = -step4.y;
+    float2 g = base;
+#pragma unroll
+    for (int k = 0; k < 16; k += 4) {
+        if (k) g = cmul(g, step4);
+        if (k == 8) g = cmul(g, up);
+        float2 c = g;
+        x[k] = cmul(x[k], c);
+#pragma unroll
+        for (int j = 1; j < 4; ++j) {
+            c = cmul(c, step);
+            x[k + j] = cmul(x[k + j], c);
+        }
+    }
+}
+
 typedef float f32x4 __attribute__((ext_vector_type(4)));
 typedef float f32x2 __attribute__((ext_vector_type(2)));
 __device__ __forceinline__ __amdgpu_buffer_rsrc_t make_rsrc(const void* p, unsigned bytes) {
@@ -245,6 +262,7 @@
 
 constexpr int kR16LogN1 = 8, kR16LogN2 = 13;
 constexpr int kN2 = 1 << kR16LogN2;
+constexpr int kLoneRows = (1 << kR16LogN1) / 2 + 1;
 
 __device__ __forceinline__ float downmix_s16(short2 lr) {
     return __fmul_rn((float)((int)lr.x + (int)lr.y), 0.5f * (1.0f / 65535.0f));
@@ -369,7 +387,19 @@
     twiddle_chain<16, false, true>(x1, w.base1, w.step1);
 }
 
-template <int KIND, int HALF>
+template <int KIND>
+__device__ __forceinline__ void k1_load_real(const Job& job, long long col, int in_stride, int hi, long long baseA, bool fast,
+                                             float2 (&x0)[16], float2 (&x1)[16]) {
+#pragma unroll
+    for (int a = 0; a < 16; ++a) {
+        const long long n = (long long)(a * 16 + hi) * in_stride + col;
+        const float2 va = fast ? load_sample2<KIND>(job.src, baseA + n) : load2_padded<KIND>(job.src, baseA + n, job.src_len);
+        x0[a] = make_float2(va.x, 0.f);
+        x1[a] = make_float2(va.y, 0.f);
+    }
+}
+
+template <int KIND, int HALF, bool LONE = false>
 __device__ __forceinline__ void k1_cols_fwd_r16_tile(const Job& job, float2* __restrict__ work, const PlanDev& pl) {
     extern __shared__ float4 lds4[];
     const int t = threadIdx.x;
@@ -400,6 +430,23 @@
         }
         return;
     }
+    if constexpr (LONE) {
+        static_assert(HALF == 0, "the lone forms exist for the f32 work matrix");
+        const long long col = (long long)n2_0 + 2 * cp;
+        const bool fastA = ((reinterpret_cast<uintptr_t>(job.src) & 7) == 0) && ((baseA & 1) == 0) && baseA >= 0 && baseA + N <= job.src_len;
+        const K1Twiddles w = k1_twiddles(pl, col, hi);
+        k1_load_real<KIND>(job, col, kN2, hi, baseA, fastA, x0, x1);
+        k1_transform(w, reinterpret_cast<float2*>(lds4), hi, cp, x0, x1);
+        float4* __restrict__ out4 = reinterpret_cast<float4*>(work + ((size_t)blockIdx.y << pl.logN) + n2_0) + cp;
+#pragma unroll
+        for (int bp = 0; bp <= 8; ++bp) {
+            if (bp == 8 && hi != 0) break;
+            const size_t k1 = (size_t)(hi + 16 * bp);
+            out4[k1 * (kN2 / 2)] = make_float4(x0[brev<16>(bp)].x, x0[brev<16>(bp)].y,
+                                                 x1[brev<16>(bp)].x, x1[brev<16>(bp)].y);
+        }
+        return;
+    }
     k1_tile<KIND>(job, pl, reinterpret_cast<float2*>(lds4), (long long)n2_0 + 2 * cp, kN2, hi, cp, baseA, baseB, validB, fast, x0, x1);
     if (HALF) {
         uint2* __restrict__ out2 = reinterpret_cast<uint2*>(reinterpret_cast<unsigned*>(work) + ((size_t)blockIdx.y << pl.logN) + n2_0) + cp;
@@ -431,6 +478,16 @@
     job.src = tb.src[z]; job.src_len = tb.src_len[z]; job.lead = 0; job.dst = nullptr; job.out_count = tb.out_count[z];
     job.hop = hop; job.nblocks = (int)((tb.out_count[z] + hop - 1) / hop); job.first_pair = -(int)z; job.src_kind = KIND;
     k1_cols_fwd_r16_tile<KIND, HALF>(job, work, pl);
+}
+template <int KIND>
+__global__ void __launch_bounds__(256, 4)
+lone_cols_fwd_r16(TailBatch tb, int hop, float2* __restrict__ work, PlanDev pl) {
+    const unsigned z = blockIdx.y;
+    Job job;
+    job.src = tb.src[z]; job.src_len = tb.src_len[z]; job.lead = 0; job.dst = nullptr; job.out_count = tb.out_count[z];
+    job.hop = hop; job.nblocks = (int)((tb.out_count[z] + hop - 1) / hop); job.first_pair = -(int)z; job.src_kind = KIND;
+    if ((tb.lone >> z) & 1u) k1_cols_fwd_r16_tile<KIND, 0, true>(job, work, pl);
+    else k1_cols_fwd_r16_tile<KIND, 0>(job, work, pl);
 }
 
 __device__ __forceinline__ void wave_sync_lds() {
@@ -794,11 +851,9 @@
 
 template <bool HALF>
 __device__ __forceinline__ void k2_rows_r16_planes_row(float2* __restrict__ work, const float2* __restrict__ hc, float2* __restrict__ dst,
-                                                       const PlanDev& pl, unsigned npairs, float hscale) {
+                                                       const PlanDev& pl, unsigned row, unsigned slot, float hscale) {
     extern __shared__ float4 lds4[];
     float2* lds2 = reinterpret_cast<float2*>(lds4);
-    unsigned row, slot;
-    k2_place(npairs, row, slot);
     const size_t row_off = ((size_t)slot << pl.logN) + (size_t)row * kN2;
     const __amdgpu_buffer_rsrc_t rrow = HALF ? make_rsrc(reinterpret_cast<unsigned*>(work) + row_off, kN2 * 4)
                                              : make_rsrc(work + row_off, kN2 * 8);
@@ -840,13 +895,24 @@
 __global__ void __launch_bounds__(256, kK2pWaves)
 k2_rows_r16_planes(float2* __restrict__ work, const float2* __restrict__ hc, float2* __restrict__ dst, PlanDev pl, unsigned npairs,
                    float hscale) {
-    k2_rows_r16_planes_row<HALF>(work, hc, dst, pl, npairs, hscale);
+    unsigned row, slot;
+    k2_place(npairs, row, slot);
+    k2_rows_r16_planes_row<HALF>(work, hc, dst, pl, row, slot, hscale);
 }
 template <bool HALF>
 __global__ void __launch_bounds__(256, kK2pWaves)
 tail_rows_r16_planes(float2* __restrict__ work, const float2* __restrict__ hc, float2* __restrict__ dst, PlanDev pl, unsigned npairs,
                      float hscale) {
-    k2_rows_r16_planes_row<HALF>(work, hc, dst, pl, npairs, hscale);
+    unsigned row, slot;
+    k2_place(npairs, row, slot);
+    k2_rows_r16_planes_row<HALF>(work, hc, dst, pl, row, slot, hscale);
+}
+__global__ void __launch_bounds__(256, kK2pWaves)
+lone_rows_r16_planes(float2* __restrict__ work, const float2* __restrict__ hc, PlanDev pl, unsigned npairs, unsigned lone) {
+    unsigned row, slot;
+    k2_place(npairs, row, slot);
+    if (((lone >> slot) & 1u) && row >= (unsigned)kLoneRows) return;
+    k2_rows_r16_planes_row<false>(work, hc, nullptr, pl, row, slot, 1.0f);
 }
 
 constexpr int kK2gpWaves = 3;
@@ -1229,7 +1295,7 @@
     return e;
 }
 
-template <int HB, bool ACC = false, bool SCALED = false>
+template <int HB, bool ACC = false, bool SCALED = false, bool NO_B = false>
 __device__ __forceinline__ void k3_finish(const Job& job, const ScanCfg& scan, const K3Edges& ed, float2* lds2,
                                           int n2_0, int out_stride, int t, long long blkA, long long blkB,
                                           float out_scale, const float2 (&x0)[16], const float2 (&x1)[16]) {
@@ -1264,10 +1330,14 @@
         scan_put<HB>(lds2, hi, cp, sa0, sa1);
         wave_sync_lds();
         scan_row_minmax<HB>(lds4, row, wholeA, leftA < 32 ? leftA : 32, rmnA, rmxA);
-        wave_sync_lds();
-        scan_put<HB>(lds2, hi, cp, sb0, sb1);
-        wave_sync_lds();
-        scan_row_minmax<HB>(lds4, row, wholeB, leftB < 32 ? leftB : 32, rmnB, rmxB);
+        if constexpr (NO_B) {
+            rmnB = FLT_MAX; rmxB = -FLT_MAX;
+        } else {
+            wave_sync_lds();
+            scan_put<HB>(lds2, hi, cp, sb0, sb1);
+            wave_sync_lds();
+            scan_row_minmax<HB>(lds4, row, wholeB, leftB < 32 ? leftB : 32, rmnB, rmxB);
+        }
         float tminA = wave_min_f(leftA > 0 ? rmnA : FLT_MAX), tminB = wave_min_f(leftB > 0 ? rmnB : FLT_MAX);
         float* slots = reinterpret_cast<float*>(lds2 + scan_row_of<HB>(t & ~63) * 16);
         wave_sync_lds();
@@ -1323,7 +1393,7 @@
             if (ACC && (a & 3) == 3) __builtin_amdgcn_sched_barrier(0);
         }
     }
-    if (wantB[0] | wantB[1]) {
+    if (!NO_B && (wantB[0] | wantB[1])) {
 #pragma unroll
         for (int a = 0; a < 16; ++a) {
             if (!((wantB[a >> 3] >> ((a & 7) * 4)) & 1u)) continue;
@@ -1343,7 +1413,7 @@
 }
 
 
-template <bool ACC = false>
+template <bool ACC = false, bool LONE = false>
 __device__ __forceinline__ void k3_tile(const Job& job, const PlanDev& pl, const ScanCfg& scan, float2* lds2,
                                         int n2_0, int out_stride, int t, long long blkA, long long blkB,
                                         float out_scale, float2 (&x0)[16], float2 (&x1)[16], const ScanCfg* geo = nullptr) {
@@ -1362,11 +1432,13 @@
         float2 step0, step1, step0q, step1q;
         tw_big_pair(pl, (n2 * 16u) & maskN, step0, step0q);
         tw_big_pair(pl, ((n2 + 1) * 16u) & maskN, step1, step1q);
-        twiddle_chain<16, true, false>(x0, base0, step0, step0q);
+        if constexpr (LONE) twiddle_chain_mirror(x0, base0, step0, step0q, tw_big(pl, (n2 << kR16LogN1) & maskN));
+        else twiddle_chain<16, true, false>(x0, base0, step0, step0q);
         dif<16, true>(x0);
 #pragma unroll
         for (int b = 0; b < 16; ++b) lds2[(hi * 16 + b) * 16 + cp] = x0[brev<16>(b)];
-        twiddle_chain<16, true, false>(x1, base1, step1, step1q);
+        if constexpr (LONE) twiddle_chain_mirror(x1, base1, step1, step1q, tw_big(pl, ((n2 + 1) << kR16LogN1) & maskN));
+        else twiddle_chain<16, true, false>(x1, base1, step1, step1q);
     }
     dif<16, true>(x1);
     __syncthreads();
@@ -1382,7 +1454,7 @@
     for (int ap = 0; ap < 16; ++ap) x1[ap] = lds2[(ap * 16 + hi) * 16 + cp];
     twiddle_nat<16, true>(x1, w256, w256q);
     dif<16, true>(x1);
-    k3_finish<4, ACC, true>(job, scan, ed, lds2, n2_0, out_stride, t, blkA, blkB, out_scale, x0, x1);
+    k3_finish<4, ACC, true, LONE>(job, scan, ed, lds2, n2_0, out_stride, t, blkA, blkB, out_scale, x0, x1);
 }
 
 __device__ __forceinline__ void k3_tile_h16(const Job& job, const PlanDev& pl, const ScanCfg& scan, float2* lds2,
@@ -1425,7 +1497,8 @@
 
 constexpr int kK3Waves = 3;
 constexpr int kK3LoadAux = 2, kK3hLoadAux = 2;
-template <int HALF, bool ACC>
+constexpr int kK3LoneLoadAux = 0;
+template <int HALF, bool ACC, bool LONE = false>
 __device__ __forceinline__ void k3_cols_inv_r16_tile(unsigned lin, float4* lds4, const Job& job, const float2* __restrict__ work,
                                                      const PlanDev& pl, float out_scale, const ScanCfg& scan, const ScanCfg* geo = nullptr) {
     const int t = threadIdx.x;
@@ -1461,13 +1534,22 @@
         const __amdgpu_buffer_rsrc_t rin = make_rsrc(work + ((size_t)slot << pl.logN) + n2_0, (unsigned)((((size_t)1 << pl.logN) - n2_0) * 8));
         const unsigned voff = (unsigned)hi * (kN2 * 8u) + (unsigned)cp * 16u;
 #pragma unroll
-        for (int bp = 0; bp < 16; ++bp) {
-            const float4 v = buf_load4<kK3LoadAux>(rin, voff, (unsigned)bp * (16u * kN2 * 8u));
+        for (int bp = 0; bp < (LONE ? 8 : 16); ++bp) {
+            const float4 v = buf_load4<LONE ? kK3LoneLoadAux : kK3LoadAux>(rin, voff, (unsigned)bp * (16u * kN2 * 8u));
             x0[bp] = make_float2(v.x, v.y);
             x1[bp] = make_float2(v.z, v.w);
         }
-    }
-    k3_tile<ACC>(job, pl, scan, reinterpret_cast<float2*>(lds4), n2_0, kN2, t, blkA, blkB, out_scale, x0, x1, geo);
+        if constexpr (LONE) {
+            const unsigned voffm = (unsigned)(16 - hi) * (kN2 * 8u) + (unsigned)cp * 16u;
+#pragma unroll
+            for (int bp = 8; bp < 16; ++bp) {
+                const float4 v = buf_load4<kK3LoneLoadAux>(rin, voffm, (unsigned)(15 - bp) * (16u * kN2 * 8u));
+                x0[bp] = make_float2(v.x, -v.y);
+                x1[bp] = make_float2(v.z, -v.w);
+            }
+        }
+    }
+    k3_tile<ACC, LONE>(job, pl, scan, reinterpret_cast<float2*>(lds4), n2_0, kN2, t, blkA, blkB, out_scale, x0, x1, geo);
 }
 template <int HALF, bool ACC = false, int REDO = 0>
 __global__ void __launch_bounds__(256, REDO ? 4 : kK3Waves)
@@ -1509,6 +1591,20 @@
     const float2* mywork = HALF ? reinterpret_cast<const float2*>(reinterpret_cast<const unsigned*>(work) + ((size_t)z << pl.logN))
                                 : work + ((size_t)z << pl.logN);
     k3_cols_inv_r16_tile<HALF, false>(blockIdx.x, lds4, job, mywork, pl, out_scale, mine);
+}
+__global__ void __launch_bounds__(256, kK3Waves)
+lone_cols_inv_r16(TailBatch tb, int hop, const float2* __restrict__ work, PlanDev pl, float out_scale) {
+    extern __shared__ float4 lds4[];
+    const unsigned z = blockIdx.y;
+    Job job;
+    job.src = nullptr; job.src_len = 0; job.lead = 0; job.dst = tb.dst[z]; job.out_count = tb.out_count[z];
+    job.hop = hop; job.nblocks = (int)((tb.out_count[z] + hop - 1) / hop); job.first_pair = 0; job.src_kind = 0;
+    ScanCfg mine;
+    mine.stats32 = tb.stats32[z]; mine.wbits = nullptr; mine.tile_theta = nullptr; mine.margin = -1.0f; mine.hist_min = FLT_MAX;
+    mine.seg_c = 0; mine.seg_d = 0; mine.inv_c = 0.0; mine.only_pairs = nullptr; mine.redo_tiles = 0; mine.edges_n = 0;
+    const float2* mywork = work + ((size_t)z << pl.logN);
+    if ((tb.lone >> z) & 1u) k3_cols_inv_r16_tile<0, false, true>(blockIdx.x, lds4, job, mywork, pl, out_scale, mine);
+    else k3_cols_inv_r16_tile<0, false>(blockIdx.x, lds4, job, mywork, pl, out_scale, mine);
 }
 
 __global__ void __launch_bounds__(256)
@@ -2288,12 +2384,16 @@
     {{tail_cols_fwd_r16<1, 0>, 256, kR16LdsK1}, {tail_cols_fwd_r16<1, 1>, 256, kR16LdsK1}, {tail_cols_fwd_r16<1, 2>, 256, kR16LdsK1}},
 };
 
+static constexpr Variant<TailK1Fn> kLoneK1[2] = {{lone_cols_fwd_r16<0>, 256, kR16LdsK1}, {lone_cols_fwd_r16<1>, 256, kR16LdsK1}};
+
 using K2Fn = void (*)(float2*, const float2*, float2*, PlanDev, unsigned, float);
 static constexpr Variant<K2Fn> kK2[2][2] = {
     {{k2_rows_r16_planes<false>, 256, kK2hLds}, {tail_rows_r16_planes<false>, 256, kK2hLds}},
     {{k2_rows_r16_planes<true>, 256, kK2hLds}, {tail_rows_r16_planes<true>, 256, kK2hLds}},
 };
 static constexpr Variant<K2Fn> kK2Spectrum = {k2_rows_r16_spectrum, 256, kR16Lds};
+using LoneK2Fn = void (*)(float2*, const float2*, PlanDev, unsigned, unsigned);
+static constexpr Variant<LoneK2Fn> kLoneK2 = {lone_rows_r16_planes, 256, kK2hLds};
 using K2hFn = void (*)(unsigned*, const unsigned*, unsigned*, PlanDev, unsigned, float);
 static constexpr Variant<K2hFn> kK2h[2] = {{k2_rows_h16, 256, kK2hLds}, {tail_rows_h16, 256, kK2hLds}};
 static constexpr Variant<K2hFn> kK2Mfma = {k2_rows_m16, 256, kK2mLds};
@@ -2321,6 +2421,7 @@
 using TailK3Fn = void (*)(TailBatch, int, const float2*, PlanDev, float);
 static constexpr Variant<TailK3Fn> kTailK3[3] = {
     {tail_cols_inv_r16<0>, 256, kR16LdsK3}, {tail_cols_inv_r16<1>, 256, kR16LdsK3}, {tail_cols_inv_r16<2>, 256, kR16LdsK3}};
+static constexpr Variant<TailK3Fn> kLoneK3 = {lone_cols_inv_r16, 256, kR16LdsK3};
 
 template <typename Fn>
 static hipError_t allow_lds(const Variant<Fn>& v) {
@@ -2347,6 +2448,9 @@
     if (e == hipSuccess) e = allow_lds(kK3Gen);
     if (e == hipSuccess) e = allow_lds(kK3Group);
     if (e == hipSuccess) e = allow_lds(kTailK3);
+    if (e == hipSuccess) e = allow_lds(kLoneK1);
+    if (e == hipSuccess) e = allow_lds(kLoneK2);
+    if (e == hipSuccess) e = allow_lds(kLoneK3);
     return e;
 }
 
@@ -2420,10 +2524,20 @@
 hipError_t launch_tail_batch_k1(hipStream_t st, const TailBatch& tb, int hop, int src_kind, float2* work, const PlanDev& pl, int half) {
     if (!plan_is_r16(pl) || tb.n < 1 || tb.n > kMaxTailBatch) return hipErrorInvalidValue;
     const dim3 grid((1u << pl.logN2) >> kColsLog, (unsigned)tb.n);
+    if (tb.lone) return half ? hipErrorInvalidValue : launch_row(kLoneK1[src_kind == 1 ? 1 : 0], grid, st, tb, hop, work, pl);
     return launch_row(kTailK1[src_kind == 1 ? 1 : 0][half_level(half)], grid, st, tb, hop, work, pl);
+}
+hipError_t launch_tail_batch_k2(hipStream_t st, const TailBatch& tb, float2* work, const float2* hc, const PlanDev& pl,
+                                int half, float hscale, float pre) {
+    if (!plan_is_r16(pl) || tb.n < 1 || tb.n > kMaxTailBatch) return hipErrorInvalidValue;
+    if (!tb.lone) return launch_k2(st, tb.n, work, hc, pl, nullptr, half, hscale, pre, true);
+    if (half) return hipErrorInvalidValue;
+    const unsigned rows = tb.lone == (1u << tb.n) - 1u ? ((unsigned)kLoneRows + 7u) & ~7u : 1u << kR16LogN1;
+    return launch_row(kLoneK2, dim3((unsigned)tb.n * rows), st, work, hc, pl, (unsigned)tb.n, tb.lone);
 }
 hipError_t launch_tail_batch_k3(hipStream_t st, const TailBatch& tb, int hop, const float2* work, const PlanDev& pl, float out_scale, int half) {
     if (!plan_is_r16(pl) || tb.n < 1 || tb.n > kMaxTailBatch) return hipErrorInvalidValue;
+    if (tb.lone) return half ? hipErrorInvalidValue : launch_row(kLoneK3, dim3(kN2 >> kColsLog, (unsigned)tb.n), st, tb, hop, work, pl, out_scale);
     return launch_row(kTailK3[half_level(half)], dim3(kN2 >> kColsLog, (unsigned)tb.n), st, tb, hop, work, pl, out_scale);
 }
 hipError_t launch_tail_preset_group(hipStream_t st, const K3Group& grp, long long blk, int log_n1, int log_n2) {
diff --git a/audio-matcher_amd/csrc/am_internal.h b/audio-matcher_amd/csrc/am_internal.h
--- a/audio-matcher_amd/csrc/am_internal.h
+++ b/audio-matcher_amd/csrc/am_internal.h
@@ -33,7 +33,7 @@
 Hooks snapshot_hooks();
 
 struct Opts {
-    long long log_n, pairs_per_group, half, batch_overlap, needle_group, dense, device_redo, debug_no_realloc, debug_redo_arm_at;
+    long long log_n, pairs_per_group, half, batch_overlap, needle_group, dense, device_redo, debug_no_realloc, debug_redo_arm_at, debug_tail_full_pair, debug_correlate_tail;
     long long peak_filter_order, distance_rule, tail_window, surrounding_from, k3_group, pick_group, tail_block, host_pick_wait;
     long long profile_mask, profile_every, pick_priority;
     long long score_norm, score_norm_floor_db;
@@ -234,6 +234,7 @@
     bool on;
     long long T;
     Geometry g;
+    bool lone;
 };
 struct HalfScale {
     int level;
diff --git a/audio-matcher_amd/csrc/am_kernels.h b/audio-matcher_amd/csrc/am_kernels.h
--- a/audio-matcher_amd/csrc/am_kernels.h
+++ b/audio-matcher_amd/csrc/am_kernels.h
@@ -97,8 +97,11 @@
     float* dst[kMaxTailBatch];
     long long out_count[kMaxTailBatch];
     float2* stats32[kMaxTailBatch];
+    unsigned lone;
 };
 hipError_t launch_tail_batch_k1(hipStream_t st, const TailBatch& tb, int hop, int src_kind, float2* work, const PlanDev& pl, int half);
+hipError_t launch_tail_batch_k2(hipStream_t st, const TailBatch& tb, float2* work, const float2* hc, const PlanDev& pl,
+                                int half, float hscale, float pre);
 hipError_t launch_tail_batch_k3(hipStream_t st, const TailBatch& tb, int hop, const float2* work, const PlanDev& pl, float out_scale, int half);
 hipError_t launch_tail_preset_group(hipStream_t st, const K3Group& grp, long long blk, int log_n1, int log_n2);
 hipError_t launch_tail_commit(hipStream_t st, const float* tail_scores, float* scores, long long n, const float2* tail_stats32, float2* stats32,
```

Result: no change. 225.2 billion (-0.4%).
